# chzhang18/RAG

Hardware: AMD Instinct MI355X
Metric: disparity maps/sec at 384x1248 D=192 (Matching-Net forward) (higher is better)
Workload: dtype f32 (RAGMI_F32X3: level-3/6/12 3x3x3 convolutions with fp32 operands split into power-of-two-scaled FP16 hi+lo halves on the 16-bit matrix cores, hi*hi + hi*lo + lo*hi, fp32 accumulate: fp32-class accuracy, bound in include/rag_amd.h; strict_fp32 holds the RAGMI_F32 number); 1 GPU; BASELINE configs[1]: 1 stereo pair(s)/GPU/step, 384x1248, D=192, f32, all-conv genotype, (left_fea,right_fea)->disp, inputs resident in HBM; global_batch=1, launch=hipGraph, ranks_seen=1

## Files before the change

### include/rag_amd.h

```cpp
#ifndef RAG_AMD_H
#define RAG_AMD_H

#include <stdint.h>

#ifdef __cplusplus
extern "C" {
#endif

#define RAGMI_OK 0
#define RAGMI_EINVAL (-1)
#define RAGMI_EUNSUPPORTED (-2)
#define RAGMI_ELAUNCH (-3)

#define RAGMI_F32 0
#define RAGMI_BF16 1
#define RAGMI_F32X3 2

#define RAGMI_MAX_GROUPS 16

int ragmi_version(void);
const char* ragmi_last_error(void);

int ragmi_costvol_fwd(const void* left_fea, const void* right_fea, void* cost,
                      int B, int C, int d, int h, int w, int dtype, void* stream);

int64_t ragmi_conv3d_k3_packed_elems(int Cout, int Cin);
int ragmi_conv3d_k3_pack(const void* weight, void* packed, int Cout, int Cin, int dtype, void* stream);

int ragmi_conv3d_k3_fwd(const void* x, int64_t x_bstride,
                        const void* packed_weight, const void* scale, const void* shift, int relu,
                        void* y, int64_t y_bstride, const int32_t* y_group_ch,
                        const void* res, int64_t res_bstride, const int32_t* res_group_ch,
                        int B, int Cin, int Cout, int D, int H, int W,
                        int dtype, void* stream);

typedef struct {
  const void* weight;
  const void* scale;
  const void* shift;
  int32_t relu;
  void* y;
  int64_t y_bstride;
  int32_t y_ch0;
  int32_t cout;
} ragmi_tail_t;
int ragmi_down2_tail_supported(int D, int H, int W);

#define RAGMI_CONV_RELU 1
#define RAGMI_CONV_X_G4 2
#define RAGMI_CONV_Y_G4 4
#define RAGMI_TAIL_G4 4
#define RAGMI_TAIL_F32 8
#define RAGMI_TAIL_ROWS 16
#define RAGMI_OUT_F32 0x100
int ragmi_conv3d_k3_g4_caps(int Cin, int Cout, int B, int D, int H, int W, int nset, int ntail, int ndown, int dtype);

int ragmi_conv3d_k3_fwd_ex(const void* x, int64_t x_bstride,
                           const void* packed_weight, const void* scale, const void* shift, int relu,
                           void* y, int64_t y_bstride, const int32_t* y_group_ch,
                           const void* res, int64_t res_bstride, const int32_t* res_group_ch,
                           int B, int Cin, int Cout, int D, int H, int W,
                           int store_main, int ntail, const ragmi_tail_t* tails, int dtype, void* stream);
int ragmi_conv3d_k3_dual_fwd_ex(const void* x, int64_t x_bstride,
                                int CinA, const void* packedA, const void* scaleA, const void* shiftA,
                                int CinB, const void* packedB, const void* scaleB, const void* shiftB,
                                int relu, void* y, int64_t y_bstride, const int32_t* y_group_ch,
                                const void* res, int64_t res_bstride, const int32_t* res_group_ch,
                                int B, int Cout, int D, int H, int W,
                                int store_main, int ntail, const ragmi_tail_t* tails, int dtype, void* stream);

int ragmi_conv3d_k3_small_fwd(const void* x, int64_t x_bstride, const void* weight, const void* scale,
                              const void* shift, int relu, void* y, int64_t y_bstride, int y_ch0,
                              const void* res, int64_t res_bstride, int res_ch0,
                              int B, int Cin, int Cout, int D, int H, int W, int dtype, void* stream);

int ragmi_conv3d_k3_small_fwd_ex(const void* x, int64_t x_bstride, const void* weight, const void* scale,
                                 const void* shift, int relu, void* y, int64_t y_bstride, int y_ch0,
                                 const void* res, int64_t res_bstride, int res_ch0,
                                 int B, int Cin, int Cout, int D, int H, int W, int dtype, int y_dtype, void* stream);

int ragmi_conv3d_k3_dual_fwd(const void* x, int64_t x_bstride,
                             int CinA, const void* packedA, const void* scaleA, const void* shiftA,
                             int CinB, const void* packedB, const void* scaleB, const void* shiftB,
                             int relu, void* y, int64_t y_bstride, const int32_t* y_group_ch,
                             const void* res, int64_t res_bstride, const int32_t* res_group_ch,
                             int B, int Cout, int D, int H, int W, int dtype, void* stream);

int ragmi_conv3d_k3_plan(int Cout, int B, int D, int H, int W, int nset, int32_t* log_tx,
                         int32_t* rows_per_lane, int32_t* launch_groups, int32_t max_launches);

int ragmi_conv3d_k1_fwd(const void* x, int64_t x_bstride,
                        const void* weight, const void* scale, const void* shift, int relu,
                        void* y, int64_t y_bstride, int y_ch0,
                        int B, int Cin, int Cout, int64_t DHW,
                        int dtype, void* stream);

int ragmi_conv3d_k1_chain_supported(int Cin, int Cmid, int Cout);
int ragmi_conv3d_k1_chain_fwd(const void* x, int64_t x_bstride, const void* weight1, const void* scale1, const void* shift1, int relu1,
                              int Cmid, const void* weight2, const void* scale2, const void* shift2, int relu2,
                              void* y, int64_t y_bstride, int y_ch0, int B, int Cin, int Cout, int64_t DHW, int dtype, void* stream);

int ragmi_conv3d_k1_fwd_ex(const void* x, int64_t x_bstride, const void* weight, int w_transposed, const void* scale,
                           const void* shift, int relu, void* y, int64_t y_bstride, int y_ch0, int B, int Cin,
                           int Cout, int64_t DHW, int dtype, void* stream);

int ragmi_conv3d_k1_resample_fwd(const void* x, int64_t x_bstride, int Di, int Hi, int Wi,
                                 const void* weight, const void* scale, const void* shift, int relu,
                                 void* y, int64_t y_bstride, int y_ch0,
                                 int B, int Cin, int Cout, int Do, int Ho, int Wo, int align_corners,
                                 int dtype, void* stream);

typedef struct {
  const void* x;
  int64_t x_bstride;
  int32_t Di, Hi, Wi;
  const void* weight;
  const void* scale;
  const void* shift;
  int32_t relu;
  int32_t y_ch0;
  int32_t Cin, Cout;
} ragmi_k1r_t;
int ragmi_conv3d_k1_resample_pair_fwd(const ragmi_k1r_t* a, const ragmi_k1r_t* b, void* y, int64_t y_bstride,
                                      int B, int Do, int Ho, int Wo, int align_corners, int dtype, void* stream);
int ragmi_conv3d_k1_resample_multi_fwd(const ragmi_k1r_t* const* specs, void* const* ys, const int64_t* y_bstrides, int n, int B,
                                       int Do, int Ho, int Wo, int align_corners, int dtype, void* stream);

typedef struct {
  const void* x;
  int64_t x_bstride;
  int32_t Cin, Hi, Wi;
  const void* weight;
  const void* scale;
  const void* shift;
  int32_t relu;
} ragmi_cell2d_in_t;
int ragmi_cell2d_supported(int C, int Cin0, int Cin1, int Cout, int H, int W, int dtype);
int ragmi_cell2d_fwd(const ragmi_cell2d_in_t* s0, const ragmi_cell2d_in_t* s1, int C, const void* packedA, const void* scaleA,
                     const void* shiftA, const void* packedB, const void* scaleB, const void* shiftB, int relu, void* y,
                     int64_t y_bstride, const int32_t* y_group_ch, int B, int Cout, int H, int W, int dtype, void* stream);

int ragmi_trilinear3d_fwd(const void* x, void* y, int B, int C,
                          int Di, int Hi, int Wi, int Do, int Ho, int Wo,
                          int align_corners, int dtype, void* stream);

int ragmi_upconv3d_c1_supported(int Cin, int Di, int Hi, int Wi);
int ragmi_upconv3d_c1_fwd(const void* x, int64_t x_bstride, const void* weight, const void* scale, const void* shift, int relu, void* y,
                          int64_t y_bstride, int y_ch0, int B, int Cin, int Di, int Hi, int Wi, int dtype, int y_dtype, void* stream);

int ragmi_trilinear3d_act_fwd(const void* x, int64_t x_bstride, void* y, int64_t y_bstride, int y_ch0, int relu, int B, int C,
                              int Di, int Hi, int Wi, int Do, int Ho, int Wo, int align_corners, int dtype, void* stream);

int ragmi_conv2d_k3_strided_fwd(const void* x, const void* weight, const void* scale, const void* shift, int relu,
                                void* y, int B, int Cin, int Cout, int H, int W, int stride, int dtype, void* stream);

int ragmi_add_fwd(const void* a, int64_t a_bstride, int a_ch0,
                  const void* b, int64_t b_bstride, int b_ch0,
                  void* y, int64_t y_bstride, int y_ch0,
                  int B, int C, int64_t DHW, int dtype, void* stream);

int ragmi_disp_softargmin_fwd(const void* cost, void* out, int B, int d, int h, int w,
                              int maxdisp, int Ho, int Wo, int dtype, void* stream);

int ragmi_disparity_regression_fwd(const void* prob, void* out, int B, int D, int H, int W,
                                   int dtype, void* stream);

int64_t ragmi_costvol_stem_weights_elems(int C, int Cout);
int ragmi_costvol_stem_prepare(const void* weight, void* variants, int C, int Cout, void* stream);
int64_t ragmi_costvol_stem_workspace_elems(int B, int C, int Cout, int D, int H, int W);
int ragmi_costvol_stem_fwd(const void* left, const void* right, const void* variants, const void* scale, const void* shift, int relu,
                           void* y, int64_t y_bstride, void* workspace, int B, int C, int Cout, int D, int H, int W,
                           int ntail, const ragmi_tail_t* tails, int dtype, void* stream);

int ragmi_costvol_stem_conv3d_supported(int C, int Cmid, int Cout, int B, int D, int H, int W, int ntail, int dtype);
int ragmi_costvol_stem_conv3d_fwd(const void* left, const void* right, const void* variants, const void* scale0, const void* shift0, int relu0,
                                  void* workspace, int ntail0, const ragmi_tail_t* tails0,
                                  const void* packed_weight, const void* scale, const void* shift, int relu,
                                  void* y, int64_t y_bstride, const int32_t* y_group_ch, int store_main, int ntail, const ragmi_tail_t* tails,
                                  int B, int C, int Cmid, int Cout, int D, int H, int W, int dtype, void* stream);

int ragmi_conv3d_k3_uses_x3(int Cin, int Cout, int B, int D, int H, int W, int nset, int has_res, int ntail, int dtype);

int ragmi_conv3d_k3_pack_ex(const void* weight, void* packed, int Cout, int Cin, int transpose, int planar2d, int dtype, void* stream);

int ragmi_conv3d_k3_pack_for(const void* weight, void* packed, int Cout, int Cin, int transpose, int planar2d, int for_dtype, void* stream);


int64_t ragmi_bn_workspace_elems(int B, int C, int64_t DHW);
int ragmi_bn_train_stats_fwd(const void* x, int64_t x_bstride, int B, int C, int64_t DHW, const void* gamma, const void* beta,
                             void* running_mean, void* running_var, void* num_batches_tracked, float momentum, float eps,
                             void* workspace, void* mean, void* invstd, void* scale, void* shift, void* stream);

int ragmi_bn_train_act_fwd(const void* x, int64_t x_bstride, int B, int C, int64_t DHW, const void* gamma, const void* beta,
                           void* running_mean, void* running_var, void* num_batches_tracked, float momentum, float eps, int relu,
                           void* workspace, void* mean, void* invstd, void* scale, void* shift, void* y, int64_t y_bstride, int y_ch0,
                           const void* res, int64_t res_bstride, int res_ch0, void* stream);

int ragmi_bn_act_bwd(const void* dy, int64_t dy_bstride, int dy_ch0, const void* x, int64_t x_bstride, const void* scale,
                     const void* shift, int relu, const void* mean, const void* invstd, int training, int B, int C, int64_t DHW,
                     void* workspace, void* dx, int64_t dx_bstride, void* dgamma, void* dbeta, int accumulate, void* stream);

int ragmi_bn_act_fwd(const void* x, int64_t x_bstride, const void* scale, const void* shift, int relu,
                     const void* res, int64_t res_bstride, int res_ch0,
                     void* y, int64_t y_bstride, int y_ch0, int B, int C, int64_t DHW, void* stream);

int ragmi_bn_act_bwd_coeffs(const void* dy, int64_t dy_bstride, int dy_ch0, const void* x, int64_t x_bstride,
                            const void* scale, const void* shift, int relu, const void* mean, const void* invstd, int training,
                            int B, int C, int64_t DHW, void* workspace, void* c1, void* c2, void* c3, void* dgamma, void* dbeta,
                            int accumulate, void* stream);

int ragmi_bn_act_bwd_apply(const void* dy, int64_t dy_bstride, int dy_ch0, const void* x, int64_t x_bstride,
                           const void* scale, const void* shift, int relu, const void* c1, const void* c2, const void* c3,
                           void* dx, int64_t dx_bstride, int B, int C, int64_t DHW, void* stream);

int64_t ragmi_conv3d_k3_wgrad_workspace_elems(int B, int Cin, int Cout, int D, int H, int W);
int ragmi_conv3d_k3_wgrad(const void* x, int64_t x_bstride, const void* g, int64_t g_bstride, int g_ch0, void* const* dw_list, int n_dw,
                          int accumulate, int planar2d, void* workspace, int B, int Cin, int Cout, int D, int H, int W, void* stream);

int ragmi_conv3d_k1_wgrad(const void* x, int64_t x_bstride, const void* g, int64_t g_bstride, int g_ch0, void* dw,
                          int B, int Cin, int Cout, int64_t DHW, void* stream);

int ragmi_trilinear3d_bwd(const void* dy, void* dx, int B, int C, int Di, int Hi, int Wi, int Do, int Ho, int Wo,
                          int align_corners, void* stream);

int ragmi_costvol_bwd(const void* dcost, void* dleft, void* dright, int B, int C, int d, int h, int w, void* stream);

int ragmi_disp_softargmin_bwd(const void* cost, const void* dout, void* dcost, int B, int d, int h, int w,
                              int maxdisp, int Ho, int Wo, void* stream);

int ragmi_conv2d_k3_strided_dgrad(const void* g, const void* weight, void* dx, int B, int Cin, int Cout, int H, int W, int stride,
                                  void* stream);
int ragmi_conv2d_k3_strided_wgrad(const void* x, const void* g, void* dw, int B, int Cin, int Cout, int H, int W, int stride,
                                  void* stream);

int ragmi_disparity_regression_bwd(const void* dout, void* dprob, int B, int D, int H, int W, void* stream);

int ragmi_stereo_metrics_fwd(const void* disp_est, const void* disp_gt, int B, int H, int W, float maxdisp, void* acc, void* out,
                             void* stream);

int ragmi_masked_smooth_l1_bwd(const void* disp_est, const void* disp_gt, const void* out, const void* gout, void* ddisp,
                               int B, int H, int W, float maxdisp, void* stream);

int64_t ragmi_selfsup_loss_workspace_elems(int B, int H, int W);
int ragmi_selfsup_loss_fwd(const void* left, const void* right, const void* disp, int B, int C, int H, int W, int dtype,
                           void* workspace, void* out, void* unit_grad, void* stream);

int ragmi_selfsup_loss_bwd(const void* unit_grad, const void* gout, void* grad, int64_t n, void* stream);

int ragmi_depth_head_supported(int Cin, int Hi, int Wi, int H, int W, int scale, int dtype);
int ragmi_depth_head_fwd(const void* y, const void* w3, const void* w1, const void* b1, void* out, int B, int Cin, int Hi, int Wi,
                         int H, int W, int scale, float max_depth, int dtype, void* stream);

int ragmi_depth_metrics_workspace_elems(long long n);
int ragmi_depth_metrics_fwd(const void* est, const void* gt, long long n, float variance_focus, void* workspace, void* out10, int dtype,
                            void* stream);

int64_t ragmi_depth_head_bwd_workspace_elems(int B, int Cin, int H, int W);
int ragmi_depth_head_bwd(const void* y, const void* w3, const void* w1, const void* b1, const void* d_out, void* dy, void* dw3,
                         void* dw1, void* db1, int accumulate, void* workspace, int B, int Cin, int Hi, int Wi, int H, int W, int scale,
                         float max_depth, int dtype, void* stream);

int ragmi_silog_loss_workspace_elems(long long n);
int ragmi_silog_loss_fwd(const void* est, const void* gt, long long n, float variance_focus, void* workspace, void* out, void* saved,
                         int dtype, void* stream);

int ragmi_silog_loss_bwd(const void* est, const void* gt, long long n, float variance_focus, const void* saved, const void* gout,
                         void* grad, int dtype, void* stream);

int64_t ragmi_sgd_workspace_bytes(void);
int ragmi_sgd_clip_step(void* param, void* grad, void* momentum_buf, int64_t n, float lr, float momentum, float weight_decay,
                        float max_norm, int first_step, void* workspace, void* norm_out, void* stream);

#define RAGMI_GT_F32 0
#define RAGMI_GT_U16 1
int ragmi_prep_batch(const void* left_u8, const void* right_u8, const void* gt, int gt_dtype, float gt_scale, const void* origin,
                     void* left, void* right, void* gt_out, int B, int Hs, int Ws, int H, int W, float mean0, float mean1, float mean2,
                     float std0, float std1, float std2, const void* stats_left, const void* stats_right, const void* stats_source,
                     void* stream);

int64_t ragmi_color_stats_workspace_elems(int B, int Hs, int Ws);
int ragmi_color_stats(const void* img_u8, int B, int Hs, int Ws, void* workspace, void* stats, void* stream);

int ragmi_color_transfer(const void* target_u8, const void* stats_target, const void* stats_source, void* out_u8, int B, int H, int W,
                         void* stream);

int ragmi_graph_node_census(void* graph, int32_t* n_kernel, int32_t* n_memcpy, int32_t* n_memset, int32_t* n_other);

#ifdef __cplusplus
}
#endif
#endif
```

### rag_amd/_lib.py

```python
import ctypes
import os
import threading

_HERE = os.path.dirname(os.path.abspath(__file__))
_LIB = None
_LOCK = threading.Lock()

c_void_p, c_int, c_int64, c_float = ctypes.c_void_p, ctypes.c_int, ctypes.c_int64, ctypes.c_float
c_int32_p = ctypes.POINTER(ctypes.c_int32)

class TailSpec(ctypes.Structure):
    _fields_ = [("weight", c_void_p), ("scale", c_void_p), ("shift", c_void_p), ("relu", ctypes.c_int32),
                ("y", c_void_p), ("y_bstride", c_int64), ("y_ch0", ctypes.c_int32), ("cout", ctypes.c_int32)]


c_tail_p = ctypes.POINTER(TailSpec)


class K1RSpec(ctypes.Structure):
    _fields_ = [("x", c_void_p), ("x_bstride", c_int64), ("Di", ctypes.c_int32), ("Hi", ctypes.c_int32), ("Wi", ctypes.c_int32),
                ("weight", c_void_p), ("scale", c_void_p), ("shift", c_void_p), ("relu", ctypes.c_int32),
                ("y_ch0", ctypes.c_int32), ("Cin", ctypes.c_int32), ("Cout", ctypes.c_int32)]


c_k1r_p = ctypes.POINTER(K1RSpec)


class Cell2dIn(ctypes.Structure):
    _fields_ = [("x", c_void_p), ("x_bstride", c_int64), ("Cin", ctypes.c_int32), ("Hi", ctypes.c_int32), ("Wi", ctypes.c_int32),
                ("weight", c_void_p), ("scale", c_void_p), ("shift", c_void_p), ("relu", ctypes.c_int32)]


c_cell2d_p = ctypes.POINTER(Cell2dIn)

SIGNATURES = {
    "ragmi_version": (c_int, []),
    "ragmi_last_error": (ctypes.c_char_p, []),
    "ragmi_graph_node_census": (c_int, [c_void_p, c_int32_p, c_int32_p, c_int32_p, c_int32_p]),
    "ragmi_costvol_fwd": (c_int, [c_void_p, c_void_p, c_void_p, c_int, c_int, c_int, c_int, c_int, c_int, c_void_p]),
    "ragmi_costvol_stem_weights_elems": (c_int64, [c_int, c_int]),
    "ragmi_costvol_stem_prepare": (c_int, [c_void_p, c_void_p, c_int, c_int, c_void_p]),
    "ragmi_costvol_stem_workspace_elems": (c_int64, [c_int, c_int, c_int, c_int, c_int, c_int]),
    "ragmi_costvol_stem_fwd": (c_int, [c_void_p, c_void_p, c_void_p, c_void_p, c_void_p, c_int, c_void_p, c_int64, c_void_p,
                                       c_int, c_int, c_int, c_int, c_int, c_int, c_int, c_tail_p, c_int, c_void_p]),
    "ragmi_costvol_stem_conv3d_supported": (c_int, [c_int] * 9),
    "ragmi_costvol_stem_conv3d_fwd": (c_int, [c_void_p, c_void_p, c_void_p, c_void_p, c_void_p, c_int, c_void_p, c_int, c_tail_p,
                                              c_void_p, c_void_p, c_void_p, c_int, c_void_p, c_int64, c_int32_p, c_int, c_int, c_tail_p,
                                              c_int, c_int, c_int, c_int, c_int, c_int, c_int, c_int, c_void_p]),
    "ragmi_conv3d_k3_uses_x3": (c_int, [c_int] * 10),
    "ragmi_conv3d_k3_g4_caps": (c_int, [c_int] * 10),
    "ragmi_conv3d_k3_packed_elems": (c_int64, [c_int, c_int]),
    "ragmi_conv3d_k3_pack": (c_int, [c_void_p, c_void_p, c_int, c_int, c_int, c_void_p]),
    "ragmi_conv3d_k3_fwd": (c_int, [c_void_p, c_int64, c_void_p, c_void_p, c_void_p, c_int,
                                    c_void_p, c_int64, c_int32_p, c_void_p, c_int64, c_int32_p,
                                    c_int, c_int, c_int, c_int, c_int, c_int, c_int, c_void_p]),
    "ragmi_conv3d_k3_small_fwd": (c_int, [c_void_p, c_int64, c_void_p, c_void_p, c_void_p, c_int, c_void_p, c_int64, c_int,
                                          c_void_p, c_int64, c_int, c_int, c_int, c_int, c_int, c_int, c_int, c_int, c_void_p]),
    "ragmi_conv3d_k3_small_fwd_ex": (c_int, [c_void_p, c_int64, c_void_p, c_void_p, c_void_p, c_int, c_void_p, c_int64, c_int,
                                             c_void_p, c_int64, c_int, c_int, c_int, c_int, c_int, c_int, c_int, c_int, c_int, c_void_p]),
    "ragmi_conv3d_k3_dual_fwd": (c_int, [c_void_p, c_int64, c_int, c_void_p, c_void_p, c_void_p,
                                         c_int, c_void_p, c_void_p, c_void_p, c_int, c_void_p, c_int64, c_int32_p,
                                         c_void_p, c_int64, c_int32_p, c_int, c_int, c_int, c_int, c_int, c_int, c_void_p]),
    "ragmi_conv3d_k3_fwd_ex": (c_int, [c_void_p, c_int64, c_void_p, c_void_p, c_void_p, c_int,
                                       c_void_p, c_int64, c_int32_p, c_void_p, c_int64, c_int32_p,
                                       c_int, c_int, c_int, c_int, c_int, c_int, c_int, c_int, c_tail_p, c_int, c_void_p]),
    "ragmi_conv3d_k3_dual_fwd_ex": (c_int, [c_void_p, c_int64, c_int, c_void_p, c_void_p, c_void_p,
                                            c_int, c_void_p, c_void_p, c_void_p, c_int, c_void_p, c_int64, c_int32_p,
                                            c_void_p, c_int64, c_int32_p, c_int, c_int, c_int, c_int, c_int,
                                            c_int, c_int, c_tail_p, c_int, c_void_p]),
    "ragmi_conv3d_k3_plan": (c_int, [c_int, c_int, c_int, c_int, c_int, c_int, c_int32_p, c_int32_p, c_int32_p, c_int]),
    "ragmi_conv3d_k1_fwd": (c_int, [c_void_p, c_int64, c_void_p, c_void_p, c_void_p, c_int,
                                    c_void_p, c_int64, c_int, c_int, c_int, c_int, c_int64, c_int, c_void_p]),
    "ragmi_conv3d_k1_chain_supported": (c_int, [c_int] * 3),
    "ragmi_conv3d_k1_chain_fwd": (c_int, [c_void_p, c_int64, c_void_p, c_void_p, c_void_p, c_int, c_int, c_void_p, c_void_p, c_void_p, c_int,
                                          c_void_p, c_int64, c_int, c_int, c_int, c_int, c_int64, c_int, c_void_p]),
    "ragmi_conv3d_k1_fwd_ex": (c_int, [c_void_p, c_int64, c_void_p, c_int, c_void_p, c_void_p, c_int,
                                       c_void_p, c_int64, c_int, c_int, c_int, c_int, c_int64, c_int, c_void_p]),
    "ragmi_conv3d_k1_resample_fwd": (c_int, [c_void_p, c_int64, c_int, c_int, c_int, c_void_p, c_void_p, c_void_p, c_int,
                                             c_void_p, c_int64, c_int, c_int, c_int, c_int, c_int, c_int, c_int, c_int, c_int, c_void_p]),
    "ragmi_conv3d_k1_resample_pair_fwd": (c_int, [c_k1r_p, c_k1r_p, c_void_p, c_int64, c_int, c_int, c_int, c_int, c_int, c_int, c_void_p]),
    "ragmi_conv3d_k1_resample_multi_fwd": (c_int, [ctypes.POINTER(c_k1r_p), ctypes.POINTER(c_void_p), ctypes.POINTER(c_int64), c_int, c_int,
                                                   c_int, c_int, c_int, c_int, c_int, c_void_p]),
    "ragmi_down2_tail_supported": (c_int, [c_int, c_int, c_int]),
    "ragmi_cell2d_supported": (c_int, [c_int] * 7),
    "ragmi_cell2d_fwd": (c_int, [c_cell2d_p, c_cell2d_p, c_int, c_void_p, c_void_p, c_void_p, c_void_p, c_void_p, c_void_p, c_int,
                                 c_void_p, c_int64, c_int32_p, c_int, c_int, c_int, c_int, c_int, c_void_p]),
    "ragmi_upconv3d_c1_supported": (c_int, [c_int, c_int, c_int, c_int]),
    "ragmi_upconv3d_c1_fwd": (c_int, [c_void_p, c_int64, c_void_p, c_void_p, c_void_p, c_int, c_void_p, c_int64, c_int, c_int, c_int, c_int,
                                      c_int, c_int, c_int, c_int, c_void_p]),
    "ragmi_trilinear3d_act_fwd": (c_int, [c_void_p, c_int64, c_void_p, c_int64, c_int, c_int, c_int, c_int, c_int, c_int, c_int, c_int,
                                          c_int, c_int, c_int, c_int, c_void_p]),
    "ragmi_trilinear3d_fwd": (c_int, [c_void_p, c_void_p, c_int, c_int, c_int, c_int, c_int, c_int, c_int, c_int,
                                      c_int, c_int, c_void_p]),
    "ragmi_conv2d_k3_strided_fwd": (c_int, [c_void_p, c_void_p, c_void_p, c_void_p, c_int, c_void_p, c_int, c_int, c_int, c_int, c_int,
                                            c_int, c_int, c_void_p]),
    "ragmi_add_fwd": (c_int, [c_void_p, c_int64, c_int, c_void_p, c_int64, c_int, c_void_p, c_int64, c_int,
                              c_int, c_int, c_int64, c_int, c_void_p]),
    "ragmi_bn_workspace_elems": (c_int64, [c_int, c_int, c_int64]),
    "ragmi_bn_train_stats_fwd": (c_int, [c_void_p, c_int64, c_int, c_int, c_int64, c_void_p, c_void_p, c_void_p, c_void_p, c_void_p,
                                         c_float, c_float, c_void_p, c_void_p, c_void_p, c_void_p, c_void_p, c_void_p]),
    "ragmi_conv3d_k3_pack_ex": (c_int, [c_void_p, c_void_p, c_int, c_int, c_int, c_int, c_int, c_void_p]),
    "ragmi_conv3d_k3_pack_for": (c_int, [c_void_p, c_void_p, c_int, c_int, c_int, c_int, c_int, c_void_p]),
    "ragmi_sgd_workspace_bytes": (c_int64, []),
    "ragmi_sgd_clip_step": (c_int, [c_void_p, c_void_p, c_void_p, c_int64, c_float, c_float, c_float, c_float, c_int, c_void_p, c_void_p,
                                    c_void_p]),
    "ragmi_bn_train_act_fwd": (c_int, [c_void_p, c_int64, c_int, c_int, c_int64, c_void_p, c_void_p, c_void_p, c_void_p, c_void_p, c_float,
                                       c_float, c_int, c_void_p, c_void_p, c_void_p, c_void_p, c_void_p, c_void_p, c_int64, c_int,
                                       c_void_p, c_int64, c_int, c_void_p]),
    "ragmi_bn_act_bwd": (c_int, [c_void_p, c_int64, c_int, c_void_p, c_int64, c_void_p, c_void_p, c_int, c_void_p, c_void_p, c_int, c_int,
                                 c_int, c_int64, c_void_p, c_void_p, c_int64, c_void_p, c_void_p, c_int, c_void_p]),
    "ragmi_bn_act_fwd": (c_int, [c_void_p, c_int64, c_void_p, c_void_p, c_int, c_void_p, c_int64, c_int, c_void_p, c_int64, c_int,
                                 c_int, c_int, c_int64, c_void_p]),
    "ragmi_bn_act_bwd_coeffs": (c_int, [c_void_p, c_int64, c_int, c_void_p, c_int64, c_void_p, c_void_p, c_int, c_void_p, c_void_p, c_int,
                                        c_int, c_int, c_int64, c_void_p, c_void_p, c_void_p, c_void_p, c_void_p, c_void_p, c_int, c_void_p]),
    "ragmi_bn_act_bwd_apply": (c_int, [c_void_p, c_int64, c_int, c_void_p, c_int64, c_void_p, c_void_p, c_int, c_void_p, c_void_p,
                                       c_void_p, c_void_p, c_int64, c_int, c_int, c_int64, c_void_p]),
    "ragmi_conv3d_k3_wgrad_workspace_elems": (c_int64, [c_int, c_int, c_int, c_int, c_int, c_int]),
    "ragmi_conv3d_k3_wgrad": (c_int, [c_void_p, c_int64, c_void_p, c_int64, c_int, ctypes.POINTER(c_void_p), c_int, c_int, c_int, c_void_p,
                                      c_int, c_int, c_int, c_int, c_int, c_int, c_void_p]),
    "ragmi_conv3d_k1_wgrad": (c_int, [c_void_p, c_int64, c_void_p, c_int64, c_int, c_void_p, c_int, c_int, c_int, c_int64, c_void_p]),
    "ragmi_trilinear3d_bwd": (c_int, [c_void_p, c_void_p, c_int, c_int, c_int, c_int, c_int, c_int, c_int, c_int, c_int, c_void_p]),
    "ragmi_costvol_bwd": (c_int, [c_void_p, c_void_p, c_void_p, c_int, c_int, c_int, c_int, c_int, c_void_p]),
    "ragmi_conv2d_k3_strided_dgrad": (c_int, [c_void_p, c_void_p, c_void_p, c_int, c_int, c_int, c_int, c_int, c_int, c_void_p]),
    "ragmi_conv2d_k3_strided_wgrad": (c_int, [c_void_p, c_void_p, c_void_p, c_int, c_int, c_int, c_int, c_int, c_int, c_void_p]),
    "ragmi_disparity_regression_bwd": (c_int, [c_void_p, c_void_p, c_int, c_int, c_int, c_int, c_void_p]),
    "ragmi_stereo_metrics_fwd": (c_int, [c_void_p, c_void_p, c_int, c_int, c_int, c_float, c_void_p, c_void_p, c_void_p]),
    "ragmi_masked_smooth_l1_bwd": (c_int, [c_void_p, c_void_p, c_void_p, c_void_p, c_void_p, c_int, c_int, c_int, c_float, c_void_p]),
    "ragmi_selfsup_loss_workspace_elems": (c_int64, [c_int, c_int, c_int]),
    "ragmi_selfsup_loss_fwd": (c_int, [c_void_p, c_void_p, c_void_p, c_int, c_int, c_int, c_int, c_int, c_void_p, c_void_p, c_void_p,
                                       c_void_p]),
    "ragmi_selfsup_loss_bwd": (c_int, [c_void_p, c_void_p, c_void_p, c_int64, c_void_p]),
    "ragmi_depth_head_supported": (c_int, [c_int] * 7),
    "ragmi_depth_head_fwd": (c_int, [c_void_p, c_void_p, c_void_p, c_void_p, c_void_p, c_int, c_int, c_int, c_int, c_int, c_int, c_int,
                                     c_float, c_int, c_void_p]),
    "ragmi_depth_metrics_workspace_elems": (c_int, [ctypes.c_longlong]),
    "ragmi_depth_metrics_fwd": (c_int, [c_void_p, c_void_p, ctypes.c_longlong, c_float, c_void_p, c_void_p, c_int, c_void_p]),
    "ragmi_depth_head_bwd_workspace_elems": (c_int64, [c_int, c_int, c_int, c_int]),
    "ragmi_depth_head_bwd": (c_int, [c_void_p, c_void_p, c_void_p, c_void_p, c_void_p, c_void_p, c_void_p, c_void_p, c_void_p, c_int,
                                     c_void_p, c_int, c_int, c_int, c_int, c_int, c_int, c_int, c_float, c_int, c_void_p]),
    "ragmi_silog_loss_workspace_elems": (c_int, [ctypes.c_longlong]),
    "ragmi_silog_loss_fwd": (c_int, [c_void_p, c_void_p, ctypes.c_longlong, c_float, c_void_p, c_void_p, c_void_p, c_int, c_void_p]),
    "ragmi_silog_loss_bwd": (c_int, [c_void_p, c_void_p, ctypes.c_longlong, c_float, c_void_p, c_void_p, c_void_p, c_int, c_void_p]),
    "ragmi_prep_batch": (c_int, [c_void_p, c_void_p, c_void_p, c_int, c_float, c_void_p, c_void_p, c_void_p, c_void_p,
                                 c_int, c_int, c_int, c_int, c_int, c_float, c_float, c_float, c_float, c_float, c_float,
                                 c_void_p, c_void_p, c_void_p, c_void_p]),
    "ragmi_color_stats_workspace_elems": (c_int64, [c_int, c_int, c_int]),
    "ragmi_color_stats": (c_int, [c_void_p, c_int, c_int, c_int, c_void_p, c_void_p, c_void_p]),
    "ragmi_color_transfer": (c_int, [c_void_p, c_void_p, c_void_p, c_void_p, c_int, c_int, c_int, c_void_p]),
    "ragmi_disp_softargmin_bwd": (c_int, [c_void_p, c_void_p, c_void_p, c_int, c_int, c_int, c_int, c_int, c_int, c_int, c_void_p]),
    "ragmi_disp_softargmin_fwd": (c_int, [c_void_p, c_void_p, c_int, c_int, c_int, c_int, c_int, c_int, c_int,
                                          c_int, c_void_p]),
    "ragmi_disparity_regression_fwd": (c_int, [c_void_p, c_void_p, c_int, c_int, c_int, c_int, c_int, c_void_p]),
}


def lib_path() -> str:
    return os.environ.get("RAG_AMD_LIB", os.path.join(_HERE, "lib", "librag_amd.so"))


def load_library():
    global _LIB
    if _LIB is not None:
        return _LIB
    with _LOCK:
        if _LIB is None:
            path = lib_path()
            if not os.path.exists(path):
                raise RuntimeError(
                    f"rag_amd: HIP library not found at {path}. Build it with `make` at the repo root "
                    "(or `python -c 'import __graft_entry__ as g; g.build()'`). There is no CPU fallback.")
            lib = ctypes.CDLL(path)
            for name, (restype, argtypes) in SIGNATURES.items():
                fn = getattr(lib, name)
                fn.restype = restype
                fn.argtypes = argtypes
            _LIB = lib
    return _LIB


def check(status: int, what: str) -> None:
    if status != 0:
        msg = load_library().ragmi_last_error()
        raise RuntimeError(f"rag_amd.{what} failed with status {status}: {msg.decode() if msg else ''}")
```

### rag_amd/csrc/pointwise.hip

```cpp
#include <algorithm>

#include "common.h"

namespace ragmi {

struct K1Args {
  const void* x;
  int64_t x_bstride;
  const float* w;
  const float* scale;
  const float* shift;
  void* y;
  int64_t y_bstride;
  int y_ch0;
  int Cin, Cout, co0;
  int64_t dhw;
  int relu;
  int w_sco, w_sci;
  int y_f32;
};

template <class T, int NCO, bool VEC>
__global__ __launch_bounds__(256) void conv_k1_kernel(K1Args a) {
  constexpr int V = VEC ? 4 : 1;
  extern __shared__ __attribute__((aligned(16))) float k1_w[];
  a.co0 = blockIdx.z * NCO;
  for (int i = threadIdx.x; i < a.Cin * NCO; i += 256) {
    const int ci = i / NCO, co = a.co0 + i % NCO;
    k1_w[i] = co < a.Cout ? a.w[co * a.w_sco + ci * a.w_sci] : 0.f;
  }
  float* const k1_bn = k1_w + a.Cin * NCO;
  if (threadIdx.x < NCO) {
    const int co = min(a.co0 + (int)threadIdx.x, a.Cout - 1);
    k1_bn[threadIdx.x] = a.scale ? a.scale[co] : 1.f;
    k1_bn[NCO + threadIdx.x] = a.scale ? a.shift[co] : 0.f;
  }
  __syncthreads();
  const int64_t p = ((int64_t)blockIdx.x * 256 + threadIdx.x) * V;
  if (p >= a.dhw) return;
  const int b = blockIdx.y;
  const T* xp = static_cast<const T*>(a.x) + b * a.x_bstride + p;
  float acc[NCO][V];
#pragma unroll
  for (int j = 0; j < NCO; ++j)
#pragma unroll
    for (int k = 0; k < V; ++k) acc[j][k] = 0.f;

#pragma unroll 4
  for (int ci = 0; ci < a.Cin; ++ci) {
    float xv[V];
    if constexpr (VEC) {
      ld4(xp + (int64_t)ci * a.dhw, xv);
    } else {
      xv[0] = ld(xp + (int64_t)ci * a.dhw);
    }
    float wv[NCO];
#pragma unroll
    for (int j = 0; j < NCO; j += 4) {
      const float4 q = *reinterpret_cast<const float4*>(k1_w + ci * NCO + j);
      wv[j] = q.x; wv[j + 1] = q.y; wv[j + 2] = q.z; wv[j + 3] = q.w;
    }
#pragma unroll
    for (int j = 0; j < NCO; ++j)
#pragma unroll
      for (int k = 0; k < V; ++k) acc[j][k] = fmaf(wv[j], xv[k], acc[j][k]);
  }
  T* yp = static_cast<T*>(a.y) + b * a.y_bstride + p;
#pragma unroll
  for (int j = 0; j < NCO; ++j) {
    const int co = a.co0 + j;
    if (co >= a.Cout) break;
    const float sc = k1_bn[j], sh = k1_bn[NCO + j];
    float o[V];
#pragma unroll
    for (int k = 0; k < V; ++k) {
      float v = a.scale ? fmaf(acc[j][k], sc, sh) : acc[j][k];
      o[k] = a.relu ? fmaxf(v, 0.f) : v;
    }
    T* dst = yp + (int64_t)(a.y_ch0 + co) * a.dhw;
    if constexpr (VEC) st4(dst, o); else st(dst, o[0]);
  }
}

template <class T, int CMID, int NCO>
__global__ __launch_bounds__(256) void conv_k1_chain_kernel(K1Args a, const float* __restrict__ w2, const float* __restrict__ scale2,
                                                            const float* __restrict__ shift2, int relu2) {
  extern __shared__ __attribute__((aligned(16))) float kc_w[];
  float* const w2l = kc_w + a.Cin * CMID;
  float* const bn1 = w2l + CMID * NCO;
  float* const bn2 = bn1 + 2 * CMID;
  for (int i = threadIdx.x; i < a.Cin * CMID; i += 256) kc_w[i] = a.w[(i % CMID) * a.Cin + i / CMID];
  for (int i = threadIdx.x; i < CMID * NCO; i += 256) w2l[i] = w2[(i % NCO) * CMID + i / NCO];
  if (threadIdx.x < CMID) { bn1[threadIdx.x] = a.scale ? a.scale[threadIdx.x] : 1.f; bn1[CMID + threadIdx.x] = a.scale ? a.shift[threadIdx.x] : 0.f; }
  if (threadIdx.x < NCO) { bn2[threadIdx.x] = scale2 ? scale2[threadIdx.x] : 1.f; bn2[NCO + threadIdx.x] = scale2 ? shift2[threadIdx.x] : 0.f; }
  __syncthreads();
  const int64_t p = (int64_t)blockIdx.x * 256 + threadIdx.x;
  if (p >= a.dhw) return;
  const int b = blockIdx.y;
  const T* xp = static_cast<const T*>(a.x) + b * a.x_bstride + p;
  float h[CMID];
#pragma unroll
  for (int j = 0; j < CMID; ++j) h[j] = 0.f;
#pragma unroll 4
  for (int ci = 0; ci < a.Cin; ++ci) {
    const float xv = ld(xp + (int64_t)ci * a.dhw);
#pragma unroll
    for (int j = 0; j < CMID; j += 4) {
      const float4 q = *reinterpret_cast<const float4*>(kc_w + ci * CMID + j);
      h[j] = fmaf(q.x, xv, h[j]); h[j + 1] = fmaf(q.y, xv, h[j + 1]); h[j + 2] = fmaf(q.z, xv, h[j + 2]); h[j + 3] = fmaf(q.w, xv, h[j + 3]);
    }
  }
#pragma unroll
  for (int j = 0; j < CMID; ++j) {
    float v = a.scale ? fmaf(h[j], bn1[j], bn1[CMID + j]) : h[j];
    v = a.relu ? fmaxf(v, 0.f) : v;
    if constexpr (!std::is_same<T, float>::value) { const bf16_t r = to_bf16(v); v = ld(&r); }
    h[j] = v;
  }
  float acc[NCO];
#pragma unroll
  for (int k = 0; k < NCO; ++k) acc[k] = 0.f;
#pragma unroll
  for (int j = 0; j < CMID; ++j) {
#pragma unroll
    for (int k = 0; k < NCO; k += 4) {
      const float4 q = *reinterpret_cast<const float4*>(w2l + j * NCO + k);
      acc[k] = fmaf(q.x, h[j], acc[k]); acc[k + 1] = fmaf(q.y, h[j], acc[k + 1]); acc[k + 2] = fmaf(q.z, h[j], acc[k + 2]); acc[k + 3] = fmaf(q.w, h[j], acc[k + 3]);
    }
  }
  T* yp = static_cast<T*>(a.y) + b * a.y_bstride + p;
#pragma unroll
  for (int k = 0; k < NCO; ++k) {
    float v = scale2 ? fmaf(acc[k], bn2[k], bn2[NCO + k]) : acc[k];
    st(yp + (int64_t)(a.y_ch0 + k) * a.dhw, relu2 ? fmaxf(v, 0.f) : v);
  }
}

struct __attribute__((packed, aligned(4))) K1RF2 { float a, b; };
struct K1RArgs {
  K1Args k;
  int Di, Hi, Wi, Do, Ho, Wo;
  float sd, sh, sw;
  int align;
};

struct K1RPair {
  K1RArgs c[3];
  int splits[3];
};

template <class T, int NCO>
__global__ __launch_bounds__(256) void conv_k1_resample_kernel(K1RPair pr) {
  extern __shared__ __attribute__((aligned(16))) float k1r_w[];
  const int which = (int)blockIdx.z >= pr.splits[0] + pr.splits[1] ? 2 : ((int)blockIdx.z >= pr.splits[0] ? 1 : 0);
  const K1RArgs& r = pr.c[which];
  const K1Args& a = r.k;
  const int64_t ovol = (int64_t)r.Do * r.Ho * r.Wo;
  const int co0 = ((int)blockIdx.z - (which == 2 ? pr.splits[0] + pr.splits[1] : (which ? pr.splits[0] : 0))) * NCO;
  for (int i = threadIdx.x; i < a.Cin * NCO; i += 256) {
    const int ci = i / NCO, co = co0 + i % NCO;
    k1r_w[i] = co < a.Cout ? a.w[co * a.w_sco + ci * a.w_sci] : 0.f;
  }
  float* const k1r_bn = k1r_w + a.Cin * NCO;
  if (threadIdx.x < NCO) {
    const int co = min(co0 + (int)threadIdx.x, a.Cout - 1);
    k1r_bn[threadIdx.x] = a.scale ? a.scale[co] : 1.f;
    k1r_bn[NCO + threadIdx.x] = a.scale ? a.shift[co] : 0.f;
  }
  __syncthreads();
  const int64_t o = (int64_t)blockIdx.x * 256 + threadIdx.x;
  if (o >= ovol) return;
  const int b = blockIdx.y;
  const int ox = (int)(o % r.Wo);
  const int64_t t = o / r.Wo;
  const int oy = (int)(t % r.Ho), oz = (int)(t / r.Ho);
  const LinIdx lz = lin_index(oz, r.Di, r.Do, r.sd, r.align);
  const LinIdx ly = lin_index(oy, r.Hi, r.Ho, r.sh, r.align);
  const LinIdx lx = lin_index(ox, r.Wi, r.Wo, r.sw, r.align);
  const int64_t ivol = (int64_t)r.Di * r.Hi * r.Wi;
  const int r00 = (lz.i0 * r.Hi + ly.i0) * r.Wi, r01 = (lz.i0 * r.Hi + ly.i1) * r.Wi;
  const int r10 = (lz.i1 * r.Hi + ly.i0) * r.Wi, r11 = (lz.i1 * r.Hi + ly.i1) * r.Wi;
  const T* xp = static_cast<const T*>(a.x) + b * a.x_bstride;
  float acc[NCO];
#pragma unroll
  for (int j = 0; j < NCO; ++j) acc[j] = 0.f;
  constexpr int U = NCO <= 4 ? 8 : 4;
  if (r.Di == r.Do && r.Hi == r.Ho && r.Wi == r.Wo) {
    constexpr int UI = 16;
    for (int c0 = 0; c0 < a.Cin; c0 += UI) {
      float xv[UI];
#pragma unroll
      for (int u = 0; u < UI; ++u) xv[u] = ld(xp + (int64_t)min(c0 + u, a.Cin - 1) * ivol + o);
#pragma unroll
      for (int u = 0; u < UI; ++u) {
        if (c0 + u >= a.Cin) break;
        const int ci = c0 + u;
        float wv[NCO];
#pragma unroll
        for (int j = 0; j < NCO; j += 4) {
          const float4 q = *reinterpret_cast<const float4*>(k1r_w + ci * NCO + j);
          wv[j] = q.x; wv[j + 1] = q.y; wv[j + 2] = q.z; wv[j + 3] = q.w;
        }
#pragma unroll
        for (int j = 0; j < NCO; ++j) acc[j] = fmaf(wv[j], xv[u], acc[j]);
      }
    }
  } else {
    const bool pair = lx.i1 == lx.i0 + 1;
    for (int c0 = 0; c0 < a.Cin; c0 += U) {
      float tap[U][8];
#pragma unroll
      for (int u = 0; u < U; ++u) {
        const T* pc = xp + (int64_t)min(c0 + u, a.Cin - 1) * ivol;
        if constexpr (std::is_same<T, float>::value) {
          if (pair) {
            const K1RF2 q0 = *reinterpret_cast<const K1RF2*>(pc + r00 + lx.i0), q1 = *reinterpret_cast<const K1RF2*>(pc + r01 + lx.i0);
            const K1RF2 q2 = *reinterpret_cast<const K1RF2*>(pc + r10 + lx.i0), q3 = *reinterpret_cast<const K1RF2*>(pc + r11 + lx.i0);
            tap[u][0] = q0.a; tap[u][1] = q0.b; tap[u][2] = q1.a; tap[u][3] = q1.b;
            tap[u][4] = q2.a; tap[u][5] = q2.b; tap[u][6] = q3.a; tap[u][7] = q3.b;
            continue;
          }
        }
        tap[u][0] = ld(pc + r00 + lx.i0); tap[u][1] = ld(pc + r00 + lx.i1); tap[u][2] = ld(pc + r01 + lx.i0); tap[u][3] = ld(pc + r01 + lx.i1);
        tap[u][4] = ld(pc + r10 + lx.i0); tap[u][5] = ld(pc + r10 + lx.i1); tap[u][6] = ld(pc + r11 + lx.i0); tap[u][7] = ld(pc + r11 + lx.i1);
      }
#pragma unroll
      for (int u = 0; u < U; ++u) {
        if (c0 + u >= a.Cin) break;
        const int ci = c0 + u;
        const float a0 = lerp2(ly.w0, lerp2(lx.w0, tap[u][0], lx.w1, tap[u][1]), ly.w1, lerp2(lx.w0, tap[u][2], lx.w1, tap[u][3]));
        const float a1 = lerp2(ly.w0, lerp2(lx.w0, tap[u][4], lx.w1, tap[u][5]), ly.w1, lerp2(lx.w0, tap[u][6], lx.w1, tap[u][7]));
        const float xv = lerp2(lz.w0, a0, lz.w1, a1);
        float wv[NCO];
#pragma unroll
        for (int j = 0; j < NCO; j += 4) {
          const float4 q = *reinterpret_cast<const float4*>(k1r_w + ci * NCO + j);
          wv[j] = q.x; wv[j + 1] = q.y; wv[j + 2] = q.z; wv[j + 3] = q.w;
        }
#pragma unroll
        for (int j = 0; j < NCO; ++j) acc[j] = fmaf(wv[j], xv, acc[j]);
      }
    }
  }
  const int64_t yo = b * a.y_bstride + o;
  const bool yf32 = !std::is_same<T, float>::value && a.y_f32;
#pragma unroll
  for (int j = 0; j < NCO; ++j) {
    const int co = co0 + j;
    if (co >= a.Cout) break;
    float v = a.scale ? fmaf(acc[j], k1r_bn[j], k1r_bn[NCO + j]) : acc[j];
    v = a.relu ? fmaxf(v, 0.f) : v;
    const int64_t off = yo + (int64_t)(a.y_ch0 + co) * ovol;
    if (yf32) static_cast<float*>(a.y)[off] = v; else st(static_cast<T*>(a.y) + off, v);
  }
}

template <class T, int NCO>
static void launch_k1r_nco(const K1RArgs* r, int n, int B, hipStream_t s) {
  const int64_t ovol = (int64_t)r[0].Do * r[0].Ho * r[0].Wo;
  K1RPair pr{};
  int nz = 0, cin_max = 0;
  for (int i = 0; i < 3; ++i) {
    pr.c[i] = r[i < n ? i : n - 1];
    pr.splits[i] = i < n ? (int)ceil_div(r[i].k.Cout, NCO) : 0;
    nz += pr.splits[i];
    cin_max = std::max(cin_max, pr.c[i].k.Cin);
  }
  dim3 grid((unsigned)ceil_div(ovol, 256), B, (unsigned)nz);
  const size_t wlds = (size_t)(cin_max + 2) * NCO * sizeof(float);
  hipLaunchKernelGGL((conv_k1_resample_kernel<T, NCO>), grid, dim3(256), wlds, s, pr);
}

static int fill_k1r(K1RArgs& r, const void* x, int64_t x_bstride, int Di, int Hi, int Wi, const void* weight, const void* scale,
                    const void* shift, int relu, void* y, int64_t y_bstride, int y_ch0, int B, int Cin, int Cout, int Do, int Ho,
                    int Wo, int align_corners) {
  RAGMI_REQUIRE(x && weight && y, RAGMI_EINVAL, "conv3d_k1_resample: null pointer");
  RAGMI_REQUIRE((scale == nullptr) == (shift == nullptr), RAGMI_EINVAL, "conv3d_k1_resample: scale/shift must both be given or both NULL");
  RAGMI_REQUIRE(B > 0 && Cin > 0 && Cout > 0 && Di > 0 && Hi > 0 && Wi > 0 && Do > 0 && Ho > 0 && Wo > 0 && y_ch0 >= 0, RAGMI_EINVAL,
                "conv3d_k1_resample: bad size");
  RAGMI_REQUIRE(B <= 65535 && (int64_t)Di * Hi * Wi < (1ll << 31) && Cin <= 512, RAGMI_EUNSUPPORTED, "conv3d_k1_resample: size too large");
  r.k = K1Args{x, x_bstride, (const float*)weight, (const float*)scale, (const float*)shift,
               y, y_bstride, y_ch0, Cin, Cout, 0, (int64_t)Do * Ho * Wo, relu, Cin, 1};
  r.Di = Di; r.Hi = Hi; r.Wi = Wi; r.Do = Do; r.Ho = Ho; r.Wo = Wo;
  r.sd = lin_scale(Di, Do, align_corners); r.sh = lin_scale(Hi, Ho, align_corners); r.sw = lin_scale(Wi, Wo, align_corners);
  r.align = align_corners ? 1 : 0;
  return RAGMI_OK;
}

template <class T>
static int launch_k1r(const K1RArgs* r, int n, int B, hipStream_t s) {
  int cmax = 0;
  for (int i = 0; i < n; ++i) cmax = std::max(cmax, r[i].k.Cout);
  const int64_t threads = (int64_t)B * r[0].Do * r[0].Ho * r[0].Wo * n, want = 256 * 256 * 2;
  int64_t in_bytes = 0;
  for (int i = 0; i < n; ++i) in_bytes += (int64_t)B * r[i].k.Cin * r[i].Di * r[i].Hi * r[i].Wi * (int64_t)sizeof(T);
  static const int widths[5] = {24, 16, 12, 8, 4};
  int cover = 24;
  for (int w : widths)
    if (w >= cmax) cover = w;
  int nco = 4;
  if (threads >= want || in_bytes >= (128ll << 20)) {
    nco = cover;
  } else {
    for (int w : widths)
      if (w <= cover && (w == cover || cmax % w == 0) && threads * ceil_div(cmax, w) >= want) { nco = w; break; }
  }
  switch (nco) {
    case 24: launch_k1r_nco<T, 24>(r, n, B, s); break;
    case 16: launch_k1r_nco<T, 16>(r, n, B, s); break;
    case 12: launch_k1r_nco<T, 12>(r, n, B, s); break;
    case 8: launch_k1r_nco<T, 8>(r, n, B, s); break;
    default: launch_k1r_nco<T, 4>(r, n, B, s); break;
  }
  return check_launch("conv3d_k1_resample");
}

template <class T, bool VEC>
__global__ __launch_bounds__(256) void add_kernel(const T* __restrict__ a, int64_t a_bs, const T* __restrict__ b,
                                                  int64_t b_bs, T* __restrict__ y, int64_t y_bs, int64_t n) {
  constexpr int V = VEC ? 4 : 1;
  const int64_t p = ((int64_t)blockIdx.x * 256 + threadIdx.x) * V;
  if (p >= n) return;
  const int bi = blockIdx.y;
  if constexpr (VEC) {
    float u[4], v[4], o[4];
    ld4(a + bi * a_bs + p, u);
    ld4(b + bi * b_bs + p, v);
#pragma unroll
    for (int k = 0; k < 4; ++k) o[k] = u[k] + v[k];
    st4(y + bi * y_bs + p, o);
  } else {
    st(y + bi * y_bs + p, ld(a + bi * a_bs + p) + ld(b + bi * b_bs + p));
  }
}

template <class T, int NCO, bool VEC>
static void launch_k1_nco(const K1Args& a, int B, hipStream_t s) {
  constexpr int V = VEC ? 4 : 1;
  dim3 grid((unsigned)ceil_div(ceil_div(a.dhw, V), 256), B, (unsigned)ceil_div(a.Cout, NCO));
  hipLaunchKernelGGL((conv_k1_kernel<T, NCO, VEC>), grid, dim3(256), (size_t)(a.Cin + 2) * NCO * sizeof(float), s, a);
}

template <class T, bool VEC>
static void launch_k1(const K1Args& a, int B, hipStream_t s) {
  constexpr int V = VEC ? 4 : 1;
  const int64_t threads = (int64_t)B * ceil_div(a.dhw, V);
  const int64_t want = 256 * 256 * 4;
  static const int widths[5] = {24, 16, 12, 8, 4};
  int cover = 24;
  for (int w : widths)
    if (w >= a.Cout) cover = w;
  int nco = 4;
  if (threads >= want) {
    nco = cover;
  } else {
    for (int w : widths)
      if (w <= cover && threads * ceil_div(a.Cout, w) >= want) { nco = w; break; }
  }
  switch (nco) {
    case 24: launch_k1_nco<T, 24, VEC>(a, B, s); break;
    case 16: launch_k1_nco<T, 16, VEC>(a, B, s); break;
    case 12: launch_k1_nco<T, 12, VEC>(a, B, s); break;
    case 8: launch_k1_nco<T, 8, VEC>(a, B, s); break;
    default: launch_k1_nco<T, 4, VEC>(a, B, s); break;
  }
}

}

extern "C" int ragmi_conv3d_k1_fwd(const void* x, int64_t x_bstride, const void* weight, const void* scale,
                                   const void* shift, int relu, void* y, int64_t y_bstride, int y_ch0, int B, int Cin,
                                   int Cout, int64_t DHW, int dtype, void* stream) {
  return ragmi_conv3d_k1_fwd_ex(x, x_bstride, weight, 0, scale, shift, relu, y, y_bstride, y_ch0, B, Cin, Cout, DHW, dtype, stream);
}

extern "C" int ragmi_conv3d_k1_fwd_ex(const void* x, int64_t x_bstride, const void* weight, int w_transposed, const void* scale,
                                      const void* shift, int relu, void* y, int64_t y_bstride, int y_ch0, int B, int Cin,
                                      int Cout, int64_t DHW, int dtype, void* stream) {
  using namespace ragmi;
  RAGMI_REQUIRE(x && weight && y, RAGMI_EINVAL, "conv3d_k1: null pointer");
  RAGMI_REQUIRE((scale == nullptr) == (shift == nullptr), RAGMI_EINVAL, "conv3d_k1: scale/shift must both be given or both NULL");
  RAGMI_REQUIRE(B > 0 && Cin > 0 && Cout > 0 && DHW > 0 && y_ch0 >= 0, RAGMI_EINVAL, "conv3d_k1: bad size");
  RAGMI_REQUIRE(dtype_ok(dtype), RAGMI_EUNSUPPORTED, "conv3d_k1: dtype %d not built", dtype);
  RAGMI_REQUIRE(B <= 65535 && Cout <= 4 * 65535 && Cin <= 512, RAGMI_EUNSUPPORTED, "conv3d_k1: B, Cin or Cout too large");
  K1Args a{x, x_bstride, (const float*)weight, (const float*)scale, (const float*)shift,
           y, y_bstride, y_ch0, Cin, Cout, 0, DHW, relu, w_transposed ? 1 : Cin, w_transposed ? Cout : 1};
  const bool vec = (DHW % 4 == 0) && (x_bstride % 4 == 0) && (y_bstride % 4 == 0) && aligned4(x, dtype) && aligned4(y, dtype) &&
                   (int64_t)B * DHW >= (1 << 18);
  hipStream_t s = static_cast<hipStream_t>(stream);
  if (dtype == RAGMI_BF16) {
    if (vec) launch_k1<bf16_t, true>(a, B, s); else launch_k1<bf16_t, false>(a, B, s);
  } else {
    if (vec) launch_k1<float, true>(a, B, s); else launch_k1<float, false>(a, B, s);
  }
  return check_launch("conv3d_k1");
}

extern "C" int ragmi_conv3d_k1_chain_supported(int Cin, int Cmid, int Cout) { return (Cin >= 1 && Cin <= 64 && Cmid == 24 && Cout == 12) ? 1 : 0; }

extern "C" int ragmi_conv3d_k1_chain_fwd(const void* x, int64_t x_bstride, const void* weight1, const void* scale1, const void* shift1, int relu1,
                                         int Cmid, const void* weight2, const void* scale2, const void* shift2, int relu2, void* y, int64_t y_bstride,
                                         int y_ch0, int B, int Cin, int Cout, int64_t DHW, int dtype, void* stream) {
  using namespace ragmi;
  RAGMI_REQUIRE(x && weight1 && weight2 && y, RAGMI_EINVAL, "conv3d_k1_chain: null pointer");
  RAGMI_REQUIRE((scale1 == nullptr) == (shift1 == nullptr) && (scale2 == nullptr) == (shift2 == nullptr), RAGMI_EINVAL,
                "conv3d_k1_chain: scale/shift must both be given or both NULL");
  RAGMI_REQUIRE(B > 0 && B <= 65535 && DHW > 0 && y_ch0 >= 0, RAGMI_EINVAL, "conv3d_k1_chain: bad size");
  RAGMI_REQUIRE(dtype_ok(dtype), RAGMI_EUNSUPPORTED, "conv3d_k1_chain: dtype %d not built", dtype);
  RAGMI_REQUIRE(ragmi_conv3d_k1_chain_supported(Cin, Cmid, Cout), RAGMI_EUNSUPPORTED,
                "conv3d_k1_chain: built for Cin <= 64 -> 24 -> 12 channels (the head's last_12_3d -> last_6_3d), got %d -> %d -> %d", Cin, Cmid, Cout);
  K1Args a{x, x_bstride, (const float*)weight1, (const float*)scale1, (const float*)shift1, y, y_bstride, y_ch0, Cin, Cmid, 0, DHW, relu1, Cin, 1};
  const dim3 grid((unsigned)ceil_div(DHW, 256), B);
  const size_t lds = (size_t)(Cin * 24 + 24 * 12 + 2 * 24 + 2 * 12) * sizeof(float);
  hipStream_t s = static_cast<hipStream_t>(stream);
  if (dtype == RAGMI_BF16)
    hipLaunchKernelGGL((conv_k1_chain_kernel<bf16_t, 24, 12>), grid, dim3(256), lds, s, a, (const float*)weight2, (const float*)scale2, (const float*)shift2, relu2);
  else
    hipLaunchKernelGGL((conv_k1_chain_kernel<float, 24, 12>), grid, dim3(256), lds, s, a, (const float*)weight2, (const float*)scale2, (const float*)shift2, relu2);
  return check_launch("conv3d_k1_chain");
}

extern "C" int ragmi_conv3d_k1_resample_fwd(const void* x, int64_t x_bstride, int Di, int Hi, int Wi, const void* weight,
                                            const void* scale, const void* shift, int relu, void* y, int64_t y_bstride,
                                            int y_ch0, int B, int Cin, int Cout, int Do, int Ho, int Wo, int align_corners,
                                            int dtype, void* stream) {
  using namespace ragmi;
  const bool out_f32 = dtype == (RAGMI_BF16 | RAGMI_OUT_F32);
  if (out_f32) dtype = RAGMI_BF16;
  RAGMI_REQUIRE(dtype_ok(dtype), RAGMI_EUNSUPPORTED, "conv3d_k1_resample: dtype %d not built", dtype);
  K1RArgs r{};
  const int rc = fill_k1r(r, x, x_bstride, Di, Hi, Wi, weight, scale, shift, relu, y, y_bstride, y_ch0, B, Cin, Cout, Do, Ho, Wo, align_corners);
  if (rc != RAGMI_OK) return rc;
  r.k.y_f32 = out_f32 ? 1 : 0;
  return dtype == RAGMI_BF16 ? launch_k1r<bf16_t>(&r, 1, B, static_cast<hipStream_t>(stream))
                             : launch_k1r<float>(&r, 1, B, static_cast<hipStream_t>(stream));
}

extern "C" int ragmi_conv3d_k1_resample_pair_fwd(const ragmi_k1r_t* a, const ragmi_k1r_t* b, void* y, int64_t y_bstride, int B,
                                                 int Do, int Ho, int Wo, int align_corners, int dtype, void* stream) {
  using namespace ragmi;
  RAGMI_REQUIRE(a && b, RAGMI_EINVAL, "conv3d_k1_resample_pair: null descriptor");
  RAGMI_REQUIRE(dtype_ok(dtype), RAGMI_EUNSUPPORTED, "conv3d_k1_resample_pair: dtype %d not built", dtype);
  K1RArgs r[2]{};
  const ragmi_k1r_t* d[2] = {a, b};
  for (int i = 0; i < 2; ++i) {
    const int rc = fill_k1r(r[i], d[i]->x, d[i]->x_bstride, d[i]->Di, d[i]->Hi, d[i]->Wi, d[i]->weight, d[i]->scale, d[i]->shift,
                            d[i]->relu, y, y_bstride, d[i]->y_ch0, B, d[i]->Cin, d[i]->Cout, Do, Ho, Wo, align_corners);
    if (rc != RAGMI_OK) return rc;
  }
  return dtype == RAGMI_BF16 ? launch_k1r<bf16_t>(r, 2, B, static_cast<hipStream_t>(stream))
                             : launch_k1r<float>(r, 2, B, static_cast<hipStream_t>(stream));
}

extern "C" int ragmi_conv3d_k1_resample_multi_fwd(const ragmi_k1r_t* const* specs, void* const* ys, const int64_t* y_bstrides, int n, int B,
                                                  int Do, int Ho, int Wo, int align_corners, int dtype, void* stream) {
  using namespace ragmi;
  RAGMI_REQUIRE(specs && ys && y_bstrides && n >= 1 && n <= 3, RAGMI_EINVAL, "conv3d_k1_resample_multi: 1..3 descriptors");
  RAGMI_REQUIRE(dtype_ok(dtype), RAGMI_EUNSUPPORTED, "conv3d_k1_resample_multi: dtype %d not built", dtype);
  K1RArgs r[3]{};
  for (int i = 0; i < n; ++i) {
    RAGMI_REQUIRE(specs[i], RAGMI_EINVAL, "conv3d_k1_resample_multi: null descriptor");
    const ragmi_k1r_t* d = specs[i];
    const int rc = fill_k1r(r[i], d->x, d->x_bstride, d->Di, d->Hi, d->Wi, d->weight, d->scale, d->shift, d->relu, ys[i], y_bstrides[i],
                            d->y_ch0, B, d->Cin, d->Cout, Do, Ho, Wo, align_corners);
    if (rc != RAGMI_OK) return rc;
  }
  return dtype == RAGMI_BF16 ? launch_k1r<bf16_t>(r, n, B, static_cast<hipStream_t>(stream))
                             : launch_k1r<float>(r, n, B, static_cast<hipStream_t>(stream));
}

extern "C" int ragmi_add_fwd(const void* a, int64_t a_bstride, int a_ch0, const void* b, int64_t b_bstride, int b_ch0,
                             void* y, int64_t y_bstride, int y_ch0, int B, int C, int64_t DHW, int dtype, void* stream) {
  using namespace ragmi;
  RAGMI_REQUIRE(a && b && y, RAGMI_EINVAL, "add: null pointer");
  RAGMI_REQUIRE(B > 0 && C > 0 && DHW > 0 && a_ch0 >= 0 && b_ch0 >= 0 && y_ch0 >= 0, RAGMI_EINVAL, "add: bad size");
  RAGMI_REQUIRE(dtype_ok(dtype), RAGMI_EUNSUPPORTED, "add: dtype %d not built", dtype);
  RAGMI_REQUIRE(B <= 65535, RAGMI_EUNSUPPORTED, "add: B too large");
  const size_t es = dtype_size(dtype);
  const char* ap = (const char*)a + (int64_t)a_ch0 * DHW * es;
  const char* bp = (const char*)b + (int64_t)b_ch0 * DHW * es;
  char* yp = (char*)y + (int64_t)y_ch0 * DHW * es;
  const int64_t n = (int64_t)C * DHW;
  const bool vec = (n % 4 == 0) && (DHW % 4 == 0) && (a_bstride % 4 == 0) && (b_bstride % 4 == 0) && (y_bstride % 4 == 0) &&
                   aligned4(ap, dtype) && aligned4(bp, dtype) && aligned4(yp, dtype);
  hipStream_t s = static_cast<hipStream_t>(stream);
  auto go = [&](auto tag) {
    using T = decltype(tag);
    if (vec)
      hipLaunchKernelGGL((add_kernel<T, true>), dim3((unsigned)ceil_div(n / 4, 256), B), dim3(256), 0, s, (const T*)ap, a_bstride,
                         (const T*)bp, b_bstride, (T*)yp, y_bstride, n);
    else
      hipLaunchKernelGGL((add_kernel<T, false>), dim3((unsigned)ceil_div(n, 256), B), dim3(256), 0, s, (const T*)ap, a_bstride,
                         (const T*)bp, b_bstride, (T*)yp, y_bstride, n);
  };
  if (dtype == RAGMI_BF16) go(bf16_t{}); else go(float{});
  return check_launch("add");
}
```

### rag_amd/modules.py

```python
from __future__ import annotations

from collections import namedtuple
from types import MappingProxyType
from typing import Dict, List, Optional, Sequence, Tuple

import numpy as np

import torch
import torch.nn as nn

from . import autograd as ag
from . import ops

Genotype = namedtuple("Genotype_2D", "normal normal_concat reduce reduce_concat")
PRIMITIVES_3D = ["skip_connect_3d", "3d_conv_3x3"]

ALL_CONV_ROWS = np.array([[0, 1], [1, 1], [2, 1], [3, 1], [5, 1], [6, 1]])
ALL_SKIP_ROWS = np.array([[0, 0], [1, 0], [2, 0], [3, 0], [5, 0], [6, 0]])
ALL_CONV_GENOTYPE = Genotype(normal=ALL_CONV_ROWS, normal_concat=None, reduce=ALL_CONV_ROWS, reduce_concat=None)


def _volume(size) -> int:
    n = 1
    for v in size:
        n *= int(v)
    return n


ALL_SKIP_GENOTYPE = Genotype(normal=ALL_SKIP_ROWS, normal_concat=None, reduce=ALL_SKIP_ROWS, reduce_concat=None)


class Identity_3d(nn.Module):

    def forward(self, x):
        return x


class _ConvBR(nn.Module):

    NDIM = 3

    def __init__(self, C_in, C_out, kernel_size, stride, padding, bn=True, relu=True):
        super().__init__()
        self.relu = relu
        self.use_bn = bn
        if self.NDIM == 3:
            self.conv = nn.Conv3d(C_in, C_out, kernel_size, stride=stride, padding=padding, bias=False)
            self.bn = nn.BatchNorm3d(C_out)
        else:
            self.conv = nn.Conv2d(C_in, C_out, kernel_size, stride=stride, padding=padding, bias=False)
            self.bn = nn.BatchNorm2d(C_out)
        self._initialize_weights()
        self._cache = None

    def _initialize_weights(self):
        nn.init.kaiming_normal_(self.conv.weight, mode="fan_out", nonlinearity="relu")
        nn.init.constant_(self.bn.weight, 1)
        nn.init.constant_(self.bn.bias, 0)

    def _geometry(self) -> int:
        k, n = self.conv.kernel_size, self.NDIM
        same = self.conv.padding == tuple((ki - 1) // 2 for ki in k) and self.conv.dilation == (1,) * n and self.conv.groups == 1
        if same and k in ((1,) * n, (3,) * n) and self.conv.stride == (1,) * n:
            return k[0]
        if same and n == 2 and k == (3, 3) and self.conv.stride[0] == self.conv.stride[1] > 1:
            return -3
        raise NotImplementedError("rag_amd ConvBR: only 1x1(x1)/pad0 and 3x3(x3)/pad1 at stride 1 (plus the strided 2-D 3x3 "
                                  "stem) are built (everything the reference instantiates)")

    def _small(self) -> bool:
        return (self.NDIM == 3 and self.conv.out_channels <= 2 and self.conv.in_channels % 4 == 0
                and self.conv.in_channels <= 128)

    def stamp(self) -> tuple:
        w, bn = self.conv.weight, self.bn
        return (w.data_ptr(), w._version, bn.weight._version, bn.bias._version, bn.running_mean._version,
                bn.running_var._version, bn.weight.data_ptr(), str(w.device), self.use_bn)

    def prepared(self) -> Tuple[torch.Tensor, Optional[torch.Tensor], Optional[torch.Tensor]]:
        if self.use_bn and self.bn.training:
            raise RuntimeError("rag_amd ConvBR: folded BatchNorm parameters requested in train mode (internal error: "
                               "train-mode units run through rag_amd.autograd)")
        stamp = self.stamp()
        if self._cache is None or self._cache[0] != stamp:
            k = self._geometry()
            w = self.conv.weight.detach()
            with torch.no_grad():
                if k == -3 or (k == 3 and self._small()):
                    wk = w.contiguous()
                elif k == 3:
                    wk = ops.conv3d_k3_pack(w)
                else:
                    wk = w.reshape(w.shape[0], w.shape[1]).contiguous()
                if self.use_bn:
                    bn = self.bn
                    scale = (bn.weight.detach() * torch.rsqrt(bn.running_var.detach() + bn.eps)).float().contiguous()
                    shift = (bn.bias.detach() - bn.running_mean.detach() * scale).float().contiguous()
                else:
                    scale = shift = None
            self._cache = (stamp, wk, scale, shift)
        return self._cache[1], self._cache[2], self._cache[3]

    def autograd_mode(self, *inputs) -> bool:
        return (ag.needs_grad(*inputs, self.conv.weight, self.bn.weight, self.bn.bias)
                or (self.use_bn and self.bn.training))

    def _forward_autograd(self, x: torch.Tensor, resample_to: Optional[Sequence[int]]) -> torch.Tensor:
        if x.dtype != torch.float32:
            raise NotImplementedError("rag_amd: the training path is fp32 (bf16 storage is inference only)")
        if self._geometry() == -3:
            return ag.StridedStemFn.apply(x if x.dim() == 4 else x.squeeze(2), self.conv.weight, self.bn.weight, self.bn.bias, self)
        squeeze = x.dim() == 4
        if squeeze:
            x = x.unsqueeze(2)
        if resample_to is not None:
            x = ag.resample(x, resample_to, True)
        y = ag.ConvBRFn.apply(x, self.conv.weight, self.bn.weight, self.bn.bias, self)
        return y.squeeze(2) if squeeze else y

    def costvol_fusable(self, C_fea: int) -> bool:
        return (self.NDIM == 3 and self._geometry() == 3 and self.conv.in_channels == 2 * C_fea and C_fea <= 16
                and self.conv.out_channels <= 16)

    def costvol_variants(self) -> torch.Tensor:
        w = self.conv.weight
        key = (w.data_ptr(), w._version, str(w.device))
        hit = getattr(self, "_cv_cache", None)
        if hit is None or hit[0] != key:
            with torch.no_grad():
                hit = (key, ops.costvol_stem_prepare(w.detach()))
            self._cv_cache = hit
        return hit[1]

    def forward_costvol(self, left_fea, right_fea, maxdisp, tails=None, out_g4: bool = False) -> torch.Tensor:
        _wk, scale, shift = self.prepared()
        return ops.costvol_stem(left_fea, right_fea, maxdisp, self.costvol_variants(), self.conv.out_channels, scale, shift,
                                self.relu, tails=tails, out_g4=out_g4)

    def as_tail(self, out: torch.Tensor, out_ch0: int, g4: bool = False) -> "ops.Tail":
        if self._geometry() != 1 or self.conv.out_channels > 4:
            raise ValueError("only 1x1x1 ConvBR with <= 4 output channels can be fused as a tail")
        wk, scale, shift = self.prepared()
        return ops.Tail(wk, scale, shift, self.relu, out, out_ch0, g4=g4)

    def as_down_tails(self, out: torch.Tensor, out_ch0: int) -> List["ops.Tail"]:
        if self._geometry() != 1 or self.conv.out_channels > 8:
            raise ValueError("only 1x1x1 ConvBR with <= 8 output channels can be fused as down-sampling tails")
        wk, scale, shift = self.prepared()
        tails = []
        for c0 in range(0, self.conv.out_channels, 4):
            c1 = min(c0 + 4, self.conv.out_channels)
            tails.append(ops.Tail(wk[c0:c1], None if scale is None else scale[c0:c1], None if shift is None else shift[c0:c1],
                                  self.relu, out, out_ch0 + c0, down=True))
        return tails

    def forward(self, x: torch.Tensor, out: Optional[torch.Tensor] = None, out_ch0: int = 0,
                resample_to: Optional[Sequence[int]] = None, tails: Optional[Sequence["ops.Tail"]] = None,
                store_main: bool = True, out_dtype: Optional[torch.dtype] = None, x_g4: bool = False) -> torch.Tensor:
        if self.autograd_mode(x):
            if out is not None or tails:
                raise RuntimeError("rag_amd ConvBR: fused destinations/tails belong to the inference executor")
            return self._forward_autograd(x, resample_to)
        k = self._geometry()
        wk, scale, shift = self.prepared()
        cout = self.conv.out_channels
        if x_g4 and (k != 3 or self._small() or resample_to is not None or x.dim() != 5):
            raise RuntimeError("rag_amd ConvBR: a G4 input is taken by the 3x3x3 form only")
        if k == -3:
            return ops.conv2d_k3_strided(x if x.dim() == 4 else x[:, :, 0], wk, scale, shift, self.relu, self.conv.stride[0])
        squeeze = x.dim() == 4
        if squeeze:
            x = x.unsqueeze(2)
        mixed = out is not None and out.dtype != x.dtype
        if mixed:
            if k != 1 or x.dtype != torch.bfloat16 or out.dtype != torch.float32:
                raise RuntimeError("rag_amd ConvBR: only a 1x1x1 conv crosses from bf16 storage to an fp32 destination")
            resample_to = tuple(x.shape[2:]) if resample_to is None else resample_to
        elif resample_to is not None and tuple(resample_to) == tuple(x.shape[2:]):
            resample_to = None
        if resample_to is not None:
            if k != 1:
                raise NotImplementedError("ConvBR: fused resample is built for the 1x1x1 form only")
            if out is None:
                out = torch.empty((x.shape[0], cout) + tuple(int(v) for v in resample_to), device=x.device, dtype=x.dtype)
            if not mixed and _volume(resample_to) > _volume(x.shape[2:]) and cout <= x.shape[1]:
                low = torch.empty((x.shape[0], cout) + tuple(x.shape[2:]), device=x.device, dtype=x.dtype)
                ops.conv3d_k1(x, wk, scale, shift, False, low)
                ops.trilinear3d_act(low, resample_to, True, self.relu, out, out_ch0)
            else:
                ops.conv3d_k1_resample(x, resample_to, True, wk, scale, shift, self.relu, out, out_ch0)
            return out[:, :, 0] if squeeze else out
        if out is None:
            odt = out_dtype if (out_dtype is not None and k == 3 and self._small()) else x.dtype
            out = torch.empty((x.shape[0], cout) + tuple(x.shape[2:]), device=x.device, dtype=odt)
        if k == 3 and self._small():
            ops.conv3d_k3_small(x, wk, scale, shift, self.relu, out, out_ch0)
        elif k == 3:
            groups = [out_ch0 + 4 * g for g in range(ops.packed_groups(cout))]
            ops.conv3d_k3(x, wk, cout, scale, shift, self.relu, out, groups, tails=tails, store_main=store_main, x_g4=x_g4)
        else:
            ops.conv3d_k1(x, wk, scale, shift, self.relu, out, out_ch0)
        return out[:, :, 0] if squeeze else out


class ConvBR_3d(_ConvBR):
    NDIM = 3


class ConvBR_2d(_ConvBR):
    NDIM = 2


class Identity_2d(nn.Module):

    def forward(self, x):
        return x


def _skip(C, stride):
    if stride != 1:
        raise NotImplementedError("skip_connect_3d with stride != 1 is dead code in the reference (FactorizedReduce typo)")
    return Identity_3d()


OPS_3d = {
    "skip_connect_3d": _skip,
    "3d_conv_3x3": lambda C, stride: ConvBR_3d(C, C, 3, stride, 1),
}


PRIMITIVES = ["skip_connect_2d", "conv_3x3"]


def _skip_2d(C, stride):
    if stride != 1:
        raise NotImplementedError("skip_connect_2d with stride != 1 is dead code in the reference")
    return Identity_2d()


OPS_2d = {"skip_connect_2d": _skip_2d, "conv_3x3": lambda C, stride: ConvBR_2d(C, C, 3, stride, 1)}


class DisparityRegression(nn.Module):

    def __init__(self, maxdisp):
        super().__init__()
        self.maxdisp = maxdisp

    def forward(self, x):
        assert x.is_contiguous() is True
        if ag.needs_grad(x):
            return ag.DispRegFn.apply(x, self.maxdisp)
        return ops.disparity_regression(x, self.maxdisp)


class Disp(nn.Module):

    def __init__(self, maxdisp=192):
        super().__init__()
        self.maxdisp = maxdisp
        self.softmax = nn.Softmin(dim=1)
        self.disparity = DisparityRegression(maxdisp=self.maxdisp)

    def forward(self, x):
        if ag.needs_grad(x):
            return ag.DispFn.apply(x, self.maxdisp)
        return ops.disp_softargmin(x, self.maxdisp)


class _Cell(nn.Module):

    def __init__(self, steps, block_multiplier, prev_prev_fmultiplier, prev_filter_multiplier, genotype,
                 filter_multiplier, downup_sample):
        super().__init__()
        self.genotype = genotype
        self.C_in = block_multiplier * filter_multiplier
        self.C_out = filter_multiplier
        self.C_prev = int(block_multiplier * prev_filter_multiplier)
        self.C_prev_prev = int(block_multiplier * prev_prev_fmultiplier)
        self.downup_sample = downup_sample
        self.pre_preprocess = self.CONV(self.C_prev_prev, self.C_out, 1, 1, 0)
        self.preprocess = self.CONV(self.C_prev, self.C_out, 1, 1, 0)
        self._steps = steps
        self.block_multiplier = block_multiplier
        self._ops = nn.ModuleList()
        if downup_sample == -1:
            self.scale = 0.5
        elif downup_sample == 1:
            self.scale = 2
        for x in self._rows():
            self._ops.append(self.OPS[self.PRIMS[x[1]]](self.C_out, stride=1))
        self._fused_cache: Dict[tuple, tuple] = {}

    def _rows(self):
        raise NotImplementedError

    def scale_dimension(self, dim, scale):
        return int((float(dim) - 1.0) * scale + 1.0) if dim % 2 == 1 else int(float(dim) * scale)

    def _contributions(self) -> Dict[int, List[Tuple[int, nn.Module]]]:
        selected = set(int(v) for v in np.asarray(self._rows())[:, 0])
        contribs: Dict[int, List[Tuple[int, nn.Module]]] = {}
        offset, n_states, ops_index = 0, 2, 0
        for _ in range(self._steps):
            lst = []
            for j in range(n_states):
                if offset + j in selected:
                    lst.append((j, self._ops[ops_index]))
                    ops_index += 1
            contribs[n_states] = lst
            offset += n_states
            n_states += 1
        return contribs

    def _fused(self, mods: Sequence[ConvBR_3d]):
        key = tuple(id(m) for m in mods)
        stamps = tuple(m.stamp() for m in mods)
        hit = self._fused_cache.get(key)
        if hit is None or hit[0] != stamps:
            prep = [m.prepared() for m in mods]
            if len(mods) == 1:
                fused = prep[0]
            else:
                with torch.no_grad():
                    wk = ops.conv3d_k3_pack(torch.cat([m.conv.weight.detach() for m in mods]))
                fused = (wk, torch.cat([p[1] for p in prep]), torch.cat([p[2] for p in prep]))
            hit = (stamps, fused)
            self._fused_cache[key] = hit
        return hit[1]

    def _convbrs(self):
        units = self.__dict__.get("_convbr_cache")
        if units is None:
            units = [m for m in self.modules() if isinstance(m, _ConvBR)]
            self.__dict__["_convbr_cache"] = units
        return units

    def autograd_mode(self, *inputs) -> bool:
        units = self._convbrs()
        if torch.is_grad_enabled():
            if any(t is not None and t.requires_grad for t in inputs):
                return True
            if any(m.conv.weight.requires_grad or m.bn.weight.requires_grad or m.bn.bias.requires_grad for m in units):
                return True
        return any(m.use_bn and m.bn.training for m in units)

    def forward(self, prev_prev_input, prev_input):
        run = self._run_autograd if self.autograd_mode(prev_prev_input, prev_input) else self._run
        if prev_input.dim() == 4:
            return prev_input, run(prev_prev_input.unsqueeze(2), prev_input.unsqueeze(2)).squeeze(2)
        return prev_input, run(prev_prev_input, prev_input)

    def _run_autograd(self, prev_prev_input, prev_input):
        s0, s1 = prev_prev_input, prev_input
        if self.downup_sample != 0:
            s1 = ag.resample(s1, self.out_size(s1.shape[2:]), True)
        s0 = ag.resample(s0, s1.shape[2:], True)
        if s0.shape[1] != self.C_out:
            s0 = self.pre_preprocess(s0)
        s1 = self.preprocess(s1)
        states = [s0, s1]
        contribs = self._contributions()
        n_states = 2 + self._steps
        pending: Dict[int, list] = {k: [] for k in contribs}
        for k, lst in contribs.items():
            if not lst:
                raise ValueError("Cell_3d: a step with no selected branch (the reference fails in torch.cat here too)")
        for j in range(n_states):
            if j >= 2:
                acc = pending[j][0]
                for h in pending[j][1:]:
                    acc = ag.AddFn.apply(acc, h)
                states.append(acc)
            out_ops = [(k, op) for k, lst in contribs.items() for (src, op) in lst if src == j]
            convs = [(k, op) for (k, op) in out_ops if isinstance(op, _ConvBR)]
            grouped = (len(convs) > 1 and all(op._geometry() == 3 and op.use_bn and op.relu for _k, op in convs)
                       and states[j].dtype == torch.float32)
            if grouped:
                params = [p for _k, op in convs for p in (op.conv.weight, op.bn.weight, op.bn.bias)]
                fuse = all(len(pending[k]) == 1 and pending[k][0].dtype == torch.float32 for k, _op in convs)
                res = [pending[k][0] for k, _op in convs] if fuse else []
                outs = dict(zip([k for k, _op in convs],
                                ag.ConvBRGroupFn.apply(states[j], tuple(op for _k, op in convs), *params, *res)))
                if fuse:
                    for k, _op in convs:
                        pending[k].clear()
            for k, op in out_ops:
                pending[k].append(outs[k] if (grouped and isinstance(op, _ConvBR)) else op(states[j]))
        return torch.cat(states[-self.block_multiplier:], dim=1)

    def out_size(self, prev_size: Sequence[int]) -> Tuple[int, int, int]:
        if self.downup_sample == 0:
            return tuple(int(v) for v in prev_size)
        return tuple(self.scale_dimension(int(v), self.scale) for v in prev_size)

    def dual_branches(self, s0_in_pre: bool):
        contribs = self._contributions()
        a, b = ([(k, op) for k, lst in contribs.items() for (src, op) in lst if src == j and isinstance(op, _ConvBR)] for j in (0, 1))
        first_cat = 2 + self._steps - self.block_multiplier
        if not (a and s0_in_pre and [k for k, _ in a] == [k for k, _ in b] and all(len(contribs[k]) == 2 for k, _ in a)
                and len({k >= first_cat for k, _ in a}) == 1):
            return None, None, False
        return a, b, len(a) == self._steps and self.block_multiplier == self._steps

    def _run(self, prev_prev_input, prev_input, plan: Optional["_CellPlan"] = None, pre: Optional[torch.Tensor] = None,
             tails: Optional[Sequence["ops.Tail"]] = None):
        C = self.C_out
        if C % 4 != 0 or self.block_multiplier > self._steps:
            raise NotImplementedError("rag_amd.Cell_3d: filter_multiplier must be a multiple of 4 and "
                                      "block_multiplier <= steps (true for every cell the reference builds)")
        s0, s1 = prev_prev_input, prev_input
        pre_has = plan.has if plan is not None else (False, False)
        a, b, whole = self.dual_branches(pre_has[0] or s0.shape[1] != C)
        if plan is None:
            plan = _CellPlan(size=self.out_size(s1.shape[2:]), dtype=s1.dtype, has=pre_has, g4=False, dual=whole, store_main=True, tails=False,
                             shared_pre=False)
        size = tuple(int(v) for v in plan.size)
        if not pre_has[0] and s0.shape[1] == C and tuple(s0.shape[2:]) != size:
            s0 = ops.trilinear3d(s0, size, True)
        D, H, W = size
        if (D == 1 and whole and pre is None and not tails and plan.store_main and s0.shape[1] != C and s1.dtype == torch.float32
                and s0.dtype == torch.float32 and ops.get_conv_precision() == "f16x3"
                and ops.cell2d_supported(C, s0.shape[1], s1.shape[1], C * self._steps, H, W)):
            cat = torch.empty((s1.shape[0], self.block_multiplier * C, D, H, W), device=s1.device, dtype=s1.dtype)
            pa, sa, ha = self._fused([op for _k, op in a])
            pb, sb, hb = self._fused([op for _k, op in b])
            groups = [(k - 2) * C + 4 * g for k, _op in a for g in range(C // 4)]
            ops.cell2d(s0, self.pre_preprocess.prepared() + (self.pre_preprocess.relu,), s1,
                       self.preprocess.prepared() + (self.preprocess.relu,), C, pa, sa, ha, pb, sb, hb, C * self._steps, True, cat, groups)
            return cat
        if pre is None:
            pre = torch.empty((s1.shape[0], 2 * C, D, H, W), device=s1.device, dtype=plan.dtype)
        B, dev, adt = pre.shape[0], pre.device, pre.dtype
        n_states = 2 + self._steps
        first_cat = n_states - self.block_multiplier
        contribs = self._contributions()
        cat = (pre if not plan.store_main else
               torch.empty((B, self.block_multiplier * C, D, H, W), device=dev, dtype=adt))
        scratch = (torch.empty((B, (first_cat - 2) * C, D, H, W), device=dev, dtype=adt)
                   if first_cat > 2 else None)

        where: List[Tuple[torch.Tensor, int]] = []
        grows = any(s is not None and _volume(size) > _volume(s.shape[2:]) and C <= s.shape[1] for s in (s0, s1))
        if not pre_has[0] and not pre_has[1] and s0.shape[1] != C and not grows and s0.dtype == s1.dtype == adt:
            w0, sc0, sh0 = self.pre_preprocess.prepared()
            w1, sc1, sh1 = self.preprocess.prepared()
            ops.conv3d_k1_resample_pair([(s0, w0, sc0, sh0, self.pre_preprocess.relu, 0),
                                         (s1, w1, sc1, sh1, self.preprocess.relu, C)], size, pre)
            where.append((pre, 0))
        else:
            if pre_has[0]:
                where.append((pre, 0))
            elif s0.shape[1] != C:
                self.pre_preprocess(s0, out=pre, out_ch0=0, resample_to=size)
                where.append((pre, 0))
            else:
                where.append((s0.contiguous(), 0))
            if not pre_has[1]:
                self.preprocess(s1, out=pre, out_ch0=C, resample_to=size)
        where.append((pre, C))
        for k in range(2, n_states):
            where.append((cat, (k - first_cat) * C) if k >= first_cat else (scratch, (k - 2) * C))

        written = {k: False for k in contribs}
        pending_id = {k: [j for (j, op) in lst if not isinstance(op, _ConvBR)] for k, lst in contribs.items()}
        for k, lst in contribs.items():
            if not lst:
                raise ValueError("Cell_3d: a step with no selected branch (the reference fails in torch.cat here too)")

        def finalize(k: int) -> None:
            buf, ch = where[k]
            ids = pending_id[k]
            while ids:
                if not written[k]:
                    if len(ids) >= 2:
                        (ba, ca), (bb, cb) = where[ids[0]], where[ids[1]]
                        ops.add(ba, ca, bb, cb, buf, ch, C)
                        del ids[:2]
                    else:
                        bs, cs = where[ids.pop(0)]
                        torch.mul(bs[:, cs:cs + C], 1, out=buf[:, ch:ch + C])
                    written[k] = True
                else:
                    bs, cs = where[ids.pop(0)]
                    ops.add(buf, ch, bs, cs, buf, ch, C)

        done = set()
        if a is not None:
            pa, sa, ha = self._fused([op for _k, op in a])
            pb, sb, hb = self._fused([op for _k, op in b])
            groups = [where[k][1] + 4 * g for k, _op in a for g in range(C // 4)]
            ops.conv3d_k3_dual(pre, C, pa, sa, ha, pb, sb, hb, C * len(a), True, where[a[0][0]][0], groups,
                               tails=tails, store_main=plan.store_main, x_g4=plan.g4)
            for j, branches in enumerate((a, b)):
                for k, op in branches:
                    written[k] = True
                    done.add((j, id(op)))

        for j in range(n_states):
            if j >= 2:
                finalize(j)
            parts: Dict[object, list] = {}
            for k, lst in contribs.items():
                for (src, op) in lst:
                    if src != j or not isinstance(op, _ConvBR) or (j, id(op)) in done:
                        continue
                    if written[k]:
                        res = where[k]
                    else:
                        ready = [i for i in pending_id[k] if i <= j]
                        if ready:
                            pending_id[k].remove(ready[0])
                            res = where[ready[0]]
                        else:
                            res = None
                    written[k] = True
                    parts.setdefault(None if res is None else id(res[0]), []).append((k, op, res))
            if not parts:
                continue
            xbuf, xch = where[j]
            x = xbuf[:, xch:xch + C]
            for items in parts.values():
                mods = [op for (_k, op, _r) in items]
                packed, scale, shift = self._fused(mods)
                out_groups, res_groups = [], []
                for (k, _op, res) in items:
                    out_groups += [where[k][1] + 4 * g for g in range(C // 4)]
                    if res is not None:
                        res_groups += [res[1] + 4 * g for g in range(C // 4)]
                res_buf = items[0][2][0] if items[0][2] is not None else None
                by_buf: Dict[int, list] = {}
                for idx, (k, _op, _res) in enumerate(items):
                    by_buf.setdefault(id(where[k][0]), []).append(idx)
                if len(by_buf) == 1:
                    ops.conv3d_k3(x, packed, C * len(mods), scale, shift, True, where[items[0][0]][0], out_groups,
                                  res_buf, res_groups if res_buf is not None else None)
                else:
                    for idxs in by_buf.values():
                        sub = [items[i] for i in idxs]
                        p2, s2, h2 = self._fused([op for (_k, op, _r) in sub])
                        og = [where[k][1] + 4 * g for (k, _o, _r) in sub for g in range(C // 4)]
                        rg = [r[1] + 4 * g for (_k, _o, r) in sub if r is not None for g in range(C // 4)]
                        ops.conv3d_k3(x, p2, C * len(sub), s2, h2, True, where[sub[0][0]][0], og,
                                      res_buf, rg if res_buf is not None else None)
        for k in contribs:
            finalize(k)
        return cat if plan.store_main else None


class Cell_3d(_Cell):
    CONV, OPS, PRIMS = ConvBR_3d, OPS_3d, PRIMITIVES_3D

    def _rows(self):
        return self.genotype.reduce


class Cell_2d(_Cell):
    CONV, OPS, PRIMS = ConvBR_2d, OPS_2d, PRIMITIVES

    def _rows(self):
        return self.genotype.normal


_CELL3D_ARCH = ((4, 4, 4, 0), (4, 4, 4, 0), (4, 4, 4, 0), (4, 4, 8, -1),
                (4, 8, 16, -1), (8, 16, 8, 1), (16, 8, 16, -1), (8, 16, 16, 0))


_CellPlan = namedtuple("_CellPlan", "size dtype has g4 dual store_main tails shared_pre")
_ChainPlan = namedtuple("_ChainPlan", "sizes cdt consumers stored cells stem0_g4 stems_fused stem_tail_rows")


def _down_tail_ok(prod, cons, B, src, dst, src_dt, dst_dt) -> bool:
    return ((src_dt != torch.float32 or ops.get_conv_precision() == "f16x3")
            and (dst_dt == src_dt or (src_dt == torch.bfloat16 and dst_dt == torch.float32))
            and tuple(2 * v for v in dst) == tuple(src) and ops.down2_tail_supported(*src)
            and cons.C_out <= 8 and cons.C_out % 4 == 0 and prod.downup_sample == 0 and prod.C_out == 4 and prod.C_out * prod._steps <= 16
            and ops.conv3d_k3_uses_x3(2 * prod.C_out, prod.C_out * prod._steps, B, *src, nset=2, ntail=1, dtype=src_dt))


def _plan_chain(stem0, stem1, cells, B: int, C_fea: int, vol, adt: torch.dtype, folded: bool) -> _ChainPlan:
    n = len(cells)
    f32, bf16 = torch.float32, torch.bfloat16
    caps = ops.conv3d_k3_g4_caps
    x3 = (adt == f32 and ops.get_conv_precision() == "f16x3") or adt == bf16
    sizes, cdt = {-2: tuple(vol), -1: tuple(vol)}, {-2: adt, -1: adt}
    cout = {-2: stem0.conv.out_channels, -1: stem1.conv.out_channels}
    for i, c in enumerate(cells):
        sizes[i] = c.out_size(sizes[i - 1])
        deep = adt == bf16 and ops.bf16_deep_fp32_enabled() and (
            _volume(sizes[i]) * ops.bf16_deep_fp32_ratio() <= _volume(vol) or f32 in (cdt[i - 1], cdt[i - 2]))
        cdt[i] = f32 if deep else adt
        cout[i] = c.block_multiplier * c.C_out

    consumers = {}
    for i in range(-2, n):
        found = []
        for j, role in ((i + 1, 1), (i + 2, 0)):
            c = cells[j] if 0 <= j < n else None
            if c is None or (role == 0 and (c.C_prev_prev == c.C_out or (j > 0 and cells[j - 1].downup_sample != 0))):
                continue
            if c.downup_sample == 0 and c.C_out == 4 and cdt[j] == cdt[i]:
                found.append((j, role, False))
            elif c.downup_sample == -1 and i >= 0 and _down_tail_ok(cells[i], c, B, sizes[i], sizes[j], cdt[i], cdt[j]):
                found.append((j, role, True))
        consumers[i] = tuple(found)
    nfull = {i: sum(not d for (_j, _r, d) in consumers[i]) for i in consumers}
    ndown = {i: sum((cells[j].C_out + 3) // 4 for (j, _r, d) in consumers[i] if d) for i in consumers}
    dual = [c.dual_branches((i, 0, False) in consumers[i - 2] or (i, 0, True) in consumers[i - 2] or cout[i - 2] != c.C_out)[2]
            for i, c in enumerate(cells)]
    tails = {i: bool(consumers[i]) and dual[i] and cout[i] <= 16 for i in range(n)}
    tails[-2] = tails[-1] = True

    g4_ok = x3 and ops.g4_enabled()
    writes = {i: bool(g4_ok and nfull[i] and tails[i]
                      and caps(2 * c.C_out, cout[i], B, *sizes[i], nset=2, ntail=nfull[i], ndown=ndown[i], dtype=cdt[i]) & 2)
              for i, c in enumerate(cells)}
    writes[-2] = bool(g4_ok and nfull[-2] and (folded or caps(stem0.conv.in_channels, cout[-2], B, *vol, nset=1, ntail=nfull[-2], dtype=adt) & 2))
    writes[-1] = bool(g4_ok and nfull[-1] and caps(cout[-2], cout[-1], B, *vol, nset=1, ntail=nfull[-1], dtype=adt) & 2)
    g4 = [bool((j, 1, False) in consumers[j - 1] and (j, 0, False) in consumers[j - 2] and writes[j - 1] and writes[j - 2] and dual[j]
               and caps(2 * c.C_out, cout[j], B, *sizes[j], nset=2, ntail=nfull[j] if tails[j] else 0, ndown=ndown[j] if tails[j] else 0,
                        dtype=cdt[j]) & 1) for j, c in enumerate(cells)]
    changed = True
    while changed:
        changed = False
        for i in range(-2, n):
            js = [j for (j, _r, d) in consumers[i] if not d]
            if len({g4[j] for j in js}) > 1:
                for j in js:
                    g4[j] = False
                changed = True
    alone = folded and (0, 0, False) in consumers[-2]
    stem0_g4 = bool(g4_ok and alone and caps(cout[-2], cout[-1], B, *vol, nset=1, ntail=nfull[-1], dtype=adt) & 1)
    stems_fused = bool(x3 and alone and ops.stem_fusion_enabled() and cout[-2] == 12 and stem1._geometry() == 3 and not stem1._small()
                       and ops.costvol_stem_conv3d_supported(C_fea, 12, cout[-1], B, *vol, ntail=nfull[-1], dtype=adt))
    stem_tail_rows = stems_fused and ops.stem_tail_rows_enabled() and cout[-1] == 12

    stored = {i: i == n - 1 or not tails[i] or len(consumers[i]) < sum(0 <= j < n for j in (i + 1, i + 2)) for i in range(-1, n)}
    stored[-2] = not stems_fused
    has = [[False, False] for _ in cells]
    plans = []
    for i in range(-2, n):
        if i >= 0:
            j = i + 1
            shared = (j < n and not any(has[i]) and not has[j][0] and sizes[i] == sizes[j] != sizes[i - 1] and stored[i - 2] and stored[i - 1]
                      and cout[i - 2] != cells[i].C_out and cout[i - 1] != cells[j].C_out and len({cdt[i - 2], cdt[i - 1], cdt[i], cdt[j]}) == 1
                      and _volume(sizes[i]) <= min(_volume(sizes[i - 2]), _volume(sizes[i - 1])))
            if shared:
                has[i], has[j][0] = [True, True], True
            plans.append(_CellPlan(sizes[i], cdt[i], tuple(has[i]), g4[i], dual[i], stored[i], tails[i], shared))
        for (j, role, _d) in consumers[i]:
            has[j][role] = True
    ro = MappingProxyType
    return _ChainPlan(ro(sizes), ro(cdt), ro(consumers), ro(stored), tuple(plans), stem0_g4, stems_fused, stem_tail_rows)


class MatchingNet(nn.Module):

    def __init__(self, genotype=ALL_CONV_GENOTYPE, maxdisp: int = 192):
        super().__init__()
        self._init_matching(genotype, maxdisp)

    def _init_matching(self, genotype, maxdisp):
        self._step = 3
        self._block_multiplier = 3
        self._filter_multiplier = 4
        self._num_layers_3d = 8
        initial_fm = self._filter_multiplier * self._block_multiplier
        if not hasattr(self, "length"):
            self.length, self.arch_init = {}, {}
        for name in ("stem_3d0", "stem_3d1", "last_3_3d", "last_6_3d", "last_12_3d"):
            self.length[name] = 1
            self.arch_init[name] = [0]
        self.cells_3d = nn.ModuleList()
        self.stem3d0 = nn.ModuleList([ConvBR_3d(initial_fm * 2, initial_fm, 3, stride=1, padding=1)])
        self.stem3d1 = nn.ModuleList([ConvBR_3d(initial_fm, initial_fm, 3, stride=1, padding=1)])
        for i in range(self._num_layers_3d):
            self.cells_3d.append(nn.ModuleList([self._new_cell_3d(i, genotype)]))
            self.arch_init["cell_3d" + str(i)] = [0]
            self.length["cell_3d" + str(i)] = 1
        self.last_3_3d = nn.ModuleList([ConvBR_3d(initial_fm, 1, 3, 1, 1, bn=False, relu=False)])
        self.last_6_3d = nn.ModuleList([ConvBR_3d(initial_fm * 2, initial_fm, 1, 1, 0)])
        self.last_12_3d = nn.ModuleList([ConvBR_3d(initial_fm * 4, initial_fm * 2, 1, 1, 0)])
        self.maxdisp = maxdisp
        self.disp = Disp(self.maxdisp)

    def _new_cell_3d(self, i: int, genotype) -> Cell_3d:
        pp, p, fm, du = _CELL3D_ARCH[i]
        return Cell_3d(self._step, self._block_multiplier, pp, p, genotype, fm, du)

    def matching(self, x, task_arch, path=None, features=None):
        def unit(name):
            return task_arch[name][0] if task_arch is not None else None

        cells = []
        for i, cell in enumerate(self.cells_3d):
            arch_cell = None
            if task_arch is not None:
                arch_cell = task_arch["cell_3d" + str(i)][0]
            elif path is not None:
                arch_cell = path[i + 1]
            cells.append(cell[arch_cell])
        last = self._run_chain(x, self.stem3d0[unit("stem_3d0")], self.stem3d1[unit("stem_3d1")], cells, features)
        return self._head(self._vol_size(x, features), last, unit("last_3_3d"), unit("last_6_3d"), unit("last_12_3d"))

    def search_matching(self, x, selected_ops, t, features=None):
        cells = [cell[selected_ops[i + 10]] for i, cell in enumerate(self.cells_3d)]
        last = self._run_chain(x, self.stem3d0[selected_ops[8]], self.stem3d1[selected_ops[9]], cells, features)
        return self._head(self._vol_size(x, features), last, t, t, t)

    def _vol_size(self, x, features):
        if x is not None:
            return tuple(x.shape[2:])
        return (int(self.maxdisp / 3),) + tuple(features[0].shape[2:])

    def _run_chain(self, x, stem0, stem1, cells, features=None):
        train = (stem0.autograd_mode(*(features if x is None else (x,))) or stem1.autograd_mode()
                 or any(c.autograd_mode() for c in cells))
        if x is None and (train or not stem0.costvol_fusable(features[0].shape[1])):
            x = self.cost_volume(*features)
        if train:
            out = (stem0(x),)
            out = (out[0], stem1(out[0]))
            for c in cells:
                out = c(out[0], out[1])
            return out[-1]
        n = len(cells)
        ref = x if x is not None else features[0]
        B, dev = ref.shape[0], ref.device
        plan = _plan_chain(stem0, stem1, cells, B, ref.shape[1], self._vol_size(x, features), ref.dtype, x is None)
        sizes, keep1 = plan.sizes, plan.stored[-1]
        self.last_g4_plan = {"pre": {j: cp.g4 for j, cp in enumerate(plan.cells)}, "stem0_out": plan.stem0_g4,
                             "stems_fused": plan.stems_fused, **({"stem_tail_rows": plan.stem_tail_rows} if plan.stems_fused else {})}
        pre: Dict[int, torch.Tensor] = {}

        def buf(j):
            if j not in pre:
                pre[j] = torch.empty((B, 2 * cells[j].C_out) + sizes[j], device=dev, dtype=plan.cdt[j])
            return pre[j]

        def unit(j, role):
            return cells[j].preprocess if role else cells[j].pre_preprocess, buf(j), cells[j].C_out * role

        def tails(i):
            out = []
            for (j, role, down) in plan.consumers[i]:
                mod, dst, ch0 = unit(j, role)
                out += mod.as_down_tails(dst, ch0) if down else [mod.as_tail(dst, ch0, g4=plan.cells[j].g4)]
            return out or None

        T: Dict[int, Optional[torch.Tensor]] = {-2: None}
        t0, t1 = tails(-2), tails(-1)
        if plan.stems_fused:
            _w0, scale0, shift0 = stem0.prepared()
            wk1, scale1, shift1 = stem1.prepared()
            cout1 = stem1.conv.out_channels
            if plan.stem_tail_rows:
                key = (stem1.stamp(), cells[0].pre_preprocess.stamp())
                hit = getattr(stem1, "_rows_cache", None)
                if hit is None or hit[0] != key:
                    with torch.no_grad():
                        hit = (key, ops.conv3d_k3_pack(ops.stem_tail_rows_weight(stem1.conv.weight.detach(), t0[0].weight2d)))
                    stem1._rows_cache = hit
                wk1 = hit[1]
            out1 = torch.empty((B, cout1) + sizes[-1], device=dev, dtype=ref.dtype) if keep1 else None
            ops.costvol_stem_conv3d(features[0], features[1], self.maxdisp, stem0.costvol_variants(), 12, scale0, shift0, stem0.relu, t0,
                                    wk1, cout1, scale1, shift1, stem1.relu, out1, [4 * g for g in range(ops.packed_groups(cout1))],
                                    tails=t1, store_main=keep1, tail0_rows=plan.stem_tail_rows)
        else:
            if x is None:
                T[-2] = stem0.forward_costvol(features[0], features[1], self.maxdisp, tails=t0, out_g4=plan.stem0_g4)
            else:
                T[-2] = stem0(x, tails=t0)
            out1 = stem1(T[-2], tails=t1, store_main=keep1, x_g4=plan.stem0_g4)
        T[-1] = out1 if keep1 else None
        for i, (c, cp) in enumerate(zip(cells, plan.cells)):
            if cp.shared_pre:
                cj = cells[i + 1]
                ops.conv3d_k1_resample_multi([(T[i - 2],) + c.pre_preprocess.prepared() + (c.pre_preprocess.relu, buf(i), 0),
                                              (T[i - 1],) + c.preprocess.prepared() + (c.preprocess.relu, buf(i), c.C_out),
                                              (T[i - 1],) + cj.pre_preprocess.prepared() + (cj.pre_preprocess.relu, buf(i + 1), 0)], sizes[i])
            T[i] = c._run(T[i - 2], T[i - 1], cp, pre.get(i), tails(i) if cp.tails else None)
            if not cp.tails:
                for (j, role, down) in plan.consumers[i]:
                    mod, dst, ch0 = unit(j, role)
                    mod(T[i], out=dst, out_ch0=ch0, resample_to=sizes[j] if down else None)
            T.pop(i - 2, None)
        return T[n - 1]

    def _head(self, vol, last_output, i3, i6, i12):
        d, h, w = vol
        f32 = torch.float32
        if last_output.size()[3] == h:
            return self.last_3_3d[i3](last_output, out_dtype=f32)
        heads = (self.last_3_3d[i3], self.last_6_3d[i6], self.last_12_3d[i12])
        up = ag.resample if any(m.autograd_mode(last_output) for m in heads) else ops.trilinear3d
        def up_last3(y):
            m3 = self.last_3_3d[i3]
            if (up is ops.trilinear3d and m3._small() and m3.conv.out_channels == 1 and tuple(y.shape[2:]) == (d // 2, h // 2, w // 2)
                    and (d, h, w) == (2 * (d // 2), 2 * (h // 2), 2 * (w // 2)) and ops.upconv3d_c1_supported(y.shape[1], d // 2, h // 2, w // 2)):
                wk, scale, shift = m3.prepared()
                return ops.upconv3d_c1(y, wk, scale, shift, m3.relu, out_dtype=f32)
            return m3(up(y, (d, h, w), True), out_dtype=f32)

        if last_output.size()[3] == h // 2:
            return up_last3(self.last_6_3d[i6](last_output))
        if last_output.size()[3] == h // 4:
            m12 = self.last_12_3d[i12]
            if (last_output.dtype == torch.bfloat16 and ops.bf16_head_fp32_enabled() and not m12.autograd_mode(last_output)
                    and m12._geometry() == 1):
                y12 = m12(last_output, out=torch.empty((last_output.shape[0], m12.conv.out_channels) + tuple(last_output.shape[2:]),
                                                       device=last_output.device, dtype=f32))
            else:
                m6 = self.last_6_3d[i6]
                half = (d // 2, h // 2, w // 2)
                if (up is ops.trilinear3d and m12._geometry() == 1 and m6._geometry() == 1 and ops.chain_k1_enabled()
                        and _volume(half) > _volume(last_output.shape[2:]) and m6.conv.out_channels <= m6.conv.in_channels
                        and ops.conv3d_k1_chain_supported(m12.conv.in_channels, m12.conv.out_channels, m6.conv.out_channels)):
                    w1, s1, h1 = m12.prepared()
                    w2, s2, h2 = m6.prepared()
                    low = torch.empty((last_output.shape[0], m6.conv.out_channels) + tuple(last_output.shape[2:]), device=last_output.device,
                                      dtype=last_output.dtype)
                    ops.conv3d_k1_chain(last_output, w1, s1, h1, m12.relu, w2, s2, h2, False, low)
                    y = torch.empty((last_output.shape[0], m6.conv.out_channels) + half, device=last_output.device, dtype=last_output.dtype)
                    ops.trilinear3d_act(low, half, True, m6.relu, y, 0)
                    return up_last3(y)
                y12 = m12(last_output)
            y = self.last_6_3d[i6](y12, resample_to=(d // 2, h // 2, w // 2))
            return up_last3(y)
        raise ValueError("MatchingNet: feature height must be a multiple of 4 (input H a multiple of 12)")

    def cost_volume(self, left_fea, right_fea):
        if ag.needs_grad(left_fea, right_fea):
            return ag.CostVolFn.apply(left_fea, right_fea, self.maxdisp)
        return ops.costvol(left_fea, right_fea, self.maxdisp)

    def forward(self, left_fea, right_fea, task_arch=None):
        if task_arch is None:
            task_arch = self.arch_init
        if left_fea.shape != right_fea.shape or left_fea.dim() != 4:
            raise ValueError("MatchingNet: left/right features must both be [B, C, h, w]")
        cost = self.matching(None, task_arch, None, features=(left_fea, right_fea))
        return self.disp(cost)
```

### rag_amd/ops.py

```python
from __future__ import annotations

import ctypes
import os
from typing import Optional, Sequence

import torch

from ._lib import K1RSpec, TailSpec, check, load_library

F32, BF16, F32X3 = 0, 1, 2
_DT = {torch.float32: F32, torch.bfloat16: BF16}

_CONV_PRECISIONS = ("f16x3", "fp32")
_PRECISION_ALIASES = {"bf16x3": "f16x3", "split": "f16x3"}
_conv_precision = "fp32" if os.environ.get("RAGMI_X3", "1").strip() == "0" else "f16x3"


def set_conv_precision(precision: str) -> str:
    global _conv_precision
    precision = _PRECISION_ALIASES.get(precision, precision)
    if precision not in _CONV_PRECISIONS:
        raise ValueError(f"conv precision must be one of {_CONV_PRECISIONS}, got {precision!r}")
    old, _conv_precision = _conv_precision, precision
    return old


def get_conv_precision() -> str:
    return _conv_precision


class conv_precision:

    def __init__(self, precision: str):
        self.precision = precision

    def __enter__(self):
        self.old = set_conv_precision(self.precision)
        return self

    def __exit__(self, *exc):
        set_conv_precision(self.old)
        return False


def _conv_dt(dt: int) -> int:
    return F32X3 if (dt == F32 and _conv_precision == "f16x3") else dt


def _stream() -> int:
    return torch.cuda.current_stream().cuda_stream


def _need_gpu(*ts: torch.Tensor) -> None:
    for t in ts:
        if t is None:
            continue
        if not t.is_cuda:
            raise RuntimeError("rag_amd ops run on the MI355X only (got a CPU tensor); there is no CPU fallback")
        if t.dtype != torch.float32:
            raise RuntimeError(f"rag_amd ops: dtype {t.dtype} not built for this argument (fp32 only)")


def _act(*ts: torch.Tensor) -> int:
    dt = None
    for t in ts:
        if t is None:
            continue
        if not t.is_cuda:
            raise RuntimeError("rag_amd ops run on the MI355X only (got a CPU tensor); there is no CPU fallback")
        if t.dtype not in _DT:
            raise RuntimeError(f"rag_amd ops: activation dtype {t.dtype} not built (float32 or bfloat16)")
        if dt is not None and t.dtype != dt:
            raise RuntimeError("rag_amd ops: activation tensors of one call must share a dtype")
        dt = t.dtype
    return _DT[dt]


def _act_with_tails(x, out, res, tails) -> int:
    dt = _act(x, out, res, *[t.out for t in (tails or []) if not (t.down and x.dtype == torch.bfloat16 and t.out.dtype == torch.float32)])
    for t in (tails or []):
        if not t.out.is_cuda:
            raise RuntimeError("rag_amd ops run on the MI355X only (got a CPU tensor); there is no CPU fallback")
    return dt


def _planes(t: torch.Tensor) -> int:
    inner = 1
    for i in range(t.dim() - 1, 0, -1):
        if t.shape[i] != 1 and t.stride(i) != inner:
            raise RuntimeError(f"rag_amd ops: planes must be dense N-C-D-H-W, got strides {t.stride()} for {tuple(t.shape)}")
        inner *= t.shape[i]
    return int(t.stride(0))


def _i32_array(vals: Optional[Sequence[int]]):
    if vals is None:
        return None
    return (ctypes.c_int32 * len(vals))(*[int(v) for v in vals])


CONV_X_G4, CONV_Y_G4, TAIL_G4 = 2, 4, 4
TAIL_ROWS = 16
_STEM_TAIL_ROWS = [os.environ.get("RAGMI_STEM_TAIL_ROWS", "1") != "0"]


def set_stem_tail_rows(enabled: bool) -> None:
    _STEM_TAIL_ROWS[0] = bool(enabled)


def stem_tail_rows_enabled() -> bool:
    return _STEM_TAIL_ROWS[0]


TAIL_F32, OUT_F32 = 8, 0x100
_BF16_DEEP_F32 = [os.environ.get("RAGMI_BF16_DEEP_F32", "1") != "0"]


def set_bf16_deep_fp32(enabled: bool) -> None:
    _BF16_DEEP_F32[0] = bool(enabled)


def bf16_deep_fp32_enabled() -> bool:
    return _BF16_DEEP_F32[0]


_BF16_HEAD_F32 = [os.environ.get("RAGMI_BF16_HEAD_F32", "1") != "0"]


def set_bf16_head_fp32(enabled: bool) -> None:
    _BF16_HEAD_F32[0] = bool(enabled)


def bf16_head_fp32_enabled() -> bool:
    return _BF16_HEAD_F32[0]


_BF16_DEEP_RATIO = [int(os.environ.get("RAGMI_BF16_DEEP_RATIO", "8"))]


def bf16_deep_fp32_ratio() -> int:
    return _BF16_DEEP_RATIO[0]
_G4 = [os.environ.get("RAGMI_G4", "1") != "0"]


_FUSE_STEMS = [os.environ.get("RAGMI_FUSE_STEMS", "1") != "0"]


def set_stem_fusion(enabled: bool) -> None:
    _FUSE_STEMS[0] = bool(enabled)


def stem_fusion_enabled() -> bool:
    return _FUSE_STEMS[0]


def set_g4(enabled: bool) -> None:
    _G4[0] = bool(enabled)


def g4_enabled() -> bool:
    return _G4[0]



def to_g4(t: torch.Tensor) -> torch.Tensor:
    B, C = t.shape[:2]
    sp = tuple(t.shape[2:])
    perm = (0, 1) + tuple(range(3, 3 + len(sp))) + (2,)
    return t.reshape((B, C // 4, 4) + sp).permute(perm).contiguous().view(t.shape)


def from_g4(t: torch.Tensor) -> torch.Tensor:
    B, C = t.shape[:2]
    sp = tuple(t.shape[2:])
    n = len(sp)
    perm = (0, 1, 2 + n) + tuple(range(2, 2 + n))
    return t.reshape((B, C // 4) + sp + (4,)).permute(perm).contiguous().view(t.shape)


def conv3d_k3_g4_caps(cin: int, cout: int, B: int, D: int, H: int, W: int, nset: int = 1, ntail: int = 0, ndown: int = 0,
                      dtype: torch.dtype = torch.float32) -> int:
    return int(load_library().ragmi_conv3d_k3_g4_caps(cin, cout, B, D, H, W, nset, ntail, ndown, _conv_dt(_DT[dtype])))


class Tail:

    def __init__(self, weight2d: torch.Tensor, scale: Optional[torch.Tensor], shift: Optional[torch.Tensor], relu: bool,
                 out: torch.Tensor, out_ch0: int, down: bool = False, g4: bool = False):
        _need_gpu(weight2d, scale, shift)
        _act(out)
        for t in (weight2d, scale, shift):
            if t is not None and not t.is_contiguous():
                raise ValueError("Tail: weight / scale / shift must be contiguous (row slices of contiguous tensors are)")
        self.weight2d, self.scale, self.shift, self.relu, self.out, self.out_ch0 = weight2d, scale, shift, relu, out, out_ch0
        self.down = bool(down)
        self.g4 = bool(g4)
        if self.g4 and (self.down or weight2d.shape[0] != 4 or out_ch0 % 4 or not out.is_contiguous()):
            raise ValueError("Tail: a G4 destination takes a full-resolution tail of 4 channels at a group-aligned channel of a contiguous tensor")

    def spec(self) -> TailSpec:
        p = lambda t: t.data_ptr() if t is not None else None
        f32 = TAIL_F32 if (self.down and self.out.dtype == torch.float32) else 0
        return TailSpec(p(self.weight2d), p(self.scale), p(self.shift), int(self.relu) | (2 if self.down else 0) | (TAIL_G4 if self.g4 else 0) | f32, self.out.data_ptr(),
                        _planes(self.out), int(self.out_ch0), int(self.weight2d.shape[0]))


def _tail_array(tails: Optional[Sequence["Tail"]]):
    if not tails:
        return 0, None
    if sum(1 for t in tails if not t.down) > 2 or sum(1 for t in tails if t.down) > 2:
        raise ValueError("at most two full-resolution and two down-sampling tails per conv launch")
    arr = (TailSpec * len(tails))(*[t.spec() for t in tails])
    return len(tails), arr


def costvol(left_fea: torch.Tensor, right_fea: torch.Tensor, maxdisp: int, out: Optional[torch.Tensor] = None) -> torch.Tensor:
    dt = _act(left_fea, right_fea, out)
    if left_fea.shape != right_fea.shape or left_fea.dim() != 4:
        raise ValueError("costvol: left/right features must both be [B, C, h, w]")
    left_fea, right_fea = left_fea.contiguous(), right_fea.contiguous()
    B, C, h, w = left_fea.shape
    d = int(maxdisp / 3)
    if out is None:
        out = torch.empty((B, 2 * C, d, h, w), device=left_fea.device, dtype=left_fea.dtype)
    check(load_library().ragmi_costvol_fwd(left_fea.data_ptr(), right_fea.data_ptr(), out.data_ptr(),
                                           B, C, d, h, w, dt, _stream()), "costvol")
    return out


def costvol_stem_prepare(weight: torch.Tensor) -> torch.Tensor:
    _need_gpu(weight)
    Cout, C2 = weight.shape[:2]
    if tuple(weight.shape[2:]) != (3, 3, 3) or C2 % 2:
        raise ValueError("costvol_stem_prepare: weight must be [Cout, 2C, 3, 3, 3]")
    lib = load_library()
    out = torch.empty((lib.ragmi_costvol_stem_weights_elems(C2 // 2, Cout),), device=weight.device, dtype=torch.float32)
    check(lib.ragmi_costvol_stem_prepare(weight.detach().contiguous().data_ptr(), out.data_ptr(), C2 // 2, Cout, _stream()),
          "costvol_stem_prepare")
    return out


def costvol_stem(left_fea: torch.Tensor, right_fea: torch.Tensor, maxdisp: int, variants: torch.Tensor, cout: int,
                 scale: Optional[torch.Tensor], shift: Optional[torch.Tensor], relu: bool, out: Optional[torch.Tensor] = None,
                 tails: Optional[Sequence[Tail]] = None, out_g4: bool = False) -> torch.Tensor:
    _need_gpu(variants, scale, shift)
    dt = _act(left_fea, right_fea, out, *[t.out for t in (tails or [])])
    if left_fea.shape != right_fea.shape or left_fea.dim() != 4:
        raise ValueError("costvol_stem: left/right features must both be [B, C, h, w]")
    left_fea, right_fea = left_fea.contiguous(), right_fea.contiguous()
    B, C, h, w = left_fea.shape
    d = int(maxdisp / 3)
    if out is None:
        out = torch.empty((B, cout, d, h, w), device=left_fea.device, dtype=left_fea.dtype)
    if tuple(out.shape[2:]) != (d, h, w) or out.shape[1] < cout or out.shape[0] != B:
        raise ValueError("costvol_stem: out must be [B, >=Cout, maxdisp/3, h, w]")
    lib = load_library()
    ws = torch.empty((lib.ragmi_costvol_stem_workspace_elems(B, C, cout, d, h, w),), device=left_fea.device, dtype=torch.float32)
    ntail, tarr = _tail_array(tails)
    p = lambda t: t.data_ptr() if t is not None else None
    if out_g4 and (not out.is_contiguous() or out.shape[1] != cout):
        raise ValueError("costvol_stem: a G4 output is a contiguous [B, Cout, ...] buffer")
    check(lib.ragmi_costvol_stem_fwd(left_fea.data_ptr(), right_fea.data_ptr(), variants.data_ptr(), p(scale), p(shift), int(relu) | (CONV_Y_G4 if out_g4 else 0),
                                     out.data_ptr(), _planes(out), ws.data_ptr(), B, C, cout, d, h, w, ntail, tarr, _conv_dt(dt), _stream()),
          "costvol_stem")
    return out


def costvol_stem_conv3d_supported(C: int, cmid: int, cout: int, B: int, d: int, h: int, w: int, ntail: int = 0,
                                  dtype: torch.dtype = torch.float32) -> bool:
    return bool(load_library().ragmi_costvol_stem_conv3d_supported(C, cmid, cout, B, d, h, w, ntail, _conv_dt(_DT[dtype])))


def costvol_stem_conv3d(left_fea: torch.Tensor, right_fea: torch.Tensor, maxdisp: int, variants: torch.Tensor, cmid: int,
                        scale0: Optional[torch.Tensor], shift0: Optional[torch.Tensor], relu0: bool, tails0: Optional[Sequence[Tail]],
                        packed: torch.Tensor, cout: int, scale: Optional[torch.Tensor], shift: Optional[torch.Tensor], relu: bool,
                        out: Optional[torch.Tensor], out_group_ch: Optional[Sequence[int]] = None,
                        tails: Optional[Sequence[Tail]] = None, store_main: bool = True, tail0_rows: bool = False) -> Optional[torch.Tensor]:
    _need_gpu(variants, scale0, shift0, packed, scale, shift)
    dt = _act(left_fea, right_fea, out, *[t.out for t in (tails0 or [])], *[t.out for t in (tails or [])])
    if left_fea.shape != right_fea.shape or left_fea.dim() != 4:
        raise ValueError("costvol_stem_conv3d: left/right features must both be [B, C, h, w]")
    if out is None and store_main:
        raise ValueError("costvol_stem_conv3d: store_main needs an output buffer")
    left_fea, right_fea = left_fea.contiguous(), right_fea.contiguous()
    B, C, h, w = left_fea.shape
    d = int(maxdisp / 3)
    lib = load_library()
    ws = torch.empty((lib.ragmi_costvol_stem_workspace_elems(B, C, cmid, d, h, w),), device=left_fea.device, dtype=torch.float32)
    n0, t0 = _tail_array(tails0)
    n1, t1 = _tail_array(tails)
    if tail0_rows:
        if n0 != 1 or cout != 12:
            raise ValueError("costvol_stem_conv3d: tail0_rows takes exactly one tail behind a 12-channel stem3d1")
        t0[0].relu |= TAIL_ROWS
    p = lambda t: t.data_ptr() if t is not None else None
    check(lib.ragmi_costvol_stem_conv3d_fwd(left_fea.data_ptr(), right_fea.data_ptr(), variants.data_ptr(), p(scale0), p(shift0), int(relu0),
                                            ws.data_ptr(), n0, t0, packed.data_ptr(), p(scale), p(shift), int(relu),
                                            p(out), _planes(out) if out is not None else 0, _i32_array(out_group_ch), int(store_main), n1, t1,
                                            B, C, cmid, cout, d, h, w, _conv_dt(dt), _stream()), "costvol_stem_conv3d")
    return out


def stem_tail_rows_weight(weight: torch.Tensor, tail_weight2d: torch.Tensor) -> torch.Tensor:
    if weight.dim() != 5 or weight.shape[0] != 12 or tuple(tail_weight2d.shape) != (4, weight.shape[1]):
        raise ValueError("stem_tail_rows_weight: a [12, Cin, 3, 3, 3] weight and a [4, Cin] tail")
    rows = torch.zeros((4,) + tuple(weight.shape[1:]), device=weight.device, dtype=weight.dtype)
    rows[:, :, 1, 1, 1] = tail_weight2d
    return torch.cat([weight, rows], dim=0).contiguous()


def conv3d_k3_pack(weight: torch.Tensor, transpose: bool = False, for_current_precision: bool = False) -> torch.Tensor:
    _need_gpu(weight)
    planar = weight.dim() == 4
    if tuple(weight.shape[2:]) != ((3, 3) if planar else (3, 3, 3)):
        raise ValueError("conv3d_k3_pack: weight must be [Cout, Cin, 3, 3, 3] (or [Cout, Cin, 3, 3])")
    Cout, Cin = (weight.shape[1], weight.shape[0]) if transpose else (weight.shape[0], weight.shape[1])
    lib = load_library()
    n = lib.ragmi_conv3d_k3_packed_elems(Cout, Cin)
    packed = torch.empty((n,), device=weight.device, dtype=torch.float32)
    w = weight.detach().contiguous()
    if for_current_precision:
        check(lib.ragmi_conv3d_k3_pack_for(w.data_ptr(), packed.data_ptr(), Cout, Cin, int(transpose), int(planar), _conv_dt(F32), _stream()),
              "conv3d_k3_pack_for")
    else:
        check(lib.ragmi_conv3d_k3_pack_ex(w.data_ptr(), packed.data_ptr(), Cout, Cin, int(transpose), int(planar), F32, _stream()),
              "conv3d_k3_pack")
    return packed


def conv3d_k3_plan(cout: int, B: int, D: int, H: int, W: int, nset: int = 1):
    log_tx, rows = ctypes.c_int32(), ctypes.c_int32()
    groups = (ctypes.c_int32 * 16)()
    n = load_library().ragmi_conv3d_k3_plan(cout, B, D, H, W, nset, ctypes.byref(log_tx), ctypes.byref(rows), groups, 16)
    if n < 0:
        check(n, "conv3d_k3_plan")
    return log_tx.value, rows.value, [groups[i] for i in range(n)]


def packed_groups(cout: int) -> int:
    return (cout + 3) // 4


def conv3d_k3(x: torch.Tensor, packed: torch.Tensor, cout: int, scale: Optional[torch.Tensor], shift: Optional[torch.Tensor],
              relu: bool, out: torch.Tensor, out_group_ch: Optional[Sequence[int]] = None,
              res: Optional[torch.Tensor] = None, res_group_ch: Optional[Sequence[int]] = None,
              tails: Optional[Sequence[Tail]] = None, store_main: bool = True, x_g4: bool = False) -> torch.Tensor:
    if x_g4 and not x.is_contiguous():
        raise ValueError("conv3d_k3: a G4 input is a contiguous buffer")
    _need_gpu(packed, scale, shift)
    dt = _act_with_tails(x, out, res, tails)
    B, Cin, D, H, W = x.shape
    xb = _planes(x)
    yb = _planes(out)
    rb = _planes(res) if res is not None else 0
    ng = packed_groups(cout)
    if out_group_ch is not None and len(out_group_ch) != ng:
        raise ValueError("conv3d_k3: out_group_ch needs one entry per group of 4 output channels")
    if res is not None and res_group_ch is None:
        res_group_ch = out_group_ch
    if tuple(out.shape[2:]) != (D, H, W) or out.shape[0] != B:
        raise ValueError("conv3d_k3: out must be [B, C, D, H, W] of the input's spatial size")
    max_ch = max(out_group_ch) + 4 if out_group_ch is not None else cout
    if max_ch > out.shape[1] + (3 if cout % 4 else 0):
        raise ValueError("conv3d_k3: destination channels exceed the output buffer")
    ntail, tarr = _tail_array(tails)
    check(load_library().ragmi_conv3d_k3_fwd_ex(
        x.data_ptr(), xb, packed.data_ptr(),
        scale.data_ptr() if scale is not None else None, shift.data_ptr() if shift is not None else None, int(relu) | (CONV_X_G4 if x_g4 else 0),
        out.data_ptr(), yb, _i32_array(out_group_ch),
        res.data_ptr() if res is not None else None, rb, _i32_array(res_group_ch),
        B, Cin, cout, D, H, W, int(store_main), ntail, tarr, _conv_dt(dt), _stream()), "conv3d_k3")
    return out


def conv3d_k3_small(x: torch.Tensor, weight: torch.Tensor, scale, shift, relu: bool, out: torch.Tensor, out_ch0: int = 0,
                    res: Optional[torch.Tensor] = None, res_ch0: int = 0) -> torch.Tensor:
    _need_gpu(weight, scale, shift)
    dt = _act(x, res)
    ydt = _act(out)
    if ydt != dt and not (dt == BF16 and ydt == F32):
        raise RuntimeError("conv3d_k3_small: out must have x's dtype (or be float32 when x is bfloat16)")
    B, Cin, D, H, W = x.shape
    cout = weight.shape[0]
    w = weight.detach().contiguous()
    if out_ch0 + cout > out.shape[1] or tuple(out.shape[2:]) != (D, H, W):
        raise ValueError("conv3d_k3_small: output buffer too small / wrong spatial size")
    ptr = lambda t: t.data_ptr() if t is not None else None
    check(load_library().ragmi_conv3d_k3_small_fwd_ex(
        x.data_ptr(), _planes(x), w.data_ptr(), ptr(scale), ptr(shift), int(relu), out.data_ptr(), _planes(out), out_ch0,
        ptr(res), _planes(res) if res is not None else 0, res_ch0, B, Cin, cout, D, H, W, dt, ydt, _stream()), "conv3d_k3_small")
    return out


def conv3d_k3_dual(x: torch.Tensor, cin_a: int, packed_a: torch.Tensor, scale_a, shift_a,
                   packed_b: torch.Tensor, scale_b, shift_b, cout: int, relu: bool, out: torch.Tensor,
                   out_group_ch: Optional[Sequence[int]] = None, res: Optional[torch.Tensor] = None,
                   res_group_ch: Optional[Sequence[int]] = None, tails: Optional[Sequence[Tail]] = None,
                   store_main: bool = True, x_g4: bool = False) -> torch.Tensor:
    if x_g4 and not x.is_contiguous():
        raise ValueError("conv3d_k3_dual: a G4 input is a contiguous buffer")
    _need_gpu(packed_a, packed_b, scale_a, shift_a, scale_b, shift_b)
    dt = _act_with_tails(x, out, res, tails)
    B, Cx, D, H, W = x.shape
    ng = packed_groups(cout)
    if out_group_ch is not None and len(out_group_ch) != ng:
        raise ValueError("conv3d_k3_dual: out_group_ch needs one entry per group of 4 output channels")
    if res is not None and res_group_ch is None:
        res_group_ch = out_group_ch
    if tuple(out.shape[2:]) != (D, H, W) or out.shape[0] != B or not 0 < cin_a < Cx:
        raise ValueError("conv3d_k3_dual: bad shapes")
    ptr = lambda t: t.data_ptr() if t is not None else None
    ntail, tarr = _tail_array(tails)
    check(load_library().ragmi_conv3d_k3_dual_fwd_ex(
        x.data_ptr(), _planes(x), cin_a, packed_a.data_ptr(), ptr(scale_a), ptr(shift_a),
        Cx - cin_a, packed_b.data_ptr(), ptr(scale_b), ptr(shift_b), int(relu) | (CONV_X_G4 if x_g4 else 0),
        out.data_ptr(), _planes(out), _i32_array(out_group_ch),
        ptr(res), _planes(res) if res is not None else 0, _i32_array(res_group_ch),
        B, cout, D, H, W, int(store_main), ntail, tarr, _conv_dt(dt), _stream()), "conv3d_k3_dual")
    return out


def conv3d_k1(x: torch.Tensor, weight2d: torch.Tensor, scale: Optional[torch.Tensor], shift: Optional[torch.Tensor],
              relu: bool, out: torch.Tensor, out_ch0: int = 0, transposed: bool = False) -> torch.Tensor:
    _need_gpu(weight2d, scale, shift)
    dt = _act(x, out)
    B, Cin = x.shape[:2]
    Cout = weight2d.shape[1 if transposed else 0]
    if not weight2d.is_contiguous() or weight2d.shape[0 if transposed else 1] != Cin:
        raise ValueError("conv3d_k1: weight must be contiguous [Cout, Cin] (or [Cin, Cout] with transposed=True)")
    dhw = 1
    for s in x.shape[2:]:
        dhw *= s
    if out_ch0 + Cout > out.shape[1] or tuple(out.shape[2:]) != tuple(x.shape[2:]):
        raise ValueError("conv3d_k1: output buffer too small / wrong spatial size")
    check(load_library().ragmi_conv3d_k1_fwd_ex(
        x.data_ptr(), _planes(x), weight2d.data_ptr(), int(transposed),
        scale.data_ptr() if scale is not None else None, shift.data_ptr() if shift is not None else None, int(relu),
        out.data_ptr(), _planes(out), out_ch0, B, Cin, Cout, dhw, dt, _stream()), "conv3d_k1")
    return out


_CHAIN_K1 = [os.environ.get("RAGMI_CHAIN_K1", "1") != "0"]


def set_chain_k1(enabled: bool) -> None:
    _CHAIN_K1[0] = bool(enabled)


def chain_k1_enabled() -> bool:
    return _CHAIN_K1[0]


def conv3d_k1_chain_supported(cin: int, cmid: int, cout: int) -> bool:
    return bool(load_library().ragmi_conv3d_k1_chain_supported(int(cin), int(cmid), int(cout)))


def conv3d_k1_chain(x: torch.Tensor, w1: torch.Tensor, scale1, shift1, relu1: bool, w2: torch.Tensor, scale2, shift2, relu2: bool,
                    out: torch.Tensor, out_ch0: int = 0) -> torch.Tensor:
    _need_gpu(w1, scale1, shift1, w2, scale2, shift2)
    dt = _act(x, out)
    B, Cin = x.shape[:2]
    Cmid, Cout = w1.shape[0], w2.shape[0]
    if not (w1.is_contiguous() and w2.is_contiguous()) or w1.shape[1] != Cin or w2.shape[1] != Cmid:
        raise ValueError("conv3d_k1_chain: weights must be contiguous [Cmid, Cin] and [Cout, Cmid]")
    dhw = 1
    for sdim in x.shape[2:]:
        dhw *= sdim
    if out_ch0 + Cout > out.shape[1] or tuple(out.shape[2:]) != tuple(x.shape[2:]):
        raise ValueError("conv3d_k1_chain: output buffer too small / wrong spatial size")
    p = lambda t: t.data_ptr() if t is not None else None
    check(load_library().ragmi_conv3d_k1_chain_fwd(x.data_ptr(), _planes(x), w1.data_ptr(), p(scale1), p(shift1), int(relu1), Cmid,
                                                   w2.data_ptr(), p(scale2), p(shift2), int(relu2), out.data_ptr(), _planes(out), out_ch0,
                                                   B, Cin, Cout, dhw, dt, _stream()), "conv3d_k1_chain")
    return out


def conv3d_k1_resample(x: torch.Tensor, size: Sequence[int], align_corners: bool, weight2d: torch.Tensor,
                       scale: Optional[torch.Tensor], shift: Optional[torch.Tensor], relu: bool, out: torch.Tensor,
                       out_ch0: int = 0) -> torch.Tensor:
    _need_gpu(weight2d, scale, shift)
    if x.dtype == torch.bfloat16 and out.dtype == torch.float32:
        dt = _act(x) | OUT_F32
        _act(out)
    else:
        dt = _act(x, out)
    B, Cin, Di, Hi, Wi = x.shape
    Do, Ho, Wo = [int(v) for v in size]
    Cout = weight2d.shape[0]
    if out_ch0 + Cout > out.shape[1] or tuple(out.shape[2:]) != (Do, Ho, Wo):
        raise ValueError("conv3d_k1_resample: output buffer too small / wrong spatial size")
    check(load_library().ragmi_conv3d_k1_resample_fwd(
        x.data_ptr(), _planes(x), Di, Hi, Wi, weight2d.data_ptr(),
        scale.data_ptr() if scale is not None else None, shift.data_ptr() if shift is not None else None, int(relu),
        out.data_ptr(), _planes(out), out_ch0, B, Cin, Cout, Do, Ho, Wo, int(bool(align_corners)), dt, _stream()),
        "conv3d_k1_resample")
    return out


def conv3d_k1_resample_pair(specs, size: Sequence[int], out: torch.Tensor) -> torch.Tensor:
    arr = []
    dt = _act(out, *[s[0] for s in specs])
    for (x, w2d, scale, shift, relu, ch0) in specs:
        _need_gpu(w2d, scale, shift)
        p = lambda t: t.data_ptr() if t is not None else None
        arr.append(K1RSpec(x.data_ptr(), _planes(x), x.shape[2], x.shape[3], x.shape[4], w2d.data_ptr(), p(scale), p(shift),
                           int(relu), int(ch0), x.shape[1], w2d.shape[0]))
        if ch0 + w2d.shape[0] > out.shape[1]:
            raise ValueError("conv3d_k1_resample_pair: output buffer too small")
    Do, Ho, Wo = [int(v) for v in size]
    if tuple(out.shape[2:]) != (Do, Ho, Wo):
        raise ValueError("conv3d_k1_resample_pair: wrong output spatial size")
    check(load_library().ragmi_conv3d_k1_resample_pair_fwd(ctypes.byref(arr[0]), ctypes.byref(arr[1]), out.data_ptr(), _planes(out),
                                                           out.shape[0], Do, Ho, Wo, 1, dt, _stream()), "conv3d_k1_resample_pair")
    return out


def conv3d_k1_resample_multi(specs, size: Sequence[int]) -> None:
    if not 1 <= len(specs) <= 3:
        raise ValueError("conv3d_k1_resample_multi: 1..3 specs")
    dt = _act(*[s[0] for s in specs], *[s[5] for s in specs])
    Do, Ho, Wo = [int(v) for v in size]
    arr, ys, bs = [], [], []
    p = lambda t: t.data_ptr() if t is not None else None
    for (x, w2d, scale, shift, relu, out, ch0) in specs:
        _need_gpu(w2d, scale, shift)
        if tuple(out.shape[2:]) != (Do, Ho, Wo) or ch0 + w2d.shape[0] > out.shape[1] or out.shape[0] != x.shape[0]:
            raise ValueError("conv3d_k1_resample_multi: output buffer too small / wrong size")
        arr.append(K1RSpec(x.data_ptr(), _planes(x), x.shape[2], x.shape[3], x.shape[4], w2d.data_ptr(), p(scale), p(shift),
                           int(relu), int(ch0), x.shape[1], w2d.shape[0]))
        ys.append(out.data_ptr())
        bs.append(_planes(out))
    n = len(arr)
    from ._lib import c_k1r_p
    parr = (c_k1r_p * n)(*[ctypes.pointer(a) for a in arr])
    check(load_library().ragmi_conv3d_k1_resample_multi_fwd(parr, (ctypes.c_void_p * n)(*ys), (ctypes.c_int64 * n)(*bs), n, specs[0][0].shape[0],
                                                            Do, Ho, Wo, 1, dt, _stream()), "conv3d_k1_resample_multi")


def cell2d_supported(C: int, cin0: int, cin1: int, cout: int, H: int, W: int, dtype=torch.float32) -> bool:
    if dtype != torch.float32:
        return False
    return bool(load_library().ragmi_cell2d_supported(int(C), int(cin0), int(cin1), int(cout), int(H), int(W), _conv_dt(_DT[dtype])))


def cell2d(s0: torch.Tensor, pre0, s1: torch.Tensor, pre1, C: int, packed_a: torch.Tensor, scale_a, shift_a,
           packed_b: torch.Tensor, scale_b, shift_b, cout: int, relu: bool, out: torch.Tensor,
           out_group_ch: Optional[Sequence[int]] = None) -> torch.Tensor:
    from ._lib import Cell2dIn
    _need_gpu(packed_a, packed_b, scale_a, shift_a, scale_b, shift_b)
    dt = _act(s0, s1, out)
    H, W = int(out.shape[-2]), int(out.shape[-1])
    B = out.shape[0]
    p = lambda t: t.data_ptr() if t is not None else None
    ins = []
    for x, (w2d, sc, sh, rl) in ((s0, pre0), (s1, pre1)):
        _need_gpu(w2d, sc, sh)
        if x.shape[0] != B or w2d.shape != (C, x.shape[1]) or not w2d.is_contiguous():
            raise ValueError("cell2d: input / 1x1 weight shapes do not match")
        ins.append(Cell2dIn(x.data_ptr(), _planes(x), x.shape[1], x.shape[-2], x.shape[-1], w2d.data_ptr(), p(sc), p(sh), int(bool(rl))))
    groups = list(out_group_ch) if out_group_ch is not None else [4 * g for g in range(cout // 4)]
    if len(groups) != cout // 4 or cout % 4 or any(g < 0 or g + 4 > out.shape[1] for g in groups):
        raise ValueError("cell2d: bad destination channel groups")
    garr = (ctypes.c_int32 * len(groups))(*groups)
    check(load_library().ragmi_cell2d_fwd(ctypes.byref(ins[0]), ctypes.byref(ins[1]), int(C), packed_a.data_ptr(), p(scale_a), p(shift_a),
                                          packed_b.data_ptr(), p(scale_b), p(shift_b), int(bool(relu)), out.data_ptr(), _planes(out), garr,
                                          B, int(cout), H, W, _conv_dt(dt), _stream()), "cell2d")
    return out


def conv2d_k3_strided(x: torch.Tensor, weight: torch.Tensor, scale, shift, relu: bool, stride: int) -> torch.Tensor:
    _need_gpu(weight, scale, shift)
    dt = _act(x)
    x = x.contiguous()
    B, Cin, H, W = x.shape
    Cout = weight.shape[0]
    Ho, Wo = (H - 1) // stride + 1, (W - 1) // stride + 1
    out = torch.empty((B, Cout, Ho, Wo), device=x.device, dtype=x.dtype)
    w = weight.detach().contiguous()
    p = lambda t: t.data_ptr() if t is not None else None
    check(load_library().ragmi_conv2d_k3_strided_fwd(x.data_ptr(), w.data_ptr(), p(scale), p(shift), int(relu), out.data_ptr(),
                                                     B, Cin, Cout, H, W, int(stride), dt, _stream()), "conv2d_k3_strided")
    return out


def down2_tail_supported(D: int, H: int, W: int) -> bool:
    return bool(load_library().ragmi_down2_tail_supported(int(D), int(H), int(W)))


def upconv3d_c1_supported(cin: int, di: int, hi: int, wi: int) -> bool:
    return bool(load_library().ragmi_upconv3d_c1_supported(int(cin), int(di), int(hi), int(wi)))


def upconv3d_c1(x: torch.Tensor, weight: torch.Tensor, scale: Optional[torch.Tensor], shift: Optional[torch.Tensor], relu: bool,
                out: Optional[torch.Tensor] = None, out_ch0: int = 0, out_dtype: Optional[torch.dtype] = None) -> torch.Tensor:
    _need_gpu(weight, scale, shift)
    dt = _act(x)
    B, Cin, Di, Hi, Wi = x.shape
    if tuple(weight.shape) != (1, Cin, 3, 3, 3):
        raise ValueError("upconv3d_c1: weight must be [1, Cin, 3, 3, 3]")
    if out is None:
        out = torch.empty((B, 1, 2 * Di, 2 * Hi, 2 * Wi), device=x.device, dtype=out_dtype or x.dtype)
    ydt = _act(out)
    if tuple(out.shape[2:]) != (2 * Di, 2 * Hi, 2 * Wi) or out.shape[0] != B or out_ch0 >= out.shape[1]:
        raise ValueError("upconv3d_c1: out must be [B, >= out_ch0 + 1, 2Di, 2Hi, 2Wi]")
    ptr = lambda t: t.data_ptr() if t is not None else None
    check(load_library().ragmi_upconv3d_c1_fwd(x.data_ptr(), _planes(x), weight.detach().contiguous().data_ptr(), ptr(scale), ptr(shift),
                                               int(relu), out.data_ptr(), _planes(out), int(out_ch0), B, Cin, Di, Hi, Wi, dt, ydt, _stream()),
          "upconv3d_c1")
    return out


def trilinear3d(x: torch.Tensor, size: Sequence[int], align_corners: bool) -> torch.Tensor:
    dt = _act(x)
    x = x.contiguous()
    B, C, Di, Hi, Wi = x.shape
    Do, Ho, Wo = [int(s) for s in size]
    out = torch.empty((B, C, Do, Ho, Wo), device=x.device, dtype=x.dtype)
    check(load_library().ragmi_trilinear3d_fwd(x.data_ptr(), out.data_ptr(), B, C, Di, Hi, Wi, Do, Ho, Wo,
                                               int(bool(align_corners)), dt, _stream()), "trilinear3d")
    return out


def trilinear3d_act(x: torch.Tensor, size: Sequence[int], align_corners: bool, relu: bool, out: torch.Tensor,
                    out_ch0: int = 0) -> torch.Tensor:
    dt = _act(x, out)
    B, C, Di, Hi, Wi = x.shape
    Do, Ho, Wo = [int(s) for s in size]
    if out_ch0 + C > out.shape[1] or tuple(out.shape[2:]) != (Do, Ho, Wo):
        raise ValueError("trilinear3d_act: output buffer too small / wrong spatial size")
    check(load_library().ragmi_trilinear3d_act_fwd(x.data_ptr(), _planes(x), out.data_ptr(), _planes(out), out_ch0, int(relu), B, C,
                                                   Di, Hi, Wi, Do, Ho, Wo, int(bool(align_corners)), dt, _stream()), "trilinear3d_act")
    return out


def add(a: torch.Tensor, a_ch0: int, b: torch.Tensor, b_ch0: int, out: torch.Tensor, out_ch0: int, channels: int) -> torch.Tensor:
    dt = _act(a, b, out)
    dhw = 1
    for s in a.shape[2:]:
        dhw *= s
    check(load_library().ragmi_add_fwd(a.data_ptr(), _planes(a), a_ch0, b.data_ptr(), _planes(b), b_ch0,
                                       out.data_ptr(), _planes(out), out_ch0, a.shape[0], channels, dhw, dt, _stream()), "add")
    return out


def disp_softargmin(cost: torch.Tensor, maxdisp: int) -> torch.Tensor:
    dt = _act(cost)
    if cost.dim() == 5:
        if cost.shape[1] != 1:
            raise ValueError("disp_softargmin: expected a single-channel cost volume")
        cost = cost[:, 0]
    cost = cost.contiguous()
    B, d, h, w = cost.shape
    out = torch.empty((B, 3 * h, 3 * w), device=cost.device, dtype=torch.float32)
    check(load_library().ragmi_disp_softargmin_fwd(cost.data_ptr(), out.data_ptr(), B, d, h, w, int(maxdisp),
                                                   3 * h, 3 * w, dt, _stream()), "disp_softargmin")
    return out


def disparity_regression(prob: torch.Tensor, maxdisp: int) -> torch.Tensor:
    dt = _act(prob)
    assert prob.is_contiguous()
    B, D, H, W = prob.shape
    if D != maxdisp:
        raise ValueError("disparity_regression: prob.shape[1] must equal maxdisp")
    out = torch.empty((B, H, W), device=prob.device, dtype=torch.float32)
    check(load_library().ragmi_disparity_regression_fwd(prob.data_ptr(), out.data_ptr(), B, D, H, W, dt, _stream()),
          "disparity_regression")
    return out


def _vol(t: torch.Tensor) -> int:
    n = 1
    for s in t.shape[2:]:
        n *= s
    return n


def bn_train_stats(x: torch.Tensor, gamma: torch.Tensor, beta: torch.Tensor, running_mean: Optional[torch.Tensor],
                   running_var: Optional[torch.Tensor], num_batches_tracked: Optional[torch.Tensor], momentum: float, eps: float):
    _need_gpu(x, gamma, beta, running_mean, running_var)
    B, C = x.shape[:2]
    lib = load_library()
    ws = torch.empty((lib.ragmi_bn_workspace_elems(B, C, _vol(x)),), device=x.device, dtype=torch.float32)
    out = torch.empty((4, C), device=x.device, dtype=torch.float32)
    if num_batches_tracked is not None and num_batches_tracked.dtype != torch.int64:
        raise RuntimeError("bn_train_stats: num_batches_tracked must be int64")
    p = lambda t: t.data_ptr() if t is not None else None
    check(lib.ragmi_bn_train_stats_fwd(x.data_ptr(), _planes(x), B, C, _vol(x), gamma.data_ptr(), beta.data_ptr(), p(running_mean),
                                       p(running_var), p(num_batches_tracked), float(momentum), float(eps), ws.data_ptr(),
                                       out[0].data_ptr(), out[1].data_ptr(), out[2].data_ptr(), out[3].data_ptr(), _stream()),
          "bn_train_stats")
    return out


def bn_train_act(x: torch.Tensor, gamma: torch.Tensor, beta: torch.Tensor, running_mean: Optional[torch.Tensor],
                 running_var: Optional[torch.Tensor], num_batches_tracked: Optional[torch.Tensor], momentum: float, eps: float, relu: bool,
                 res: Optional[torch.Tensor] = None):
    _need_gpu(x, gamma, beta, running_mean, running_var, res)
    B, C = x.shape[:2]
    if res is not None and tuple(res.shape) != tuple(x.shape):
        raise ValueError("bn_train_act: res must have the shape of x")
    lib = load_library()
    ws = torch.empty((lib.ragmi_bn_workspace_elems(B, C, _vol(x)),), device=x.device, dtype=torch.float32)
    st = torch.empty((4, C), device=x.device, dtype=torch.float32)
    y = torch.empty(x.shape, device=x.device, dtype=torch.float32)
    if num_batches_tracked is not None and num_batches_tracked.dtype != torch.int64:
        raise RuntimeError("bn_train_act: num_batches_tracked must be int64")
    p = lambda t: t.data_ptr() if t is not None else None
    check(lib.ragmi_bn_train_act_fwd(x.data_ptr(), _planes(x), B, C, _vol(x), gamma.data_ptr(), beta.data_ptr(), p(running_mean),
                                     p(running_var), p(num_batches_tracked), float(momentum), float(eps), int(relu), ws.data_ptr(),
                                     st[0].data_ptr(), st[1].data_ptr(), st[2].data_ptr(), st[3].data_ptr(), y.data_ptr(), _planes(y), 0,
                                     p(res), _planes(res) if res is not None else 0, 0, _stream()), "bn_train_act")
    return y, st


def bn_act_bwd(dy: torch.Tensor, x: torch.Tensor, scale, shift, relu: bool, mean, invstd, training: bool,
               out: Optional[torch.Tensor] = None, dgamma_into: Optional[torch.Tensor] = None, dbeta_into: Optional[torch.Tensor] = None):
    _need_gpu(dy, x, scale, shift, mean, invstd, out, dgamma_into, dbeta_into)
    B, C = x.shape[:2]
    lib = load_library()
    ws = torch.empty((lib.ragmi_bn_workspace_elems(B, C, _vol(x)),), device=x.device, dtype=torch.float32)
    dx = out if out is not None else torch.empty(x.shape, device=x.device, dtype=torch.float32)
    direct = dgamma_into is not None and dbeta_into is not None
    gb = None if direct else torch.empty((2, C), device=x.device, dtype=torch.float32)
    dg, db = (dgamma_into, dbeta_into) if direct else (gb[0], gb[1])
    check(lib.ragmi_bn_act_bwd(dy.data_ptr(), _planes(dy), 0, x.data_ptr(), _planes(x), scale.data_ptr(), shift.data_ptr(), int(relu),
                               mean.data_ptr(), invstd.data_ptr(), int(training), B, C, _vol(x), ws.data_ptr(), dx.data_ptr(), _planes(dx),
                               dg.data_ptr(), db.data_ptr(), int(direct), _stream()), "bn_act_bwd")
    return dx, (None if direct else gb[0]), (None if direct else gb[1])


def bn_act(x: torch.Tensor, scale: torch.Tensor, shift: torch.Tensor, relu: bool, out: Optional[torch.Tensor] = None,
           out_ch0: int = 0, res: Optional[torch.Tensor] = None, res_ch0: int = 0) -> torch.Tensor:
    _need_gpu(x, scale, shift, out, res)
    B, C = x.shape[:2]
    if out is None:
        out = torch.empty_like(x)
    check(load_library().ragmi_bn_act_fwd(x.data_ptr(), _planes(x), scale.data_ptr(), shift.data_ptr(), int(relu),
                                          res.data_ptr() if res is not None else None, _planes(res) if res is not None else 0, res_ch0,
                                          out.data_ptr(), _planes(out), out_ch0, B, C, _vol(x), _stream()), "bn_act")
    return out


def bn_act_bwd_coeffs(dy: torch.Tensor, dy_ch0: int, x: torch.Tensor, scale, shift, relu: bool, mean, invstd, training: bool,
                      dgamma_into: Optional[torch.Tensor] = None, dbeta_into: Optional[torch.Tensor] = None):
    _need_gpu(dy, x, scale, shift, mean, invstd, dgamma_into, dbeta_into)
    B, C = x.shape[:2]
    lib = load_library()
    ws = torch.empty((lib.ragmi_bn_workspace_elems(B, C, _vol(x)),), device=x.device, dtype=torch.float32)
    out = torch.empty((5, C), device=x.device, dtype=torch.float32)
    direct = dgamma_into is not None or dbeta_into is not None
    if direct and (dgamma_into is None or dbeta_into is None):
        raise ValueError("bn_act_bwd_coeffs: pass both dgamma_into and dbeta_into, or neither")
    dg, db = (dgamma_into, dbeta_into) if direct else (out[3], out[4])
    check(lib.ragmi_bn_act_bwd_coeffs(dy.data_ptr(), _planes(dy), dy_ch0, x.data_ptr(), _planes(x), scale.data_ptr(), shift.data_ptr(),
                                      int(relu), mean.data_ptr(), invstd.data_ptr(), int(training), B, C, _vol(x), ws.data_ptr(),
                                      out[0].data_ptr(), out[1].data_ptr(), out[2].data_ptr(), dg.data_ptr(), db.data_ptr(), int(direct),
                                      _stream()), "bn_act_bwd_coeffs")
    return out


def bn_act_bwd_apply(dy: torch.Tensor, dy_ch0: int, x: torch.Tensor, scale, shift, relu: bool, c1, c2, c3,
                     out: Optional[torch.Tensor] = None) -> torch.Tensor:
    _need_gpu(dy, x, scale, shift, c1, c2, c3, out)
    B, C = x.shape[:2]
    dx = out if out is not None else torch.empty(x.shape, device=x.device, dtype=torch.float32)
    check(load_library().ragmi_bn_act_bwd_apply(dy.data_ptr(), _planes(dy), dy_ch0, x.data_ptr(), _planes(x), scale.data_ptr(),
                                                shift.data_ptr(), int(relu), c1.data_ptr(), c2.data_ptr(), c3.data_ptr(), dx.data_ptr(),
                                                _planes(dx), B, C, _vol(x), _stream()), "bn_act_bwd_apply")
    return dx


def conv3d_k3_wgrad(x: torch.Tensor, g: torch.Tensor, cout: int, g_ch0: int = 0, into: Optional[Sequence[torch.Tensor]] = None,
                    planar2d: bool = False):
    _need_gpu(x, g, *(into or []))
    B, Cin, D, H, W = x.shape
    lib = load_library()
    n = lib.ragmi_conv3d_k3_wgrad_workspace_elems(B, Cin, cout, D, H, W)
    if n < 0:
        check(-2, "conv3d_k3_wgrad_workspace_elems")
    ws = torch.empty((n,), device=x.device, dtype=torch.float32)
    if into is None:
        dw = torch.empty((cout, Cin, 3, 3) if planar2d else (cout, Cin, 3, 3, 3), device=x.device, dtype=torch.float32)
        dsts, acc = [dw], 0
    else:
        want = (cout // len(into), Cin, 3, 3) if planar2d else (cout // len(into), Cin, 3, 3, 3)
        if any(tuple(t.shape) != want or not t.is_contiguous() for t in into):
            raise ValueError(f"conv3d_k3_wgrad: every destination must be a contiguous {want} tensor")
        dw, dsts, acc = None, list(into), 1
    arr = (ctypes.c_void_p * len(dsts))(*[t.data_ptr() for t in dsts])
    check(lib.ragmi_conv3d_k3_wgrad(x.data_ptr(), _planes(x), g.data_ptr(), _planes(g), g_ch0, arr, len(dsts), acc, int(planar2d),
                                    ws.data_ptr(), B, Cin, cout, D, H, W, _stream()), "conv3d_k3_wgrad")
    return dw


def conv3d_k1_wgrad(x: torch.Tensor, g: torch.Tensor, cout: int, g_ch0: int = 0, into: Optional[torch.Tensor] = None) -> torch.Tensor:
    _need_gpu(x, g, into)
    B, Cin = x.shape[:2]
    if into is not None and (into.numel() != cout * Cin or not into.is_contiguous()):
        raise ValueError("conv3d_k1_wgrad: destination must be contiguous with cout*Cin elements")
    dw = into if into is not None else torch.zeros((cout, Cin), device=x.device, dtype=torch.float32)
    check(load_library().ragmi_conv3d_k1_wgrad(x.data_ptr(), _planes(x), g.data_ptr(), _planes(g), g_ch0, dw.data_ptr(), B, Cin, cout,
                                               _vol(x), _stream()), "conv3d_k1_wgrad")
    return dw


def trilinear3d_bwd(dy: torch.Tensor, in_size: Sequence[int], align_corners: bool) -> torch.Tensor:
    _need_gpu(dy)
    dy = dy.contiguous()
    B, C, Do, Ho, Wo = dy.shape
    Di, Hi, Wi = [int(v) for v in in_size]
    dx = torch.empty((B, C, Di, Hi, Wi), device=dy.device, dtype=torch.float32)
    check(load_library().ragmi_trilinear3d_bwd(dy.data_ptr(), dx.data_ptr(), B, C, Di, Hi, Wi, Do, Ho, Wo, int(bool(align_corners)),
                                               _stream()), "trilinear3d_bwd")
    return dx


def costvol_bwd(dcost: torch.Tensor):
    _need_gpu(dcost)
    dcost = dcost.contiguous()
    B, C2, d, h, w = dcost.shape
    dl = torch.empty((B, C2 // 2, h, w), device=dcost.device, dtype=torch.float32)
    dr = torch.empty_like(dl)
    check(load_library().ragmi_costvol_bwd(dcost.data_ptr(), dl.data_ptr(), dr.data_ptr(), B, C2 // 2, d, h, w, _stream()), "costvol_bwd")
    return dl, dr


def disp_softargmin_bwd(cost: torch.Tensor, dout: torch.Tensor, maxdisp: int) -> torch.Tensor:
    _need_gpu(cost, dout)
    shape = cost.shape
    c4 = (cost[:, 0] if cost.dim() == 5 else cost).contiguous()
    B, d, h, w = c4.shape
    dout = dout.contiguous()
    dc = torch.zeros_like(c4)
    check(load_library().ragmi_disp_softargmin_bwd(c4.data_ptr(), dout.data_ptr(), dc.data_ptr(), B, d, h, w, int(maxdisp), 3 * h, 3 * w,
                                                   _stream()), "disp_softargmin_bwd")
    return dc.reshape(shape)


def conv2d_k3_strided_dgrad(g: torch.Tensor, weight: torch.Tensor, in_hw: Sequence[int], stride: int) -> torch.Tensor:
    _need_gpu(g, weight)
    g, w = g.contiguous(), weight.detach().contiguous()
    B, Cout = g.shape[:2]
    Cin, (H, W) = w.shape[1], [int(v) for v in in_hw]
    if tuple(g.shape[2:]) != ((H - 1) // stride + 1, (W - 1) // stride + 1):
        raise ValueError("conv2d_k3_strided_dgrad: gradient size does not match the input size / stride")
    dx = torch.empty((B, Cin, H, W), device=g.device, dtype=torch.float32)
    check(load_library().ragmi_conv2d_k3_strided_dgrad(g.data_ptr(), w.data_ptr(), dx.data_ptr(), B, Cin, Cout, H, W, int(stride),
                                                       _stream()), "conv2d_k3_strided_dgrad")
    return dx


def conv2d_k3_strided_wgrad(x: torch.Tensor, g: torch.Tensor, stride: int, into: Optional[torch.Tensor] = None) -> torch.Tensor:
    _need_gpu(x, g, into)
    x, g = x.contiguous(), g.contiguous()
    B, Cin, H, W = x.shape
    Cout = g.shape[1]
    if into is not None and (tuple(into.shape) != (Cout, Cin, 3, 3) or not into.is_contiguous()):
        raise ValueError("conv2d_k3_strided_wgrad: destination must be a contiguous [Cout, Cin, 3, 3] tensor")
    dw = into if into is not None else torch.zeros((Cout, Cin, 3, 3), device=x.device, dtype=torch.float32)
    check(load_library().ragmi_conv2d_k3_strided_wgrad(x.data_ptr(), g.data_ptr(), dw.data_ptr(), B, Cin, Cout, H, W, int(stride),
                                                       _stream()), "conv2d_k3_strided_wgrad")
    return dw


def disparity_regression_bwd(dout: torch.Tensor, maxdisp: int) -> torch.Tensor:
    _need_gpu(dout)
    dout = dout.contiguous()
    B, H, W = dout.shape
    dp = torch.empty((B, int(maxdisp), H, W), device=dout.device, dtype=torch.float32)
    check(load_library().ragmi_disparity_regression_bwd(dout.data_ptr(), dp.data_ptr(), B, int(maxdisp), H, W, _stream()),
          "disparity_regression_bwd")
    return dp



def conv3d_k3_uses_x3(cin: int, cout: int, B: int, D: int, H: int, W: int, nset: int = 1, has_res: bool = False, ntail: int = 0,
                      dtype: torch.dtype = torch.float32) -> bool:
    return bool(load_library().ragmi_conv3d_k3_uses_x3(cin, cout, B, D, H, W, nset, int(has_res), ntail, _conv_dt(_DT[dtype])))


def sgd_clip_step(param: torch.Tensor, grad: torch.Tensor, buf: torch.Tensor, lr: float, momentum: float, weight_decay: float,
                  max_norm: float, first_step: bool, workspace: Optional[torch.Tensor] = None,
                  norm_out: Optional[torch.Tensor] = None) -> torch.Tensor:
    _need_gpu(param, grad, buf, workspace, norm_out)
    for t in (param, grad, buf):
        if t.dim() != 1 or t.dtype != torch.float32 or not t.is_contiguous() or t.numel() != param.numel():
            raise RuntimeError("sgd_clip_step: param / grad / momentum buffers must be flat contiguous fp32 of equal length")
    lib = load_library()
    if workspace is None:
        workspace = torch.empty((lib.ragmi_sgd_workspace_bytes() // 4,), device=param.device, dtype=torch.float32)
    if norm_out is None:
        norm_out = torch.empty((1,), device=param.device, dtype=torch.float32)
    check(lib.ragmi_sgd_clip_step(param.data_ptr(), grad.data_ptr(), buf.data_ptr(), param.numel(), float(lr), float(momentum),
                                  float(weight_decay), float(max_norm), int(first_step), workspace.data_ptr(), norm_out.data_ptr(),
                                  _stream()), "sgd_clip_step")
    return norm_out


def depth_head_supported(cin: int, hi: int, wi: int, h: int, w: int, scale: int = 3, dtype=torch.float32) -> bool:
    return bool(load_library().ragmi_depth_head_supported(cin, hi, wi, h, w, scale, _DT.get(dtype, -1)))


def depth_head(y: torch.Tensor, w3: torch.Tensor, w1: torch.Tensor, b1: torch.Tensor, size: Sequence[int], scale: int = 3,
               max_depth: float = 80.0) -> torch.Tensor:
    for t in (y, w3, w1, b1):
        if not t.is_cuda:
            raise RuntimeError("rag_amd ops run on the MI355X only (got a CPU tensor); there is no CPU fallback")
    if y.dim() != 4 or w3.numel() != 9 * y.shape[1] or w1.numel() != 9 or b1.numel() != 1:
        raise ValueError("depth_head: y must be [B, Cin, Hi, Wi], w3 [1, Cin, 3, 3], w1 [1, 1, 3, 3], b1 [1]")
    dtypes = {y.dtype, w3.dtype, w1.dtype, b1.dtype}
    dt = _DT.get(y.dtype, -1) if len(dtypes) == 1 else -1
    y, w3, w1, b1 = y.contiguous(), w3.contiguous(), w1.contiguous(), b1.contiguous()
    B, C, Hi, Wi = y.shape
    H, W = (int(v) for v in size)
    out = torch.empty((B, scale * H, scale * W), device=y.device, dtype=torch.float32)
    check(load_library().ragmi_depth_head_fwd(y.data_ptr(), w3.data_ptr(), w1.data_ptr(), b1.data_ptr(), out.data_ptr(), B, C, Hi, Wi,
                                              H, W, int(scale), float(max_depth), dt, _stream()), "depth_head")
    return out


def depth_metrics(est: torch.Tensor, gt: torch.Tensor, variance_focus: float = 0.85) -> torch.Tensor:
    for t in (est, gt):
        if not t.is_cuda:
            raise RuntimeError("rag_amd ops run on the MI355X only (got a CPU tensor); there is no CPU fallback")
    if est.shape != gt.shape or est.numel() == 0:
        raise ValueError("depth_metrics: est and gt must have the same non-empty shape")
    dt = _DT.get(est.dtype, -1) if est.dtype == gt.dtype else -1
    est, gt = est.contiguous(), gt.contiguous()
    lib = load_library()
    n = est.numel()
    ws = torch.empty((max(2, lib.ragmi_depth_metrics_workspace_elems(n)),), device=est.device, dtype=torch.float32)
    out = torch.empty((10,), device=est.device, dtype=torch.float32)
    check(lib.ragmi_depth_metrics_fwd(est.data_ptr(), gt.data_ptr(), n, float(variance_focus), ws.data_ptr(), out.data_ptr(), dt,
                                      _stream()), "depth_metrics")
    return out


def depth_head_bwd(y: torch.Tensor, w3: torch.Tensor, w1: torch.Tensor, b1: torch.Tensor, d_out: torch.Tensor, size: Sequence[int],
                   scale: int = 3, max_depth: float = 80.0, dw3_into: Optional[torch.Tensor] = None,
                   dw1_into: Optional[torch.Tensor] = None, db1_into: Optional[torch.Tensor] = None):
    _need_gpu(y, w3, w1, b1, d_out)
    if y.dim() != 4 or w3.numel() != 9 * y.shape[1] or w1.numel() != 9 or b1.numel() != 1:
        raise ValueError("depth_head_bwd: y must be [B, Cin, Hi, Wi], w3 [1, Cin, 3, 3], w1 [1, 1, 3, 3], b1 [1]")
    B, C, Hi, Wi = y.shape
    H, W = (int(v) for v in size)
    if tuple(d_out.shape) != (B, scale * H, scale * W):
        raise ValueError(f"depth_head_bwd: d_out must be [{B}, {scale * H}, {scale * W}], got {tuple(d_out.shape)}")
    dtypes = {y.dtype, w3.dtype, w1.dtype, b1.dtype, d_out.dtype}
    dt = _DT.get(y.dtype, -1) if len(dtypes) == 1 else -1
    y, w3, w1, b1, d_out = y.contiguous(), w3.contiguous(), w1.contiguous(), b1.contiguous(), d_out.contiguous()
    outs, acc = [], 0
    for bit, (w, into) in enumerate(((w3, dw3_into), (w1, dw1_into), (b1, db1_into))):
        if into is not None:
            if into.numel() != w.numel() or into.dtype != torch.float32 or not into.is_contiguous() or into.device != w.device:
                raise ValueError("depth_head_bwd: an *_into target must be a contiguous fp32 tensor of the weight's size")
            outs.append(into)
            acc |= 1 << bit
        else:
            outs.append(torch.empty(w.shape, device=w.device, dtype=torch.float32))
    dy = torch.empty((B, C, Hi, Wi), device=y.device, dtype=torch.float32)
    lib = load_library()
    ws = torch.empty((max(2, lib.ragmi_depth_head_bwd_workspace_elems(B, C, H, W)),), device=y.device, dtype=torch.float32)
    check(lib.ragmi_depth_head_bwd(y.data_ptr(), w3.data_ptr(), w1.data_ptr(), b1.data_ptr(), d_out.data_ptr(), dy.data_ptr(),
                                   outs[0].data_ptr(), outs[1].data_ptr(), outs[2].data_ptr(), acc, ws.data_ptr(), B, C, Hi, Wi, H, W,
                                   int(scale), float(max_depth), dt, _stream()), "depth_head_bwd")
    return dy, outs[0], outs[1], outs[2]


def silog_loss(est: torch.Tensor, gt: torch.Tensor, variance_focus: float = 0.85):
    for t in (est, gt):
        if not t.is_cuda:
            raise RuntimeError("rag_amd ops run on the MI355X only (got a CPU tensor); there is no CPU fallback")
    if est.shape != gt.shape or est.numel() == 0:
        raise ValueError("silog_loss: est and gt must have the same non-empty shape")
    dt = _DT.get(est.dtype, -1) if est.dtype == gt.dtype else -1
    est, gt = est.contiguous(), gt.contiguous()
    lib = load_library()
    n = est.numel()
    ws = torch.empty((max(2, lib.ragmi_silog_loss_workspace_elems(n)),), device=est.device, dtype=torch.float32)
    out = torch.empty((1,), device=est.device, dtype=torch.float32)
    saved = torch.empty((3,), device=est.device, dtype=torch.float64)
    check(lib.ragmi_silog_loss_fwd(est.data_ptr(), gt.data_ptr(), n, float(variance_focus), ws.data_ptr(), out.data_ptr(),
                                   saved.data_ptr(), dt, _stream()), "silog_loss")
    return out, saved


def silog_loss_bwd(est: torch.Tensor, gt: torch.Tensor, saved: torch.Tensor, gout: torch.Tensor, variance_focus: float = 0.85):
    _need_gpu(gout)
    dt = _DT.get(est.dtype, -1) if est.dtype == gt.dtype else -1
    est, gt, gout = est.contiguous(), gt.contiguous(), gout.reshape(-1)[:1].contiguous()
    grad = torch.empty(est.shape, device=est.device, dtype=torch.float32)
    check(load_library().ragmi_silog_loss_bwd(est.data_ptr(), gt.data_ptr(), est.numel(), float(variance_focus), saved.data_ptr(),
                                              gout.data_ptr(), grad.data_ptr(), dt, _stream()), "silog_loss_bwd")
    return grad
```

Before: 1079 disparity maps/s.

## Add split-channel k1 resample kernel and fused k1 conv-upsample paths

Adds a k1 resample kernel that stages interpolated inputs in LDS and splits channels across four thread groups. It is chosen by default for small output volumes. Also adds a fused kernel that runs a 1x1x1 conv (optionally chained) on the low-resolution tile and then trilinearly upsamples from LDS, optionally alongside a same-size 1x1x1 conv in the same launch. The fused cell and head paths sit behind flags that are off by default. The aim is to cut the per-voxel channel-loop cost on small resample launches and, when enabled, to avoid computing convs at high resolution and writing intermediates.

```diff
diff --git a/include/rag_amd.h b/include/rag_amd.h
--- a/include/rag_amd.h
+++ b/include/rag_amd.h
@@ -125,6 +125,40 @@
                                       int B, int Do, int Ho, int Wo, int align_corners, int dtype, void* stream);
 int ragmi_conv3d_k1_resample_multi_fwd(const ragmi_k1r_t* const* specs, void* const* ys, const int64_t* y_bstrides, int n, int B,
                                        int Do, int Ho, int Wo, int align_corners, int dtype, void* stream);
+int ragmi_conv3d_k1_resample_set_form(int form);
+int ragmi_conv3d_k1_resample_split_chosen(int n, const int* Cin, const int* Cout, int Do, int Ho, int Wo);
+
+typedef struct {
+  const void* x;
+  int64_t x_bstride;
+  int32_t Cin, Di, Hi, Wi;
+  const void* weight1;
+  const void* scale1;
+  const void* shift1;
+  int32_t relu1;
+  int32_t Cmid;
+  const void* weight2;
+  const void* scale2;
+  const void* shift2;
+  int32_t Cout;
+  int32_t relu;
+  void* y;
+  int64_t y_bstride;
+  int32_t y_ch0;
+  int32_t Do, Ho, Wo;
+  const void* xs;
+  int64_t xs_bstride;
+  int32_t Cin_s, Cout_s;
+  const void* weight_s;
+  const void* scale_s;
+  const void* shift_s;
+  int32_t relu_s;
+  int32_t ys_ch0;
+  void* ys;
+  int64_t ys_bstride;
+} ragmi_k1up_t;
+int ragmi_conv3d_k1_up_supported(int Cin, int Cmid, int Cout, int Di, int Hi, int Wi, int Do, int Ho, int Wo, int Cin_s, int Cout_s);
+int ragmi_conv3d_k1_up_fwd(const ragmi_k1up_t* d, int B, int dtype, void* stream);
 
 typedef struct {
   const void* x;
diff --git a/rag_amd/_lib.py b/rag_amd/_lib.py
--- a/rag_amd/_lib.py
+++ b/rag_amd/_lib.py
@@ -24,6 +24,17 @@
 
 
 c_k1r_p = ctypes.POINTER(K1RSpec)
+
+
+class K1UpSpec(ctypes.Structure):
+    _i = ctypes.c_int32
+    _fields_ = [("x", c_void_p), ("x_bstride", c_int64), ("Cin", _i), ("Di", _i), ("Hi", _i), ("Wi", _i),
+                ("weight1", c_void_p), ("scale1", c_void_p), ("shift1", c_void_p), ("relu1", _i), ("Cmid", _i),
+                ("weight2", c_void_p), ("scale2", c_void_p), ("shift2", c_void_p), ("Cout", _i), ("relu", _i),
+                ("y", c_void_p), ("y_bstride", c_int64), ("y_ch0", _i), ("Do", _i), ("Ho", _i), ("Wo", _i),
+                ("xs", c_void_p), ("xs_bstride", c_int64), ("Cin_s", _i), ("Cout_s", _i),
+                ("weight_s", c_void_p), ("scale_s", c_void_p), ("shift_s", c_void_p), ("relu_s", _i), ("ys_ch0", _i),
+                ("ys", c_void_p), ("ys_bstride", c_int64)]
 
 
 class Cell2dIn(ctypes.Structure):
@@ -81,6 +92,10 @@
     "ragmi_conv3d_k1_resample_pair_fwd": (c_int, [c_k1r_p, c_k1r_p, c_void_p, c_int64, c_int, c_int, c_int, c_int, c_int, c_int, c_void_p]),
     "ragmi_conv3d_k1_resample_multi_fwd": (c_int, [ctypes.POINTER(c_k1r_p), ctypes.POINTER(c_void_p), ctypes.POINTER(c_int64), c_int, c_int,
                                                    c_int, c_int, c_int, c_int, c_int, c_void_p]),
+    "ragmi_conv3d_k1_resample_set_form": (c_int, [c_int]),
+    "ragmi_conv3d_k1_resample_split_chosen": (c_int, [c_int, c_int32_p, c_int32_p, c_int, c_int, c_int]),
+    "ragmi_conv3d_k1_up_supported": (c_int, [c_int] * 11),
+    "ragmi_conv3d_k1_up_fwd": (c_int, [ctypes.POINTER(K1UpSpec), c_int, c_int, c_void_p]),
     "ragmi_down2_tail_supported": (c_int, [c_int, c_int, c_int]),
     "ragmi_cell2d_supported": (c_int, [c_int] * 7),
     "ragmi_cell2d_fwd": (c_int, [c_cell2d_p, c_cell2d_p, c_int, c_void_p, c_void_p, c_void_p, c_void_p, c_void_p, c_void_p, c_int,
diff --git a/rag_amd/csrc/pointwise.hip b/rag_amd/csrc/pointwise.hip
--- a/rag_amd/csrc/pointwise.hip
+++ b/rag_amd/csrc/pointwise.hip
@@ -1,4 +1,5 @@
 #include <algorithm>
+#include <atomic>
 
 #include "common.h"
 
@@ -255,6 +256,130 @@
   }
 }
 
+constexpr int K1S_VOX = 64, K1S_SPLIT = 4, K1S_U = 6, K1S_MAXC = 64;
+
+template <class T>
+__global__ __launch_bounds__(K1S_VOX * K1S_SPLIT) void conv_k1_resample_split_kernel(K1RPair pr) {
+  extern __shared__ __attribute__((aligned(16))) float k1s_lds[];
+  const K1RArgs& r = pr.c[blockIdx.z >= 2 ? 2 : (blockIdx.z == 1 ? 1 : 0)];
+  const K1Args& a = r.k;
+  const int cp = (a.Cout + 3) & ~3;
+  float* const xs = k1s_lds;
+  float* const wl = xs + a.Cin * K1S_VOX;
+  float* const bn = wl + a.Cin * cp;
+  for (int i = threadIdx.x; i < a.Cin * cp; i += K1S_VOX * K1S_SPLIT) {
+    const int ci = i / cp, co = i % cp;
+    wl[i] = co < a.Cout ? a.w[co * a.w_sco + ci * a.w_sci] : 0.f;
+  }
+  for (int i = threadIdx.x; i < cp; i += K1S_VOX * K1S_SPLIT) {
+    const int co = min(i, a.Cout - 1);
+    bn[i] = a.scale ? a.scale[co] : 1.f;
+    bn[cp + i] = a.scale ? a.shift[co] : 0.f;
+  }
+  const int64_t ovol = (int64_t)r.Do * r.Ho * r.Wo;
+  const int v = threadIdx.x % K1S_VOX, q = threadIdx.x / K1S_VOX;
+  const int64_t og = (int64_t)blockIdx.x * K1S_VOX + v;
+  const int64_t o = og < ovol ? og : ovol - 1;
+  const int b = blockIdx.y;
+  const int64_t ivol = (int64_t)r.Di * r.Hi * r.Wi;
+  const T* xp = static_cast<const T*>(a.x) + b * a.x_bstride;
+  if (r.Di == r.Do && r.Hi == r.Ho && r.Wi == r.Wo) {
+    constexpr int UI = 16;
+    for (int c0 = q; c0 < a.Cin; c0 += K1S_SPLIT * UI) {
+      float xv[UI];
+#pragma unroll
+      for (int u = 0; u < UI; ++u) xv[u] = ld(xp + (int64_t)min(c0 + u * K1S_SPLIT, a.Cin - 1) * ivol + o);
+#pragma unroll
+      for (int u = 0; u < UI; ++u)
+        if (c0 + u * K1S_SPLIT < a.Cin) xs[(c0 + u * K1S_SPLIT) * K1S_VOX + v] = xv[u];
+    }
+  } else {
+    const int ox = (int)(o % r.Wo);
+    const int64_t t = o / r.Wo;
+    const int oy = (int)(t % r.Ho), oz = (int)(t / r.Ho);
+    const LinIdx lz = lin_index(oz, r.Di, r.Do, r.sd, r.align);
+    const LinIdx ly = lin_index(oy, r.Hi, r.Ho, r.sh, r.align);
+    const LinIdx lx = lin_index(ox, r.Wi, r.Wo, r.sw, r.align);
+    const int r00 = (lz.i0 * r.Hi + ly.i0) * r.Wi, r01 = (lz.i0 * r.Hi + ly.i1) * r.Wi;
+    const int r10 = (lz.i1 * r.Hi + ly.i0) * r.Wi, r11 = (lz.i1 * r.Hi + ly.i1) * r.Wi;
+    const bool pair = lx.i1 == lx.i0 + 1;
+    for (int c0 = q; c0 < a.Cin; c0 += K1S_SPLIT * K1S_U) {
+      float tap[K1S_U][8];
+#pragma unroll
+      for (int u = 0; u < K1S_U; ++u) {
+        const T* pc = xp + (int64_t)min(c0 + u * K1S_SPLIT, a.Cin - 1) * ivol;
+        if constexpr (std::is_same<T, float>::value) {
+          if (pair) {
+            const K1RF2 q0 = *reinterpret_cast<const K1RF2*>(pc + r00 + lx.i0), q1 = *reinterpret_cast<const K1RF2*>(pc + r01 + lx.i0);
+            const K1RF2 q2 = *reinterpret_cast<const K1RF2*>(pc + r10 + lx.i0), q3 = *reinterpret_cast<const K1RF2*>(pc + r11 + lx.i0);
+            tap[u][0] = q0.a; tap[u][1] = q0.b; tap[u][2] = q1.a; tap[u][3] = q1.b;
+            tap[u][4] = q2.a; tap[u][5] = q2.b; tap[u][6] = q3.a; tap[u][7] = q3.b;
+            continue;
+          }
+        }
+        tap[u][0] = ld(pc + r00 + lx.i0); tap[u][1] = ld(pc + r00 + lx.i1); tap[u][2] = ld(pc + r01 + lx.i0); tap[u][3] = ld(pc + r01 + lx.i1);
+        tap[u][4] = ld(pc + r10 + lx.i0); tap[u][5] = ld(pc + r10 + lx.i1); tap[u][6] = ld(pc + r11 + lx.i0); tap[u][7] = ld(pc + r11 + lx.i1);
+      }
+#pragma unroll
+      for (int u = 0; u < K1S_U; ++u) {
+        if (c0 + u * K1S_SPLIT >= a.Cin) break;
+        const float a0 = lerp2(ly.w0, lerp2(lx.w0, tap[u][0], lx.w1, tap[u][1]), ly.w1, lerp2(lx.w0, tap[u][2], lx.w1, tap[u][3]));
+        const float a1 = lerp2(ly.w0, lerp2(lx.w0, tap[u][4], lx.w1, tap[u][5]), ly.w1, lerp2(lx.w0, tap[u][6], lx.w1, tap[u][7]));
+        xs[(c0 + u * K1S_SPLIT) * K1S_VOX + v] = lerp2(lz.w0, a0, lz.w1, a1);
+      }
+    }
+  }
+  __syncthreads();
+  const int64_t yo = b * a.y_bstride + o;
+  const bool yf32 = !std::is_same<T, float>::value && a.y_f32;
+  for (int k = q; 4 * k < a.Cout; k += K1S_SPLIT) {
+    float acc[4] = {0.f, 0.f, 0.f, 0.f};
+#pragma unroll 4
+    for (int ci = 0; ci < a.Cin; ++ci) {
+      const float xv = xs[ci * K1S_VOX + v];
+      const float4 w4 = *reinterpret_cast<const float4*>(wl + ci * cp + 4 * k);
+      acc[0] = fmaf(w4.x, xv, acc[0]); acc[1] = fmaf(w4.y, xv, acc[1]); acc[2] = fmaf(w4.z, xv, acc[2]); acc[3] = fmaf(w4.w, xv, acc[3]);
+    }
+    if (og >= ovol) continue;
+#pragma unroll
+    for (int j = 0; j < 4; ++j) {
+      const int co = 4 * k + j;
+      if (co >= a.Cout) break;
+      float val = a.scale ? fmaf(acc[j], bn[co], bn[cp + co]) : acc[j];
+      val = a.relu ? fmaxf(val, 0.f) : val;
+      const int64_t off = yo + (int64_t)(a.y_ch0 + co) * ovol;
+      if (yf32) static_cast<float*>(a.y)[off] = val; else st(static_cast<T*>(a.y) + off, val);
+    }
+  }
+}
+
+static std::atomic<int> k1r_form{1};
+
+static bool k1r_split_built(const K1RArgs* r, int n) {
+  for (int i = 0; i < n; ++i)
+    if (r[i].k.Cin > K1S_MAXC || r[i].k.Cout > K1S_MAXC) return false;
+  return (int64_t)r[0].Do * r[0].Ho * r[0].Wo <= (int64_t)K1S_VOX * 0x7fffffff;
+}
+static bool k1r_split_chosen(const K1RArgs* r, int n) {
+  const int form = k1r_form.load(std::memory_order_relaxed);
+  if (form == 0 || !k1r_split_built(r, n)) return false;
+  return form == 2 || (int64_t)r[0].Do * r[0].Ho * r[0].Wo < 256 * 256 * 2;
+}
+
+template <class T>
+static void launch_k1r_split(const K1RArgs* r, int n, int B, hipStream_t s) {
+  const int64_t ovol = (int64_t)r[0].Do * r[0].Ho * r[0].Wo;
+  K1RPair pr{};
+  size_t lds = 0;
+  for (int i = 0; i < 3; ++i) {
+    pr.c[i] = r[i < n ? i : n - 1];
+    const K1Args& k = pr.c[i].k;
+    lds = std::max(lds, ((size_t)k.Cin * (K1S_VOX + ((k.Cout + 3) & ~3)) + 2 * ((k.Cout + 3) & ~3)) * sizeof(float));
+  }
+  dim3 grid((unsigned)ceil_div(ovol, K1S_VOX), B, (unsigned)n);
+  hipLaunchKernelGGL((conv_k1_resample_split_kernel<T>), grid, dim3(K1S_VOX * K1S_SPLIT), lds, s, pr);
+}
+
 template <class T, int NCO>
 static void launch_k1r_nco(const K1RArgs* r, int n, int B, hipStream_t s) {
   const int64_t ovol = (int64_t)r[0].Do * r[0].Ho * r[0].Wo;
@@ -289,6 +414,10 @@
 
 template <class T>
 static int launch_k1r(const K1RArgs* r, int n, int B, hipStream_t s) {
+  if (k1r_split_chosen(r, n)) {
+    launch_k1r_split<T>(r, n, B, s);
+    return check_launch("conv3d_k1_resample");
+  }
   int cmax = 0;
   for (int i = 0; i < n; ++i) cmax = std::max(cmax, r[i].k.Cout);
   const int64_t threads = (int64_t)B * r[0].Do * r[0].Ho * r[0].Wo * n, want = 256 * 256 * 2;
@@ -363,6 +492,179 @@
     case 12: launch_k1_nco<T, 12, VEC>(a, B, s); break;
     case 8: launch_k1_nco<T, 8, VEC>(a, B, s); break;
     default: launch_k1_nco<T, 4, VEC>(a, B, s); break;
+  }
+}
+
+constexpr int KU_TZ = 4, KU_TY = 8, KU_TX = 32, KU_PZ = 4, KU_PY = 6, KU_PX = 18, KU_PV = KU_PZ * KU_PY * KU_PX, KU_NS = 8;
+
+struct K1UpArgs {
+  K1Args p;
+  const float* w2;
+  const float* scale2;
+  const float* shift2;
+  int Cout, relu;
+  int Di, Hi, Wi, Do, Ho, Wo;
+  float sd, sh, sw;
+  K1Args s;
+  unsigned nblk_up;
+};
+
+template <class T>
+__device__ __forceinline__ float round_as_stored(float v) {
+  if constexpr (!std::is_same<T, float>::value) { const bf16_t r = to_bf16(v); v = ld(&r); }
+  return v;
+}
+
+template <class T, int CMID, int NCO, bool VEC>
+__global__ __launch_bounds__(256) void conv_k1_up_kernel(K1UpArgs u) {
+  extern __shared__ __attribute__((aligned(16))) float ku_lds[];
+  const int tid = threadIdx.x, b = blockIdx.y;
+  if (blockIdx.x >= u.nblk_up) {
+    constexpr int V = VEC ? 4 : 1;
+    const K1Args& a = u.s;
+    for (int i = tid; i < a.Cin * KU_NS; i += 256) {
+      const int ci = i / KU_NS, co = i % KU_NS;
+      ku_lds[i] = co < a.Cout ? a.w[co * a.w_sco + ci * a.w_sci] : 0.f;
+    }
+    float* const bn = ku_lds + a.Cin * KU_NS;
+    if (tid < KU_NS) {
+      const int co = min(tid, a.Cout - 1);
+      bn[tid] = a.scale ? a.scale[co] : 1.f;
+      bn[KU_NS + tid] = a.scale ? a.shift[co] : 0.f;
+    }
+    __syncthreads();
+    const int64_t p = ((int64_t)(blockIdx.x - u.nblk_up) * 256 + tid) * V;
+    if (p >= a.dhw) return;
+    const T* xp = static_cast<const T*>(a.x) + b * a.x_bstride + p;
+    float acc[KU_NS][V];
+#pragma unroll
+    for (int j = 0; j < KU_NS; ++j)
+#pragma unroll
+      for (int k = 0; k < V; ++k) acc[j][k] = 0.f;
+#pragma unroll 8
+    for (int ci = 0; ci < a.Cin; ++ci) {
+      float xv[V];
+      if constexpr (VEC) ld4(xp + (int64_t)ci * a.dhw, xv); else xv[0] = ld(xp + (int64_t)ci * a.dhw);
+      const float4 q0 = *reinterpret_cast<const float4*>(ku_lds + ci * KU_NS), q1 = *reinterpret_cast<const float4*>(ku_lds + ci * KU_NS + 4);
+      const float wv[KU_NS] = {q0.x, q0.y, q0.z, q0.w, q1.x, q1.y, q1.z, q1.w};
+#pragma unroll
+      for (int j = 0; j < KU_NS; ++j)
+#pragma unroll
+        for (int k = 0; k < V; ++k) acc[j][k] = fmaf(wv[j], xv[k], acc[j][k]);
+    }
+    T* yp = static_cast<T*>(a.y) + b * a.y_bstride + p;
+#pragma unroll
+    for (int j = 0; j < KU_NS; ++j) {
+      if (j >= a.Cout) break;
+      float o[V];
+#pragma unroll
+      for (int k = 0; k < V; ++k) {
+        const float v = a.scale ? fmaf(acc[j][k], bn[j], bn[KU_NS + j]) : acc[j][k];
+        o[k] = a.relu ? fmaxf(v, 0.f) : v;
+      }
+      T* dst = yp + (int64_t)(a.y_ch0 + j) * a.dhw;
+      if constexpr (VEC) st4(dst, o); else st(dst, o[0]);
+    }
+    return;
+  }
+
+  const K1Args& a = u.p;
+  constexpr int C1 = CMID > 0 ? CMID : NCO;
+  float* const w1l = ku_lds;
+  float* const w2l = w1l + a.Cin * C1;
+  float* const bn1 = w2l + (CMID > 0 ? CMID * NCO : 0);
+  float* const bn2 = bn1 + 2 * C1;
+  float* const lo = bn2 + (CMID > 0 ? 2 * NCO : 0);
+  for (int i = tid; i < a.Cin * C1; i += 256) {
+    const int ci = i / C1, co = i % C1;
+    w1l[i] = co < a.Cout ? a.w[co * a.Cin + ci] : 0.f;
+  }
+  if (tid < C1) {
+    const int co = min(tid, a.Cout - 1);
+    bn1[tid] = a.scale ? a.scale[co] : 1.f;
+    bn1[C1 + tid] = a.scale ? a.shift[co] : 0.f;
+  }
+  if constexpr (CMID > 0) {
+    for (int i = tid; i < CMID * NCO; i += 256) w2l[i] = u.w2[(i % NCO) * CMID + i / NCO];
+    if (tid < NCO) { bn2[tid] = u.scale2 ? u.scale2[tid] : 1.f; bn2[NCO + tid] = u.scale2 ? u.shift2[tid] : 0.f; }
+  }
+  __syncthreads();
+
+  const int tx = tid % KU_TX, ty = tid / KU_TX;
+  const int nbx = (u.Wo + KU_TX - 1) / KU_TX, nby = (u.Ho + KU_TY - 1) / KU_TY;
+  const int ox0 = ((int)blockIdx.x % nbx) * KU_TX, oy0 = ((int)blockIdx.x / nbx % nby) * KU_TY, oz0 = ((int)blockIdx.x / (nbx * nby)) * KU_TZ;
+  const int pz0 = lin_index(oz0, u.Di, u.Do, u.sd, 1).i0, py0 = lin_index(oy0, u.Hi, u.Ho, u.sh, 1).i0, px0 = lin_index(ox0, u.Wi, u.Wo, u.sw, 1).i0;
+  const int64_t ivol = (int64_t)u.Di * u.Hi * u.Wi, ovol = (int64_t)u.Do * u.Ho * u.Wo;
+  const T* xp = static_cast<const T*>(a.x) + b * a.x_bstride;
+  for (int e = tid; e < KU_PV; e += 256) {
+    const int gz = min(pz0 + e / (KU_PY * KU_PX), u.Di - 1), gy = min(py0 + e / KU_PX % KU_PY, u.Hi - 1), gx = min(px0 + e % KU_PX, u.Wi - 1);
+    const T* xe = xp + ((int64_t)gz * u.Hi + gy) * u.Wi + gx;
+    float h[C1];
+#pragma unroll
+    for (int j = 0; j < C1; ++j) h[j] = 0.f;
+#pragma unroll 8
+    for (int ci = 0; ci < a.Cin; ++ci) {
+      const float xv = ld(xe + (int64_t)ci * ivol);
+#pragma unroll
+      for (int j = 0; j < C1; j += 4) {
+        const float4 q = *reinterpret_cast<const float4*>(w1l + ci * C1 + j);
+        h[j] = fmaf(q.x, xv, h[j]); h[j + 1] = fmaf(q.y, xv, h[j + 1]); h[j + 2] = fmaf(q.z, xv, h[j + 2]); h[j + 3] = fmaf(q.w, xv, h[j + 3]);
+      }
+    }
+#pragma unroll
+    for (int j = 0; j < C1; ++j) {
+      float v = a.scale ? fmaf(h[j], bn1[j], bn1[C1 + j]) : h[j];
+      v = a.relu ? fmaxf(v, 0.f) : v;
+      h[j] = round_as_stored<T>(v);
+    }
+    if constexpr (CMID > 0) {
+      float acc[NCO];
+#pragma unroll
+      for (int k = 0; k < NCO; ++k) acc[k] = 0.f;
+#pragma unroll
+      for (int j = 0; j < CMID; ++j) {
+#pragma unroll
+        for (int k = 0; k < NCO; k += 4) {
+          const float4 q = *reinterpret_cast<const float4*>(w2l + j * NCO + k);
+          acc[k] = fmaf(q.x, h[j], acc[k]); acc[k + 1] = fmaf(q.y, h[j], acc[k + 1]); acc[k + 2] = fmaf(q.z, h[j], acc[k + 2]); acc[k + 3] = fmaf(q.w, h[j], acc[k + 3]);
+        }
+      }
+#pragma unroll
+      for (int k = 0; k < NCO; ++k) lo[k * KU_PV + e] = round_as_stored<T>(u.scale2 ? fmaf(acc[k], bn2[k], bn2[NCO + k]) : acc[k]);
+    } else {
+#pragma unroll
+      for (int k = 0; k < NCO; ++k) lo[k * KU_PV + e] = h[k];
+    }
+  }
+  __syncthreads();
+
+  const int ox = min(ox0 + tx, u.Wo - 1), oy = min(oy0 + ty, u.Ho - 1);
+  const LinIdx ly = lin_index(oy, u.Hi, u.Ho, u.sh, 1);
+  const LinIdx lx = lin_index(ox, u.Wi, u.Wo, u.sw, 1);
+  const int o00 = (ly.i0 - py0) * KU_PX + (lx.i0 - px0), o01 = o00 + (lx.i1 - lx.i0);
+  const int o10 = o00 + (ly.i1 - ly.i0) * KU_PX, o11 = o10 + (lx.i1 - lx.i0);
+  LinIdx lz[KU_TZ];
+#pragma unroll
+  for (int k = 0; k < KU_TZ; ++k) lz[k] = lin_index(min(oz0 + k, u.Do - 1), u.Di, u.Do, u.sd, 1);
+  const bool inside = ox0 + tx < u.Wo && oy0 + ty < u.Ho;
+  T* yp = static_cast<T*>(a.y) + b * a.y_bstride + (int64_t)a.y_ch0 * ovol + ((int64_t)oz0 * u.Ho + oy) * u.Wo + ox;
+  const int64_t zs = (int64_t)u.Ho * u.Wo;
+  for (int c = 0; c < u.Cout; ++c) {
+    const float* t = lo + c * KU_PV;
+    float pl[KU_PZ];
+#pragma unroll
+    for (int p = 0; p < KU_PZ; ++p) {
+      const float* q = t + p * (KU_PY * KU_PX);
+      pl[p] = lerp2(ly.w0, lerp2(lx.w0, q[o00], lx.w1, q[o01]), ly.w1, lerp2(lx.w0, q[o10], lx.w1, q[o11]));
+    }
+#pragma unroll
+    for (int k = 0; k < KU_TZ; ++k) {
+      const int i0 = lz[k].i0 - pz0, i1 = lz[k].i1 - pz0;
+      const float a0 = i0 == 0 ? pl[0] : i0 == 1 ? pl[1] : i0 == 2 ? pl[2] : pl[3];
+      const float a1 = i1 == 0 ? pl[0] : i1 == 1 ? pl[1] : i1 == 2 ? pl[2] : pl[3];
+      const float v = lerp2(lz[k].w0, a0, lz[k].w1, a1);
+      if (inside && oz0 + k < u.Do) st(yp + c * ovol + k * zs, u.relu ? fmaxf(v, 0.f) : v);
+    }
   }
 }
 
@@ -420,6 +722,20 @@
   return check_launch("conv3d_k1_chain");
 }
 
+extern "C" int ragmi_conv3d_k1_resample_set_form(int form) {
+  RAGMI_REQUIRE(form >= 0 && form <= 2, RAGMI_EINVAL, "conv3d_k1_resample_set_form: 0 (one voxel per thread), 1 (by shape) or 2 (channel-split wherever built)");
+  ragmi::k1r_form.store(form, std::memory_order_relaxed);
+  return RAGMI_OK;
+}
+
+extern "C" int ragmi_conv3d_k1_resample_split_chosen(int n, const int* Cin, const int* Cout, int Do, int Ho, int Wo) {
+  using namespace ragmi;
+  if (!Cin || !Cout || n < 1 || n > 3 || Do <= 0 || Ho <= 0 || Wo <= 0) return 0;
+  K1RArgs r[3]{};
+  for (int i = 0; i < n; ++i) { r[i].k.Cin = Cin[i]; r[i].k.Cout = Cout[i]; r[i].Do = Do; r[i].Ho = Ho; r[i].Wo = Wo; }
+  return k1r_split_chosen(r, n) ? 1 : 0;
+}
+
 extern "C" int ragmi_conv3d_k1_resample_fwd(const void* x, int64_t x_bstride, int Di, int Hi, int Wi, const void* weight,
                                             const void* scale, const void* shift, int relu, void* y, int64_t y_bstride,
                                             int y_ch0, int B, int Cin, int Cout, int Do, int Ho, int Wo, int align_corners,
@@ -467,6 +783,66 @@
   }
   return dtype == RAGMI_BF16 ? launch_k1r<bf16_t>(r, n, B, static_cast<hipStream_t>(stream))
                              : launch_k1r<float>(r, n, B, static_cast<hipStream_t>(stream));
+}
+
+extern "C" int ragmi_conv3d_k1_up_supported(int Cin, int Cmid, int Cout, int Di, int Hi, int Wi, int Do, int Ho, int Wo, int Cin_s, int Cout_s) {
+  using namespace ragmi;
+  if (Cin < 1 || Cin > 64 || Di < 1 || Hi < 1 || Wi < 1 || Do < 1 || Ho < 1 || Wo < 1) return 0;
+  if (!((Cmid == 0 && Cout >= 1 && Cout <= KU_NS) || (Cmid == 24 && Cout == 12))) return 0;
+  if (!(Cin_s == 0 || (Cin_s >= 1 && Cin_s <= 64 && Cout_s >= 1 && Cout_s <= KU_NS))) return 0;
+  if (!(lin_scale(Di, Do, 1) <= 0.5f && lin_scale(Hi, Ho, 1) <= 0.5f && lin_scale(Wi, Wo, 1) <= 0.5f)) return 0;
+  const int64_t nblk = ceil_div(Wo, KU_TX) * ceil_div(Ho, KU_TY) * ceil_div(Do, KU_TZ) + ceil_div((int64_t)Do * Ho * Wo, 256);
+  return (nblk < (1ll << 31) && (int64_t)Cin * Di * Hi * Wi < (1ll << 31)) ? 1 : 0;
+}
+
+extern "C" int ragmi_conv3d_k1_up_fwd(const ragmi_k1up_t* d, int B, int dtype, void* stream) {
+  using namespace ragmi;
+  RAGMI_REQUIRE(d && d->x && d->weight1 && d->y, RAGMI_EINVAL, "conv3d_k1_up: null pointer");
+  RAGMI_REQUIRE((d->scale1 == nullptr) == (d->shift1 == nullptr) && (d->scale2 == nullptr) == (d->shift2 == nullptr) &&
+                (d->scale_s == nullptr) == (d->shift_s == nullptr), RAGMI_EINVAL, "conv3d_k1_up: scale/shift must both be given or both NULL");
+  RAGMI_REQUIRE((d->Cmid == 0 || d->weight2) && (!d->xs || (d->weight_s && d->ys)), RAGMI_EINVAL, "conv3d_k1_up: null pointer");
+  RAGMI_REQUIRE(B > 0 && B <= 65535 && d->y_ch0 >= 0 && d->ys_ch0 >= 0, RAGMI_EINVAL, "conv3d_k1_up: bad size");
+  RAGMI_REQUIRE(dtype_ok(dtype), RAGMI_EUNSUPPORTED, "conv3d_k1_up: dtype %d not built", dtype);
+  RAGMI_REQUIRE(ragmi_conv3d_k1_up_supported(d->Cin, d->Cmid, d->Cout, d->Di, d->Hi, d->Wi, d->Do, d->Ho, d->Wo, d->xs ? d->Cin_s : 0, d->Cout_s),
+                RAGMI_EUNSUPPORTED, "conv3d_k1_up: built for Cin <= 64 -> (<= 8 | 24 -> 12) channels up by two or more per axis, and a same-size "
+                "conv of <= 64 -> <= 8 channels; got %d -> %d -> %d, [%d,%d,%d] -> [%d,%d,%d], %d -> %d", d->Cin, d->Cmid, d->Cout, d->Di, d->Hi,
+                d->Wi, d->Do, d->Ho, d->Wo, d->xs ? d->Cin_s : 0, d->Cout_s);
+  const int64_t ovol = (int64_t)d->Do * d->Ho * d->Wo;
+  K1UpArgs u{};
+  const int c1 = d->Cmid > 0 ? d->Cmid : d->Cout;
+  u.p = K1Args{d->x, d->x_bstride, (const float*)d->weight1, (const float*)d->scale1, (const float*)d->shift1, d->y, d->y_bstride, d->y_ch0,
+               d->Cin, c1, 0, (int64_t)d->Di * d->Hi * d->Wi, d->relu1, d->Cin, 1};
+  u.w2 = (const float*)d->weight2; u.scale2 = (const float*)d->scale2; u.shift2 = (const float*)d->shift2;
+  u.Cout = d->Cout; u.relu = d->relu ? 1 : 0;
+  u.Di = d->Di; u.Hi = d->Hi; u.Wi = d->Wi; u.Do = d->Do; u.Ho = d->Ho; u.Wo = d->Wo;
+  u.sd = lin_scale(d->Di, d->Do, 1); u.sh = lin_scale(d->Hi, d->Ho, 1); u.sw = lin_scale(d->Wi, d->Wo, 1);
+  u.nblk_up = (unsigned)(ceil_div(d->Wo, KU_TX) * ceil_div(d->Ho, KU_TY) * ceil_div(d->Do, KU_TZ));
+  bool vec = false;
+  unsigned nblk_s = 0;
+  size_t lds_s = 0;
+  if (d->xs) {
+    u.s = K1Args{d->xs, d->xs_bstride, (const float*)d->weight_s, (const float*)d->scale_s, (const float*)d->shift_s, d->ys, d->ys_bstride,
+                 d->ys_ch0, d->Cin_s, d->Cout_s, 0, ovol, d->relu_s, d->Cin_s, 1};
+    vec = ovol % 4 == 0 && d->xs_bstride % 4 == 0 && d->ys_bstride % 4 == 0 && aligned4(d->xs, dtype) && aligned4(d->ys, dtype) && ovol >= (1 << 18) &&
+          d->Cmid == 0;
+    nblk_s = (unsigned)ceil_div(ceil_div(ovol, vec ? 4 : 1), 256);
+    lds_s = (size_t)(d->Cin_s + 2) * KU_NS * sizeof(float);
+  }
+  const dim3 grid(u.nblk_up + nblk_s, B);
+  hipStream_t s = static_cast<hipStream_t>(stream);
+  auto go = [&](auto tag) {
+    using T = decltype(tag);
+    if (d->Cmid > 0) {
+      const size_t lds = (size_t)(d->Cin * 24 + 24 * 12 + 2 * 24 + 2 * 12 + 12 * KU_PV) * sizeof(float);
+      hipLaunchKernelGGL((conv_k1_up_kernel<T, 24, 12, false>), grid, dim3(256), std::max(lds, lds_s), s, u);
+    } else {
+      const size_t lds = (size_t)(d->Cin * KU_NS + 2 * KU_NS + KU_NS * KU_PV) * sizeof(float);
+      if (vec) hipLaunchKernelGGL((conv_k1_up_kernel<T, 0, KU_NS, true>), grid, dim3(256), std::max(lds, lds_s), s, u);
+      else hipLaunchKernelGGL((conv_k1_up_kernel<T, 0, KU_NS, false>), grid, dim3(256), std::max(lds, lds_s), s, u);
+    }
+  };
+  if (dtype == RAGMI_BF16) go(bf16_t{}); else go(float{});
+  return check_launch("conv3d_k1_up");
 }
 
 extern "C" int ragmi_add_fwd(const void* a, int64_t a_bstride, int a_ch0, const void* b, int64_t b_bstride, int b_ch0,
diff --git a/rag_amd/modules.py b/rag_amd/modules.py
--- a/rag_amd/modules.py
+++ b/rag_amd/modules.py
@@ -414,7 +414,7 @@
         a, b, whole = self.dual_branches(pre_has[0] or s0.shape[1] != C)
         if plan is None:
             plan = _CellPlan(size=self.out_size(s1.shape[2:]), dtype=s1.dtype, has=pre_has, g4=False, dual=whole, store_main=True, tails=False,
-                             shared_pre=False)
+                             shared_pre=False, up_pair=False)
         size = tuple(int(v) for v in plan.size)
         if not pre_has[0] and s0.shape[1] == C and tuple(s0.shape[2:]) != size:
             s0 = ops.trilinear3d(s0, size, True)
@@ -442,7 +442,13 @@
 
         where: List[Tuple[torch.Tensor, int]] = []
         grows = any(s is not None and _volume(size) > _volume(s.shape[2:]) and C <= s.shape[1] for s in (s0, s1))
-        if not pre_has[0] and not pre_has[1] and s0.shape[1] != C and not grows and s0.dtype == s1.dtype == adt:
+        if plan.up_pair:
+            w0, sc0, sh0 = self.pre_preprocess.prepared()
+            w1, sc1, sh1 = self.preprocess.prepared()
+            ops.conv3d_k1_up(s1, w1, sc1, sh1, False, None, size, self.preprocess.relu, pre, C,
+                             same=(s0, w0, sc0, sh0, self.pre_preprocess.relu, pre, 0))
+            where.append((pre, 0))
+        elif not pre_has[0] and not pre_has[1] and s0.shape[1] != C and not grows and s0.dtype == s1.dtype == adt:
             w0, sc0, sh0 = self.pre_preprocess.prepared()
             w1, sc1, sh1 = self.preprocess.prepared()
             ops.conv3d_k1_resample_pair([(s0, w0, sc0, sh0, self.pre_preprocess.relu, 0),
@@ -566,7 +572,7 @@
                 (4, 8, 16, -1), (8, 16, 8, 1), (16, 8, 16, -1), (8, 16, 16, 0))
 
 
-_CellPlan = namedtuple("_CellPlan", "size dtype has g4 dual store_main tails shared_pre")
+_CellPlan = namedtuple("_CellPlan", "size dtype has g4 dual store_main tails shared_pre up_pair")
 _ChainPlan = namedtuple("_ChainPlan", "sizes cdt consumers stored cells stem0_g4 stems_fused stem_tail_rows")
 
 
@@ -647,7 +653,12 @@
                       and _volume(sizes[i]) <= min(_volume(sizes[i - 2]), _volume(sizes[i - 1])))
             if shared:
                 has[i], has[j][0] = [True, True], True
-            plans.append(_CellPlan(sizes[i], cdt[i], tuple(has[i]), g4[i], dual[i], stored[i], tails[i], shared))
+            c = cells[i]
+            up_pair = (ops.cell_up_fusion_enabled() and not any(has[i]) and stored[i - 2] and stored[i - 1] and sizes[i - 2] == sizes[i]
+                       and cout[i - 2] != c.C_out and _volume(sizes[i]) > _volume(sizes[i - 1]) and c.C_out <= cout[i - 1]
+                       and len({cdt[i - 2], cdt[i - 1], cdt[i]}) == 1 and c.pre_preprocess._geometry() == 1 and c.preprocess._geometry() == 1
+                       and ops.conv3d_k1_up_supported(cout[i - 1], 0, c.C_out, sizes[i - 1], sizes[i], cout[i - 2], c.C_out))
+            plans.append(_CellPlan(sizes[i], cdt[i], tuple(has[i]), g4[i], dual[i], stored[i], tails[i], shared, bool(up_pair)))
         for (j, role, _d) in consumers[i]:
             has[j][role] = True
     ro = MappingProxyType
@@ -818,6 +829,11 @@
                         and ops.conv3d_k1_chain_supported(m12.conv.in_channels, m12.conv.out_channels, m6.conv.out_channels)):
                     w1, s1, h1 = m12.prepared()
                     w2, s2, h2 = m6.prepared()
+                    if ops.head_up_fusion_enabled() and ops.conv3d_k1_up_supported(m12.conv.in_channels, m12.conv.out_channels,
+                                                                                   m6.conv.out_channels, last_output.shape[2:], half):
+                        y = torch.empty((last_output.shape[0], m6.conv.out_channels) + half, device=last_output.device, dtype=last_output.dtype)
+                        ops.conv3d_k1_up(last_output, w1, s1, h1, m12.relu, (w2, s2, h2), half, m6.relu, y, 0)
+                        return up_last3(y)
                     low = torch.empty((last_output.shape[0], m6.conv.out_channels) + tuple(last_output.shape[2:]), device=last_output.device,
                                       dtype=last_output.dtype)
                     ops.conv3d_k1_chain(last_output, w1, s1, h1, m12.relu, w2, s2, h2, False, low)
diff --git a/rag_amd/ops.py b/rag_amd/ops.py
--- a/rag_amd/ops.py
+++ b/rag_amd/ops.py
@@ -537,6 +537,81 @@
                                                             Do, Ho, Wo, 1, dt, _stream()), "conv3d_k1_resample_multi")
 
 
+def set_k1_resample_form(form: int) -> None:
+    check(load_library().ragmi_conv3d_k1_resample_set_form(int(form)), "conv3d_k1_resample_set_form")
+
+
+def k1_resample_split_chosen(cins: Sequence[int], couts: Sequence[int], size: Sequence[int]) -> bool:
+    Do, Ho, Wo = [int(v) for v in size]
+    return bool(load_library().ragmi_conv3d_k1_resample_split_chosen(len(cins), _i32_array(cins), _i32_array(couts), Do, Ho, Wo))
+
+
+_FUSE_CELL_UP = [False]
+_FUSE_HEAD_UP = [False]
+
+
+def set_cell_up_fusion(enabled: bool) -> None:
+    _FUSE_CELL_UP[0] = bool(enabled)
+
+
+def cell_up_fusion_enabled() -> bool:
+    return _FUSE_CELL_UP[0]
+
+
+def set_head_up_fusion(enabled: bool) -> None:
+    _FUSE_HEAD_UP[0] = bool(enabled)
+
+
+def head_up_fusion_enabled() -> bool:
+    return _FUSE_HEAD_UP[0]
+
+
+def conv3d_k1_up_supported(cin: int, cmid: int, cout: int, in_size: Sequence[int], size: Sequence[int], cin_s: int = 0,
+                           cout_s: int = 0) -> bool:
+    return bool(load_library().ragmi_conv3d_k1_up_supported(int(cin), int(cmid), int(cout), *[int(v) for v in in_size],
+                                                            *[int(v) for v in size], int(cin_s), int(cout_s)))
+
+
+def conv3d_k1_up(x: torch.Tensor, w1: torch.Tensor, scale1, shift1, relu1: bool, chain, size: Sequence[int], relu: bool,
+                 out: torch.Tensor, out_ch0: int = 0, same=None) -> torch.Tensor:
+    from ._lib import K1UpSpec
+    _need_gpu(w1, scale1, shift1)
+    dt = _act(x, out)
+    p = lambda t: t.data_ptr() if t is not None else None
+    B, Cin, Di, Hi, Wi = x.shape
+    Do, Ho, Wo = [int(v) for v in size]
+    d = K1UpSpec()
+    d.x, d.x_bstride, d.Cin, d.Di, d.Hi, d.Wi = x.data_ptr(), _planes(x), Cin, Di, Hi, Wi
+    d.weight1, d.scale1, d.shift1, d.relu1 = w1.data_ptr(), p(scale1), p(shift1), int(relu1)
+    if not w1.is_contiguous() or w1.shape[1] != Cin:
+        raise ValueError("conv3d_k1_up: weights must be contiguous [Cout, Cin]")
+    cout = w1.shape[0]
+    if chain is not None:
+        w2, scale2, shift2 = chain
+        _need_gpu(w2, scale2, shift2)
+        if not w2.is_contiguous() or w2.shape[1] != w1.shape[0]:
+            raise ValueError("conv3d_k1_up: chain weight must be contiguous [Cout, Cmid]")
+        d.Cmid, d.weight2, d.scale2, d.shift2 = w1.shape[0], w2.data_ptr(), p(scale2), p(shift2)
+        cout = w2.shape[0]
+    d.Cout, d.relu = cout, int(relu)
+    if out_ch0 + cout > out.shape[1] or tuple(out.shape[2:]) != (Do, Ho, Wo) or out.shape[0] != B:
+        raise ValueError("conv3d_k1_up: output buffer too small / wrong size")
+    d.y, d.y_bstride, d.y_ch0, d.Do, d.Ho, d.Wo = out.data_ptr(), _planes(out), int(out_ch0), Do, Ho, Wo
+    if same is not None:
+        xs, ws, scale_s, shift_s, relu_s, out_s, ch0_s = same
+        _need_gpu(ws, scale_s, shift_s)
+        if _act(xs, out_s) != dt:
+            raise ValueError("conv3d_k1_up: one storage type per launch")
+        if (tuple(xs.shape[2:]) != (Do, Ho, Wo) or tuple(out_s.shape[2:]) != (Do, Ho, Wo) or xs.shape[0] != B or out_s.shape[0] != B
+                or not ws.is_contiguous() or ws.shape[1] != xs.shape[1] or ch0_s + ws.shape[0] > out_s.shape[1]):
+            raise ValueError("conv3d_k1_up: same-size conv: wrong sizes")
+        d.xs, d.xs_bstride, d.Cin_s, d.Cout_s = xs.data_ptr(), _planes(xs), xs.shape[1], ws.shape[0]
+        d.weight_s, d.scale_s, d.shift_s, d.relu_s = ws.data_ptr(), p(scale_s), p(shift_s), int(relu_s)
+        d.ys, d.ys_bstride, d.ys_ch0 = out_s.data_ptr(), _planes(out_s), int(ch0_s)
+    check(load_library().ragmi_conv3d_k1_up_fwd(ctypes.byref(d), B, dt, _stream()), "conv3d_k1_up")
+    return out
+
+
 def cell2d_supported(C: int, cin0: int, cin1: int, cout: int, H: int, W: int, dtype=torch.float32) -> bool:
     if dtype != torch.float32:
         return False
```

Result: no change. 1078 disparity maps/s (-0.2%).
